# gafniguy/4D-Facial-Avatars

Measured on AMD Instinct MI355X. Metric: rays/sec at 512x512, 64 coarse + 128 fine samples, higher is better.
Workload: dtype f32; 1 GPU; configs[1]: paper-model eval forward, 512x512 frame, 64+128 samples, chunksize 65536, perturb on, expression+latent conditioned, background prior; frames sharded over GPUs

## Files before the change

### 4d-facial-avatars_amd/csrc/nf_mlp_gated_stats.hip

```cpp
#include "nf_mlp_live_kernel.h"

static int nf_gated_stats_launch(bool clocks, const float* packed, const float* bound, const float* cond, const float* ro, const float* rd,
                                 const float* rd_view, const float* z, int64_t n_rays, int n_samples, float* raw, float* scratch,
                                 size_t scratch_floats, int max_workgroups, int64_t* stats, size_t stats_rows, nf_stream_t stream) {
    static_assert(sizeof(long long) == sizeof(int64_t), "a statistics row is int64s");
    if (max_workgroups < 0 || !stats || ((uintptr_t)stats & 7) || stats_rows < (size_t)nf_live_grid_cap(max_workgroups) * NF_MLP_WAVES) return NF_EINVAL;
    const size_t cols = NF_GATE_STAT_COLS + (clocks ? NF_LIVE_PHASES : 0);
    const hipError_t e = hipMemsetAsync(stats, 0, stats_rows * cols * sizeof(int64_t), nf_s(stream));
    if (e != hipSuccess) return (int)e;
    return nf_live_launch<true, true>(packed, cond, ro, rd, rd_view, z, n_rays, n_samples, raw, scratch, scratch_floats, max_workgroups,
                                      reinterpret_cast<long long*>(stats), stream, bound, clocks);
}

extern "C" int nf_paper_mlp_fwd_gated_stats(const float* packed, const float* bound, const float* cond, const float* ro, const float* rd,
                                            const float* rd_view, const float* z, int64_t n_rays, int n_samples, float* raw, float* scratch,
                                            size_t scratch_floats, int max_workgroups, int64_t* stats, size_t stats_rows, nf_stream_t stream) {
    return nf_gated_stats_launch(false, packed, bound, cond, ro, rd, rd_view, z, n_rays, n_samples, raw, scratch, scratch_floats, max_workgroups,
                                 stats, stats_rows, stream);
}

extern "C" int nf_paper_mlp_fwd_gated_phases(const float* packed, const float* bound, const float* cond, const float* ro, const float* rd,
                                             const float* rd_view, const float* z, int64_t n_rays, int n_samples, float* raw, float* scratch,
                                             size_t scratch_floats, int max_workgroups, int64_t* stats, size_t stats_rows, nf_stream_t stream) {
    return nf_gated_stats_launch(true, packed, bound, cond, ro, rd, rd_view, z, n_rays, n_samples, raw, scratch, scratch_floats, max_workgroups,
                                 stats, stats_rows, stream);
}
```

### 4d-facial-avatars_amd/csrc/nf_mlp_live_kernel.h

```cpp
#pragma once
#include <mutex>
#include "nf_mlp_paper_net.h"

#define NF_LIVE_ROWS 64
#ifndef NF_LIVE_PF
#define NF_LIVE_PF 8
#endif
#define NF_LIVE_DIR_B (NF_LIVE_ROWS * 1024)
#define NF_LIVE_META_B (NF_LIVE_DIR_B + NF_LIVE_ROWS * 64)
#define NF_LIVE_WAVE_B (NF_LIVE_META_B + NF_LIVE_ROWS * 16)
#define NF_LIVE_OOB NF_LIVE_WAVE_B
#define NF_LIVE_SC1 16

static_assert(NF_LIVE_ROWS == 64 && NF_MLP_NT == 2, "row numbers wrap with & 63; a pass's liveness is one 32-bit mask");
static_assert(NF_LIVE_PF >= 0 && NF_LIVE_PF <= 16, "prefetched rows live in registers beside fc_alpha's weights");

__device__ __forceinline__ __amdgpu_buffer_rsrc_t nf_live_ring(char* ring_v) {
    const uint64_t a = (uint64_t)ring_v;
    const uint64_t s = (uint64_t)(uint32_t)__builtin_amdgcn_readfirstlane((int)(uint32_t)a) |
                       ((uint64_t)(uint32_t)__builtin_amdgcn_readfirstlane((int)(a >> 32)) << 32);
    return __builtin_amdgcn_make_buffer_rsrc(reinterpret_cast<char*>(s), (short)0, NF_LIVE_WAVE_B, 0x00020000);
}
__device__ __forceinline__ void nf_live_store(__amdgpu_buffer_rsrc_t ring, int off_b, f32x4 v) {
    __builtin_amdgcn_raw_buffer_store_b128(__builtin_bit_cast(nf_u32x4, v), ring, off_b, 0, 0);
}
__device__ __forceinline__ f32x4 nf_live_load(__amdgpu_buffer_rsrc_t ring, int off_b) {
    return __builtin_bit_cast(f32x4, __builtin_amdgcn_raw_buffer_load_b128(ring, off_b, 0, NF_LIVE_SC1));
}
__device__ __forceinline__ int nf_live_pop(unsigned& m) {
    const int r = __builtin_ctz(m);
    m &= m - 1u;
    return r;
}
__device__ __forceinline__ int nf_live_slab(int prow, int lane) { return nf_act_idx4(prow, lane); }

struct NfLivePre {
    NfStream<NF_MLP_NT>& st;
    f32x4 (&wd)[16];
    f32x4 (&pf)[NF_LIVE_PF > 0 ? NF_LIVE_PF : 1];
    char* ring_v;
    int head_v, tail_v;
    __device__ __forceinline__ void wait() const {
        __builtin_amdgcn_fence(__ATOMIC_RELEASE, "workgroup");
        __builtin_amdgcn_s_waitcnt(0x0F70);
        __builtin_amdgcn_fence(__ATOMIC_ACQUIRE, "workgroup");
    }
    __device__ __forceinline__ void loads(const NfW& Wi, const NfW& Ci, int lane) {
        using Net = NfPaperNet;
        const __amdgpu_buffer_rsrc_t ring = nf_live_ring(ring_v);
        const int tail = __builtin_amdgcn_readfirstlane(tail_v), cnt = __builtin_amdgcn_readfirstlane(head_v) - tail;
#pragma unroll
        for (int i = 0; i < NF_LIVE_PF; ++i)
            pf[i] = nf_live_load(ring, i < cnt ? ((tail + i) & (NF_LIVE_ROWS - 1)) * 1024 + lane * 16 : NF_LIVE_OOB);
        nf_load_bias<8>(st.bias, Ci, Net::B_D0, lane);
        nf_load_w16<8>(st.wa, Wi, Net::OFF_D0 / 4, lane);
        nf_load_w16<8>(wd, Wi, Net::OFF_D0 / 4 + 16 * 9 * 64, lane);
        __builtin_amdgcn_sched_barrier(0);
    }
};

struct NfGatePre {
    NfStream<NF_MLP_NT>& st;
    f32x4 (&pf)[NF_LIVE_PF > 0 ? NF_LIVE_PF : 1];
    char* ring_v;
    int head_v, tail_v;
    const float* bound_v;
    __device__ __forceinline__ NfW image() const {
        const uint64_t a = (uint64_t)bound_v;
        const uint64_t s = (uint64_t)(uint32_t)__builtin_amdgcn_readfirstlane((int)(uint32_t)a) |
                           ((uint64_t)(uint32_t)__builtin_amdgcn_readfirstlane((int)(a >> 32)) << 32);
        return nf_w_image(reinterpret_cast<const float*>(s), NF_BOUND_FLOATS);
    }
    __device__ __forceinline__ void wait() const {
        __builtin_amdgcn_fence(__ATOMIC_RELEASE, "workgroup");
        __builtin_amdgcn_s_waitcnt(0x0F70);
        __builtin_amdgcn_fence(__ATOMIC_ACQUIRE, "workgroup");
    }
    __device__ __forceinline__ void loads(const NfW& Wi, const NfW& Ci, int lane) {
        using Net = NfPaperNet;
        const __amdgpu_buffer_rsrc_t ring = nf_live_ring(ring_v);
        const int tail = __builtin_amdgcn_readfirstlane(tail_v), cnt = __builtin_amdgcn_readfirstlane(head_v) - tail;
#pragma unroll
        for (int i = 0; i < NF_LIVE_PF; ++i)
            pf[i] = nf_live_load(ring, i < cnt ? ((tail + i) & (NF_LIVE_ROWS - 1)) * 1024 + lane * 16 : NF_LIVE_OOB);
        nf_load_bias<16>(st.bias, Ci, Net::B_FEAT, lane);
        nf_load_w16<16>(st.wa, Wi, Net::OFF_FEAT / 4, lane);
        __builtin_amdgcn_sched_barrier(0);
    }
};

#define NF_LIVE_STAT_UNITS 0
#define NF_LIVE_STAT_RUNS 1
#define NF_LIVE_STAT_FLUSH 2
#define NF_LIVE_STAT_CLOCK 3
#define NF_GATE_STAT_PROVEN 4
#define NF_LIVE_PH_TRUNK 0
#define NF_LIVE_PH_TILE 1
#define NF_LIVE_PH_APPEND 2
#define NF_LIVE_PH_ENTRY 3
#define NF_LIVE_PH_RUN 4
#define NF_LIVE_PH_DEAD 5
#define NF_LIVE_PHASES 6
#define NF_LIVE_STAT_COLS 4
#define NF_GATE_STAT_COLS 5

template <bool STATS, int COLS = NF_LIVE_STAT_COLS>
__device__ __forceinline__ void nf_live_stat(long long* stats, int col, long long add, bool set = false) {
    if constexpr (STATS) {
        const int cols = COLS + (((uintptr_t)stats & 1) ? NF_LIVE_PHASES : 0);
        stats = reinterpret_cast<long long*>((uintptr_t)stats & ~(uintptr_t)7);
        if ((threadIdx.x & 63) == 0) {
            long long* at = stats + ((size_t)blockIdx.x * NF_MLP_WAVES + (threadIdx.x >> 6)) * cols + col;
            if (set) *at = add;
            else (void)__hip_atomic_fetch_add(at, add, __ATOMIC_RELAXED, __HIP_MEMORY_SCOPE_AGENT);
        }
    }
}

template <bool STATS, int COLS>
__device__ __forceinline__ void nf_live_mark(long long* stats, int end, int start) {
    if constexpr (STATS) {
        if ((uintptr_t)stats & 1) {
            __builtin_amdgcn_sched_barrier(0);
            const long long t = (long long)__builtin_amdgcn_s_memtime();
            if ((threadIdx.x & 63) == 0) {
                long long* row = reinterpret_cast<long long*>((uintptr_t)stats & ~(uintptr_t)7) +
                                 ((size_t)blockIdx.x * NF_MLP_WAVES + (threadIdx.x >> 6)) * (COLS + NF_LIVE_PHASES) + COLS;
                if (end >= 0) (void)__hip_atomic_fetch_add(row + end, t, __ATOMIC_RELAXED, __HIP_MEMORY_SCOPE_AGENT);
                if (start >= 0) (void)__hip_atomic_fetch_add(row + start, -t, __ATOMIC_RELAXED, __HIP_MEMORY_SCOPE_AGENT);
            }
            __builtin_amdgcn_sched_barrier(0);
        }
    }
}
template <class Pre, int COLS>
struct NfMarkedPre : Pre {
    long long* stats;
    __device__ __forceinline__ void wait() const {
        nf_live_mark<true, COLS>(stats, NF_LIVE_PH_TRUNK, NF_LIVE_PH_TILE);
        Pre::wait();
    }
};

template <int NT, bool STATS, bool GATE = false>
__global__ void __launch_bounds__(64 * NF_MLP_WAVES, 1)
k_paper_mlp_fwd_live(const float* __restrict__ packed, const float* __restrict__ cond_, const float* __restrict__ ro,
                     const float* __restrict__ rd, const float* __restrict__ rd_view, const float* __restrict__ z,
                     int64_t n_points, int S, float* __restrict__ raw, float* __restrict__ scratch, unsigned* __restrict__ counter,
                     long long* __restrict__ stats, const float* __restrict__ bound) {
    using Net = NfPaperNet;
    constexpr int COLS = GATE ? NF_GATE_STAT_COLS : NF_LIVE_STAT_COLS;
    __shared__ __attribute__((aligned(16))) f32x4 lds[NF_MLP_WAVES * 16 * NT * 64];
    const int lane = threadIdx.x & 63, wave = threadIdx.x >> 6;
    f32x4* act4 = lds + wave * (16 * NT * 64);
    typedef __attribute__((address_space(1))) f32x4 nf_gf32x4;
    nf_gf32x4* raw_v = (nf_gf32x4*)raw;
    asm volatile("" : "+v"(raw_v));
    char* ring_v = reinterpret_cast<char*>(scratch) + ((size_t)blockIdx.x * NF_MLP_WAVES + wave) * NF_LIVE_WAVE_B;
    asm volatile("" : "+v"(ring_v));
    const float* z_v = z;
    const float* rdv_v = rd_view;
    asm volatile("" : "+v"(z_v), "+v"(rdv_v));
    const float* bound_v = bound;
    if constexpr (GATE) asm volatile("" : "+v"(bound_v));
    int head_v = 0, tail_v = 0;
    asm volatile("" : "+v"(head_v), "+v"(tail_v));
    typedef __attribute__((address_space(1))) unsigned nf_gu32;
    nf_gu32* ctr_v = (nf_gu32*)counter;
    asm volatile("" : "+v"(ctr_v));
    unsigned unit_v = 0;
    if (lane == 0) unit_v = __hip_atomic_fetch_add(ctr_v, 1u, __ATOMIC_RELAXED, __HIP_MEMORY_SCOPE_AGENT);
    asm volatile("" : "+v"(unit_v));
#pragma unroll 1
    for (;;) {
        const int64_t p0 = (int64_t)(uint32_t)__builtin_amdgcn_readfirstlane((int)unit_v) * (16 * NT);
        int64_t p0_v = p0;
        asm volatile("" : "+v"(p0_v));
        int more_v = p0 < n_points;
        asm volatile("" : "+v"(more_v));
        const bool more = __builtin_amdgcn_readfirstlane(more_v) != 0;
        unsigned next_v = 0;
        if (more && lane == 0) next_v = __hip_atomic_fetch_add(ctr_v, 1u, __ATOMIC_RELAXED, __HIP_MEMORY_SCOPE_AGENT);
        if (more) nf_live_stat<STATS, COLS>(stats, NF_LIVE_STAT_UNITS, 1);
        int opaque0 = 0;
        asm volatile("" : "+s"(opaque0));
        const NfW Wi = nf_w_image(packed + opaque0, Net::PACKED), Ci = nf_w_image(cond_ + opaque0, Net::COND_FLOATS);
        NfStream<NT> st;
        f32x4 wd[16], pf[NF_LIVE_PF > 0 ? NF_LIVE_PF : 1];
        f32x4 dirf[NT][1];
        float sigma_own[NT];
        float tag_own[NT] = {};
        bool proven[NT] = {};
        int live_v = 0, run_v = 0;
        if (more) {
            nf_live_mark<STATS, COLS>(stats, -1, NF_LIVE_PH_TRUNK);
            f32x4 pe[NT][4];
            nf_net_inputs<NT>(pe, dirf, p0, n_points, S, lane, ro, rd, rdv_v, z_v);
            f32x4 acc[NT][16];
            if constexpr (GATE) {
                if constexpr (STATS)
                    nf_paper_net_body<Net, NT, 1, true, NfMarkedPre<NfGatePre, COLS>, true>(
                        acc, sigma_own, pe, dirf, Wi, Ci, act4, lane, NfMarkedPre<NfGatePre, COLS>{{st, pf, ring_v, head_v, tail_v, bound_v}, stats});
                else
                    nf_paper_net_body<Net, NT, 1, true, NfGatePre, true>(acc, sigma_own, pe, dirf, Wi, Ci, act4, lane,
                                                                         NfGatePre{st, pf, ring_v, head_v, tail_v, bound_v});
#pragma unroll
                for (int t = 0; t < NT; ++t) {
                    const float s = acc[t][8].x, u = acc[t][8].y;
                    sigma_own[t] = nf_add(s, nf_mul(u, 0x1p-13f));
                    proven[t] = sigma_own[t] < -0x1p-100f && s > -INFINITY && u < INFINITY;
                }
            } else if constexpr (STATS) {
                nf_paper_net_body<Net, NT, 1, true>(acc, sigma_own, pe, dirf, Wi, Ci, act4, lane,
                                                    NfMarkedPre<NfLivePre, COLS>{{st, wd, pf, ring_v, head_v, tail_v}, stats});
            } else {
                nf_paper_net_body<Net, NT, 1, true>(acc, sigma_own, pe, dirf, Wi, Ci, act4, lane, NfLivePre{st, wd, pf, ring_v, head_v, tail_v});
            }
            nf_live_mark<STATS, COLS>(stats, NF_LIVE_PH_TILE, NF_LIVE_PH_APPEND);
            int lane_o = lane;
            asm volatile("" : "+v"(lane_o));
            const int g = lane_o >> 4, c = lane_o & 15;
            unsigned live = 0;
            int S_o = S;
            asm volatile("" : "+v"(S_o));
            const int64_t p0_o = (int64_t)(uint32_t)__builtin_amdgcn_readfirstlane((int)(uint32_t)p0_v) |
                                 ((int64_t)__builtin_amdgcn_readfirstlane((int)(p0_v >> 32)) << 32);
#pragma unroll
            for (int t = 0; t < NT; ++t) {
                const int64_t p = p0_o + 16 * t + c;
                bool is_live;
                if constexpr (GATE) {
                    const bool last = (p + 1) % S_o == 0;
                    is_live = g == 0 && p < n_points && (!proven[t] || last);
                    tag_own[t] = __int_as_float(last ? 1 : 0);
                } else {
                    is_live = g == 0 && p < n_points && (!(sigma_own[t] <= 0.0f) || (p + 1) % S_o == 0);
                }
                live |= ((unsigned)__builtin_amdgcn_ballot_w64(is_live) & 0xffffu) << (16 * t);
            }
            const int head = __builtin_amdgcn_readfirstlane(head_v), cnt = head - __builtin_amdgcn_readfirstlane(tail_v);
            const int n_live = __builtin_popcount(live);
            live_v = (int)live;
            if constexpr (GATE) {
                const int64_t left = n_points - p0_o;
                nf_live_stat<STATS, COLS>(stats, NF_GATE_STAT_PROVEN, (left < 16 * NT ? (int)left : 16 * NT) - n_live);
            }
            if (cnt + n_live >= 16 * NT) {
                run_v = 1;
            } else {
                const __amdgpu_buffer_rsrc_t ring = nf_live_ring(ring_v);
                unsigned mm = live;
#pragma unroll 1
                for (int i = 0; i < n_live; i += 4) {
                    f32x4 v[4];
                    int off[4];
#pragma unroll
                    for (int u = 0; u < 4; ++u) {
                        const bool ok = i + u < n_live;
                        const int r = ok ? nf_live_pop(mm) : 0;
                        off[u] = ok ? ((head + i + u) & (NF_LIVE_ROWS - 1)) * 1024 + lane_o * 16 : NF_LIVE_OOB;
                        v[u] = act4[nf_live_slab(r, lane_o)];
                    }
#pragma unroll
                    for (int u = 0; u < 4; ++u) nf_live_store(ring, off[u], v[u]);
                }
#pragma unroll
                for (int t = 0; t < NT; ++t) {
                    const int bit = 16 * t + c;
                    if ((live >> bit) & 1u) {
                        const int row = (head + __builtin_popcount(live & ((1u << bit) - 1u))) & (NF_LIVE_ROWS - 1);
                        nf_live_store(ring, NF_LIVE_DIR_B + row * 64 + g * 16, dirf[t][0]);
                        if (g == 0) {
                            const int64_t p = p0_o + bit;
                            nf_live_store(ring, NF_LIVE_META_B + row * 16,
                                          (f32x4){__int_as_float((int)(uint32_t)p), __int_as_float((int)(p >> 32)), GATE ? tag_own[t] : sigma_own[t], 0.0f});
                        }
                    }
                }
                head_v = head + n_live;
                asm volatile("" : "+v"(head_v));
            }
            nf_live_mark<STATS, COLS>(stats, NF_LIVE_PH_APPEND, -1);
        } else {
            if constexpr (GATE) {
                NfGatePre pre{st, pf, ring_v, head_v, tail_v, bound_v};
                pre.wait();
                pre.loads(Wi, Ci, lane);
            } else {
                NfLivePre pre{st, wd, pf, ring_v, head_v, tail_v};
                pre.wait();
                pre.loads(Wi, Ci, lane);
            }
#pragma unroll
            for (int t = 0; t < NT; ++t) {
                dirf[t][0] = (f32x4){0.0f, 0.0f, 0.0f, 0.0f};
                sigma_own[t] = 0.0f;
            }
            run_v = __builtin_amdgcn_readfirstlane(head_v) != __builtin_amdgcn_readfirstlane(tail_v) ? 2 : 0;
        }
        asm volatile("" : "+v"(live_v), "+v"(run_v));
        const int run = __builtin_amdgcn_readfirstlane(run_v);
        if (run != 0) {
            nf_live_stat<STATS, COLS>(stats, NF_LIVE_STAT_RUNS, 1);
            if (run == 2) nf_live_stat<STATS, COLS>(stats, NF_LIVE_STAT_FLUSH, __builtin_amdgcn_readfirstlane(head_v) - __builtin_amdgcn_readfirstlane(tail_v));
            nf_live_mark<STATS, COLS>(stats, -1, NF_LIVE_PH_ENTRY);
            int lane_o = lane;
            asm volatile("" : "+v"(lane_o));
            const int g = lane_o >> 4, c = lane_o & 15;
            const __amdgpu_buffer_rsrc_t ring = nf_live_ring(ring_v);
            const int tail = __builtin_amdgcn_readfirstlane(tail_v), cnt = __builtin_amdgcn_readfirstlane(head_v) - tail;
            const unsigned own = run == 1 ? (unsigned)__builtin_amdgcn_readfirstlane(live_v) : 0u;
            const unsigned fill = run == 1 ? ~own : (1u << cnt) - 1u;
            const int n_fill = __builtin_popcount(fill);
            f32x4 meta[NT];
            bool valid[NT];
#pragma unroll
            for (int t = 0; t < NT; ++t) {
                const int bit = 16 * t + c;
                const bool f = (fill >> bit) & 1u;
                const int row = (tail + __builtin_popcount(fill & ((1u << bit) - 1u))) & (NF_LIVE_ROWS - 1);
                const f32x4 fd = nf_live_load(ring, f ? NF_LIVE_DIR_B + row * 64 + g * 16 : NF_LIVE_OOB);
                const f32x4 fm = nf_live_load(ring, f ? NF_LIVE_META_B + row * 16 : NF_LIVE_OOB);
                const int64_t p = (p0_v) + bit;
                dirf[t][0] = f ? fd : dirf[t][0];
                meta[t] = f ? fm : (f32x4){__int_as_float((int)(uint32_t)p), __int_as_float((int)(p >> 32)), GATE ? tag_own[t] : sigma_own[t], 0.0f};
                valid[t] = f || ((own >> bit) & 1u);
            }
            unsigned hh = fill;
#pragma unroll
            for (int i = 0; i < NF_LIVE_PF; ++i) {
                if (i < n_fill) {
                    const int h = nf_live_pop(hh);
                    act4[nf_live_slab(h, lane_o)] = pf[i];
                }
            }
#pragma unroll 1
            for (int i = NF_LIVE_PF; i < n_fill; i += 4) {
                f32x4 v[4];
                int h[4];
#pragma unroll
                for (int u = 0; u < 4; ++u) {
                    const bool ok = i + u < n_fill;
                    h[u] = ok ? nf_live_pop(hh) : -1;
                    v[u] = nf_live_load(ring, ok ? ((tail + i + u) & (NF_LIVE_ROWS - 1)) * 1024 + lane_o * 16 : NF_LIVE_OOB);
                }
#pragma unroll
                for (int u = 0; u < 4; ++u)
                    if (h[u] >= 0) act4[nf_live_slab(h[u], lane_o)] = v[u];
            }
            constexpr int NDIR = 1;
            constexpr unsigned D0 = Net::OFF_D0 / 4;
            nf_read_b<NT>(st.b0, act4, lane, 0);
            nf_live_mark<STATS, COLS>(stats, NF_LIVE_PH_ENTRY, NF_LIVE_PH_RUN);
            f32x4 acc[NT][16], bj[NT];
            float sigma_raw[NT];
            if constexpr (GATE) {
                nf_seg_lds<NT, 16, true, true>(acc, st, Wi, Net::OFF_FEAT / 4, 16, act4, lane);
                nf_pending_b<NT, true>(bj, st);
                nf_tail<NT, 16, 16, 9, 1>(acc, st.wb, bj, st, Wi, D0, Ci, Net::B_D0, act4, lane);
                NF_NET_COLOUR();
            } else {
                NF_NET_COLOUR_D0(8, 9, wd);
                NF_NET_COLOUR_REST();
            }
            int lane_s = lane;
            asm volatile("" : "+v"(lane_s));
            if ((lane_s >> 4) == 0) {
#pragma unroll
                for (int t = 0; t < NT; ++t) {
                    if (valid[t]) {
                        const int64_t p = (int64_t)(uint32_t)__float_as_int(meta[t].x) | ((int64_t)__float_as_int(meta[t].y) << 32);
                        if constexpr (GATE) {
                            const bool keep = !(sigma_raw[t] <= 0.0f) || __float_as_int(meta[t].z) != 0;
                            if (p >= 0 && p < n_points)
                                raw_v[p] = (f32x4){keep ? acc[t][0].x : 0.0f, keep ? acc[t][0].y : 0.0f, keep ? acc[t][0].z : 0.0f, sigma_raw[t]};
                        } else {
                            if (p >= 0 && p < n_points) raw_v[p] = (f32x4){acc[t][0].x, acc[t][0].y, acc[t][0].z, meta[t].z};
                        }
                    }
                }
            }
            tail_v = tail + n_fill;
            asm volatile("" : "+v"(tail_v));
            nf_live_mark<STATS, COLS>(stats, NF_LIVE_PH_RUN, -1);
        }
        asm volatile("" : "+v"(more_v));
        if (__builtin_amdgcn_readfirstlane(more_v) == 0) break;
        {
            nf_live_mark<STATS, COLS>(stats, -1, NF_LIVE_PH_DEAD);
            int lane_s = lane;
            asm volatile("" : "+v"(lane_s));
            const int g = lane_s >> 4, c = lane_s & 15;
            asm volatile("" : "+v"(live_v));
#pragma unroll
            for (int t = 0; t < NT; ++t) {
                const int64_t p = p0_v + 16 * t + c;
                if (g == 0 && p < n_points && !(((unsigned)live_v >> (16 * t + c)) & 1u)) raw_v[p] = (f32x4){0.0f, 0.0f, 0.0f, sigma_own[t]};
            }
            nf_live_mark<STATS, COLS>(stats, NF_LIVE_PH_DEAD, -1);
        }
        asm volatile("" : "+v"(next_v));
        unit_v = next_v;
    }
    nf_live_stat<STATS, COLS>(stats, NF_LIVE_STAT_CLOCK, (long long)wall_clock64(), true);
}

static inline int64_t nf_live_grid_cap(int max_workgroups) {
    const int64_t cu = nf_cu_count();
    return max_workgroups > 0 && max_workgroups < cu ? max_workgroups : cu;
}

#define NF_LIVE_SLOTS 256
#define NF_LIVE_SLOT_B 128

inline unsigned* nf_live_counter(hipStream_t stream) {
    struct Pool {
        char* base;
        const void* owner[NF_LIVE_SLOTS];
        int used;
    };
    static std::mutex mu;
    static Pool pools[64];
    static thread_local char this_thread;
    int dev = 0;
    if (hipGetDevice(&dev) != hipSuccess || dev < 0 || dev >= 64) return nullptr;
    const void* key = stream == hipStreamPerThread ? (const void*)&this_thread : (const void*)stream;
    std::lock_guard<std::mutex> lock(mu);
    Pool& p = pools[dev];
    if (!p.base) {
        void* mem = nullptr;
        if (hipMalloc(&mem, (size_t)NF_LIVE_SLOTS * NF_LIVE_SLOT_B) != hipSuccess) {
            (void)hipGetLastError();
            return nullptr;
        }
        p.base = (char*)mem;
        p.used = 0;
    }
    int i = 0;
    while (i < p.used && p.owner[i] != key) ++i;
    if (i == p.used) {
        if (p.used == NF_LIVE_SLOTS) {
            if (hipDeviceSynchronize() != hipSuccess) return nullptr;
            p.used = i = 0;
        }
        p.owner[p.used++] = key;
    }
    return reinterpret_cast<unsigned*>(p.base + (size_t)i * NF_LIVE_SLOT_B);
}

template <bool STATS, bool GATE = false>
static inline int nf_live_launch(const float* packed, const float* cond, const float* ro, const float* rd, const float* rd_view, const float* z,
                                 int64_t n_rays, int n_samples, float* raw, float* scratch, size_t scratch_floats, int max_workgroups,
                                 long long* stats, nf_stream_t stream, const float* bound = nullptr, bool clocks = false) {
    static_assert(NF_MLP_WAVES * 16 * NF_MLP_NT == 128, "nf_mlp_fwd_launch sizes the grid for 128 points per workgroup");
    if (max_workgroups < 0 || !scratch || ((uintptr_t)scratch & 15) ||
        scratch_floats < (size_t)nf_live_grid_cap(max_workgroups) * NF_MLP_WAVES * (NF_LIVE_WAVE_B / 4) ||
        (GATE && (!bound || ((uintptr_t)bound & 15))))
        return NF_EINVAL;
    const float* rdv = rd_view ? rd_view : rd;
    if (STATS && clocks) stats = reinterpret_cast<long long*>((uintptr_t)stats | 1);
    int rc = 0;
    const int launched = nf_mlp_fwd_launch(NF_FWD_INFER, packed, cond, ro, rd, z, raw, nullptr, n_rays, n_samples, [&](int64_t n_points, unsigned grid) {
        if ((n_points + 31) / 32 > ((int64_t)1 << 31)) {
            rc = NF_EINVAL;
            return;
        }
        unsigned* counter = nf_live_counter(nf_s(stream));
        if (!counter) {
            rc = (int)hipErrorOutOfMemory;
            return;
        }
        const hipError_t e = hipMemsetAsync(counter, 0, sizeof(unsigned), nf_s(stream));
        if (e != hipSuccess) {
            rc = (int)e;
            return;
        }
        const int64_t cap = nf_live_grid_cap(max_workgroups);
        hipLaunchKernelGGL((k_paper_mlp_fwd_live<NF_MLP_NT, STATS, GATE>), dim3((unsigned)(grid < cap ? grid : cap)), dim3(64 * NF_MLP_WAVES), 0,
                           nf_s(stream), packed, cond, ro, rd, rdv, z, n_points, n_samples, raw, scratch, counter, stats, bound);
    });
    return rc ? rc : launched;
}
```

### 4d-facial-avatars_amd/csrc/nf_mlp_live_stats.hip

```cpp
#include "nf_mlp_live_kernel.h"

static int nf_live_stats_launch(bool clocks, const float* packed, const float* cond, const float* ro, const float* rd, const float* rd_view,
                                const float* z, int64_t n_rays, int n_samples, float* raw, float* scratch, size_t scratch_floats,
                                int max_workgroups, int64_t* stats, size_t stats_rows, nf_stream_t stream) {
    static_assert(sizeof(long long) == sizeof(int64_t), "a statistics row is int64s");
    if (max_workgroups < 0 || !stats || ((uintptr_t)stats & 7) || stats_rows < (size_t)nf_live_grid_cap(max_workgroups) * NF_MLP_WAVES) return NF_EINVAL;
    const size_t cols = NF_LIVE_STAT_COLS + (clocks ? NF_LIVE_PHASES : 0);
    const hipError_t e = hipMemsetAsync(stats, 0, stats_rows * cols * sizeof(int64_t), nf_s(stream));
    if (e != hipSuccess) return (int)e;
    return nf_live_launch<true>(packed, cond, ro, rd, rd_view, z, n_rays, n_samples, raw, scratch, scratch_floats, max_workgroups,
                                reinterpret_cast<long long*>(stats), stream, nullptr, clocks);
}

extern "C" int nf_paper_mlp_fwd_live_stats(const float* packed, const float* cond, const float* ro, const float* rd, const float* rd_view,
                                           const float* z, int64_t n_rays, int n_samples, float* raw, float* scratch, size_t scratch_floats,
                                           int max_workgroups, int64_t* stats, size_t stats_rows, nf_stream_t stream) {
    return nf_live_stats_launch(false, packed, cond, ro, rd, rd_view, z, n_rays, n_samples, raw, scratch, scratch_floats, max_workgroups, stats,
                                stats_rows, stream);
}

extern "C" int nf_paper_mlp_fwd_live_phases(const float* packed, const float* cond, const float* ro, const float* rd, const float* rd_view,
                                            const float* z, int64_t n_rays, int n_samples, float* raw, float* scratch, size_t scratch_floats,
                                            int max_workgroups, int64_t* stats, size_t stats_rows, nf_stream_t stream) {
    return nf_live_stats_launch(true, packed, cond, ro, rd, rd_view, z, n_rays, n_samples, raw, scratch, scratch_floats, max_workgroups, stats,
                                stats_rows, stream);
}
```

### 4d-facial-avatars_amd/csrc/nf_mlp_net_common.h

```cpp
#pragma once
#include "nf_mlp_dev.h"
#include "nf_mlp_stream.h"

template <int NT>
__device__ __forceinline__ void nf_net_inputs(f32x4 (&pe)[NT][4], f32x4 (&dirf)[NT][1], int64_t p0, int64_t n_points, int S, int lane,
                                              const float* __restrict__ ro, const float* __restrict__ rd,
                                              const float* __restrict__ rd_view, const float* __restrict__ z) {
    const int g = lane >> 4, c = lane & 15;
#pragma unroll
    for (int t = 0; t < NT; ++t) {
        int64_t p = p0 + 16 * t + c;
        if (p >= n_points) p = n_points - 1;
        const int64_t ray = p / S;
        const float zz = z[p];
        const float dx = rd[ray * 3 + 0], dy = rd[ray * 3 + 1], dz = rd[ray * 3 + 2];
        const float px = nf_add(ro[ray * 3 + 0], nf_mul(dx, zz));
        const float py = nf_add(ro[ray * 3 + 1], nf_mul(dy, zz));
        const float pz = nf_add(ro[ray * 3 + 2], nf_mul(dz, zz));
        nf_encode_point(px, py, pz, g, pe[t]);
        float s, cs;
        nf_sincos(nf_mul(rd_view[ray * 3 + 2], (float)(1 << g)), &s, &cs);
        dirf[t][0] = (f32x4){s, cs, 0.0f, 0.0f};
    }
}

template <int NT>
__device__ __forceinline__ void nf_net_inputs_encoded(f32x4 (&pe)[NT][4], f32x4 (&dirf)[NT][2], int64_t p0, int64_t n_points, int lane,
                                                      const float* __restrict__ x87) {
    const int g = lane >> 4, c = lane & 15;
#pragma unroll
    for (int t = 0; t < NT; ++t) {
        int64_t p = p0 + 16 * t + c;
        if (p >= n_points) p = n_points - 1;
        const float* row = x87 + p * 87;
#pragma unroll
        for (int j = 0; j < 4; ++j) {
            float v[4];
#pragma unroll
            for (int r = 0; r < 4; ++r) {
                const int col = nfl::pe_slot_to_col(16 * j + 4 * g + r);
                v[r] = col >= 0 ? row[col] : 0.0f;
            }
            pe[t][j] = (f32x4){v[0], v[1], v[2], v[3]};
        }
#pragma unroll
        for (int j = 0; j < 2; ++j) {
            float v[4];
#pragma unroll
            for (int r = 0; r < 4; ++r) {
                const int s = 16 * j + 4 * g + r;
                v[r] = s < 24 ? row[63 + s] : 0.0f;
            }
            dirf[t][j] = (f32x4){v[0], v[1], v[2], v[3]};
        }
    }
}

template <int NT>
__device__ __forceinline__ void nf_net_store_raw(const f32x4 (&acc)[NT][16], const float (&sigma_raw)[NT], int64_t p0, int64_t n_points,
                                                 int lane, float* __restrict__ out) {
    const int g = lane >> 4, c = lane & 15;
    if (g == 0) {
#pragma unroll
        for (int t = 0; t < NT; ++t) {
            const int64_t p = p0 + 16 * t + c;
            if (p < n_points) reinterpret_cast<f32x4*>(out)[p] = (f32x4){acc[t][0].x, acc[t][0].y, acc[t][0].z, sigma_raw[t]};
        }
    }
}

#define NF_NET_PE_B(J_) do { _Pragma("unroll") for (int t = 0; t < NT; ++t) bj[t] = pe[t][J_]; } while (0)
#define NF_NET_PE_LAYER(B_, OFF_, OFF_NEXT_, B_NEXT_)                                                         \
    do {                                                                                                      \
        nf_load_bias<16>(st.bias, Ci, B_, lane);                                                              \
        f32x4 w[16];                                                                                          \
        nf_load_w16<16>(w, Wi, (OFF_) / 4, lane);                                                             \
        NF_NET_PE_B(0); nf_chunk<NT, 16, true>(acc, w, bj, st.bias);                                          \
        nf_load_w16<16>(w, Wi, (OFF_) / 4 + 1 * 16 * 64, lane);                                               \
        NF_NET_PE_B(1); nf_chunk<NT, 16, false>(acc, w, bj, st.bias);                                         \
        nf_load_w16<16>(w, Wi, (OFF_) / 4 + 2 * 16 * 64, lane);                                               \
        NF_NET_PE_B(2); nf_chunk<NT, 16, false>(acc, w, bj, st.bias);                                         \
        nf_load_w16<16>(w, Wi, (OFF_) / 4 + 3 * 16 * 64, lane);                                               \
        NF_NET_PE_B(3); nf_tail<NT, 16, 16, 16, 1>(acc, w, bj, st, Wi, (OFF_NEXT_) / 4, Ci, B_NEXT_, act4, lane); \
    } while (0)

#define NF_NET_SAVE_PENDING(RELU_, MASKL_, NCH_)                                                    \
    do {                                                                                            \
        nf_pending_b<NT, RELU_>(bj, st);                                                            \
        if ((MASKL_) >= 0) {                                                                        \
            nf_mask_bits<NT>(m64, st.bp, (NCH_) - 2);                                               \
            nf_mask_bits<NT>(m64, bj, (NCH_) - 1);                                                  \
            _Pragma("unroll") for (int t = 0; t < NT; ++t)                                          \
                if (p0 + 16 * t < n)                                                                \
                    *nf_mask_ptr<Net::S_MASK>(saved, n, (MASKL_) >= 0 ? (MASKL_) : 0, (p0 >> 4) + t, lane) = make_uint2((uint32_t)m64[t], (uint32_t)(m64[t] >> 32)); \
        }                                                                                           \
    } while (0)
#define NF_NET_SAVE_LAYER256(OFF_, FIRST_, SEC_, MASKL_, OFF_NEXT_, B_NEXT_, NO_NEXT_, NEXT_B_)                           \
    do {                                                                                                                   \
        NfCopyH<64, 4, ((MASKL_) >= 0)> cs{act4, sec(SEC_, 256), lane, 8, {}};                                             \
        cs.prime();                                                                                                        \
        _Pragma("unroll") for (int t = 0; t < NT; ++t) m64[t] = 0;                                                         \
        nf_seg_lds<NT, 16, FIRST_, ((MASKL_) >= 0), ((MASKL_) >= 0)>(acc, st, Wi, OFF_, 16, act4, lane, cs, m64);          \
        NF_NET_SAVE_PENDING(((MASKL_) >= 0), MASKL_, 16);                                                                  \
        nf_tail<NT, 16, 16, NO_NEXT_, NEXT_B_>(acc, st.wb, bj, st, Wi, OFF_NEXT_, Ci, B_NEXT_, act4, lane);               \
    } while (0)

#define NF_NET_CHAIN_BEGIN(MASKL_, OFF_NEXT_, NO_NEXT_)                                                               \
    static_assert(NT == 2, "the copy schedule below is written for 32-point slabs");                                 \
    const int lane = threadIdx.x & 63, wave = threadIdx.x >> 6;                                                      \
    const int g = lane >> 4, c = lane & 15;                                                                          \
    const int64_t p0 = ((int64_t)blockIdx.x * NF_MLP_WAVES + wave) * (16 * NT);                                      \
    if (p0 >= n_points) return;                                                                                      \
    f32x4* act4 = lds + wave * (16 * NT * 64);                                                                       \
    const int64_t n = n_points;                                                                                      \
    const NfW Wi = nf_w_image(packed_t, Net::PACKED_T);                                                              \
    auto sec = [&](int zs, int width) { return nf_slab_copy(dz, zs, width, p0, n); };                                \
    auto masks = [&](int l, uint2 (&m)[NT]) {                                                                        \
        _Pragma("unroll") for (int t = 0; t < NT; ++t)                                                               \
            m[t] = p0 + 16 * t < n ? *nf_mask_ptr<Net::S_MASK>(const_cast<float*>(saved), n, l, (p0 >> 4) + t, lane) : make_uint2(0u, 0u); \
    };                                                                                                               \
    f32x4 frag_rgb[NT][1], frag_sig[NT];                                                                             \
    _Pragma("unroll") for (int t = 0; t < NT; ++t) {                                                                 \
        const int64_t p = p0 + 16 * t + c;                                                                           \
        f32x4 d = (f32x4){0.f, 0.f, 0.f, 0.f};                                                                       \
        if (p < n && g == 0) d = reinterpret_cast<const f32x4*>(d_raw)[p];                                           \
        frag_rgb[t][0] = (f32x4){d.x, d.y, d.z, 0.f};                                                                \
        frag_sig[t] = (f32x4){d.w, 0.f, 0.f, 0.f};                                                                   \
    }                                                                                                                \
    f32x4 acc[NT][16];                                                                                               \
    NfStream<NT> st;                                                                                                 \
    f32x4 bj[NT];                                                                                                    \
    uint64_t unused64[NT];                                                                                           \
    uint2 m[NT];                                                                                                     \
    _Pragma("unroll") for (int no = 0; no < 16; ++no) st.bias[no] = (f32x4){0.f, 0.f, 0.f, 0.f};                     \
    masks(MASKL_, m);                                                                                                \
    nf_zero_acc<NT, 8>(acc);                                                                                         \
    nf_mma_from_regs<NT, 8, 1>(acc, reinterpret_cast<const f32x4*>(packed_t) + Net::OFFT_RGB / 4, frag_rgb, lane);   \
    nf_apply_mask<NT, 8>(acc, m);                                                                                    \
    nf_store_act<NT, 8, false>(acc, act4, lane);                                                                     \
    nf_load_w16<NO_NEXT_>(st.wa, Wi, OFF_NEXT_, lane);                                                               \
    nf_read_b<NT>(st.b0, act4, lane, 0)
#define NF_NET_CHAIN_LAYER(OFF_, NO_, NCH_, W4_, ZSEC_, MASKL_, OFF_NEXT_, NO_NEXT_)                                   \
    do {                                                                                                             \
        NfCopyH<W4_, 4, false> cs{act4, sec(ZSEC_, 4 * (W4_)), lane, (NCH_) / 2, {}};                                  \
        cs.prime();                                                                                                  \
        if ((MASKL_) >= 0) masks((MASKL_) >= 0 ? (MASKL_) : 0, m);                                                   \
        nf_seg_lds<NT, NO_, true, false, false>(acc, st, Wi, OFF_, NCH_, act4, lane, cs, unused64);                  \
        nf_pending_b<NT, false>(bj, st);                                                                             \
        nf_tail_dz<NT, NO_, NO_NEXT_, ((MASKL_) >= 0)>(acc, st.wb, bj, st, Wi, OFF_NEXT_, act4, lane, m);            \
    } while (0)
#define NF_NET_CHAIN_END(ZSEC_)                                                                                      \
    do {                                                                                                             \
        const NfSlabCopy cp = sec(ZSEC_, 256);                                                                       \
        _Pragma("unroll 4") for (int k = 0; k < 16 * NT; ++k) nf_copy_rows<64>(act4, cp, k, lane);                   \
    } while (0)
```

### 4d-facial-avatars_amd/csrc/nf_mlp_paper_net.h

```cpp
#pragma once
#include "nf_mlp_net_common.h"
#include "nf_mlp_smaller_layout.h"
#include "nf_pack.h"

#define NF_NET_COMMON(F)                                                                                                              \
    F(FRAG) F(NCOND) F(OFF_L0) F(OFF_L1) F(OFF_L2) F(OFF_L3) F(OFF_L4) F(OFF_FEAT) F(OFF_D0) F(OFF_D0E) F(OFF_D1) F(OFF_D2) F(OFF_RGB) \
    F(OFF_WC0) F(OFF_WC3) F(OFF_WCD) F(OFF_BIAS) F(B_L0) F(B_L1) F(B_L2) F(B_L3) F(B_L4) F(B_FEAT) F(B_D0) F(B_D1) F(B_D2) F(B_RGB)     \
    F(B_CVEC) F(B_DVEC) F(COND_FLOATS) F(S_PE) F(S_H0) F(S_H1) F(S_H2) F(S_H3) F(S_H4) F(S_FEAT) F(S_D0) F(S_D1) F(S_D2) F(S_DIRF)     \
    F(S_MASK) F(SAVED_PER_POINT) F(Z_L0) F(Z_L1) F(Z_L2) F(Z_L3) F(Z_L4) F(Z_FEAT) F(Z_D0) F(Z_D1) F(Z_D2) F(DZ_PER_POINT)             \
    F(OFFT_RGB) F(OFFT_D2) F(OFFT_D1) F(OFFT_D0) F(OFFT_FEAT) F(OFFT_L4) F(OFFT_L3) F(OFFT_L2) F(OFFT_L1)                              \
    F(G_L0) F(G_L1) F(G_L2) F(G_L3A) F(G_L3B) F(G_L4) F(G_FEAT) F(G_D0A) F(G_D0B) F(G_D1) F(G_D2) F(G_RGB) F(G_ALPHA)                  \
    F(CS_L0) F(CS_D0) F(CS_RGB) F(SLAB_FLOATS) F(GRAD_PARAM_FLOATS) F(GRAD_FLOATS)

struct NfPaperNet {
#define NF_NET_COPY(X) static constexpr int X = nfl::X;
    NF_NET_COMMON(NF_NET_COPY)
    NF_NET_COPY(OFF_L5) NF_NET_COPY(B_L5) NF_NET_COPY(S_H5) NF_NET_COPY(Z_L5) NF_NET_COPY(OFFT_L5) NF_NET_COPY(G_L5)
#undef NF_NET_COPY
    static constexpr bool HAS_L5 = true, D0_EXPR = false;
    static constexpr int PACKED = nfl::PACKED_FLOATS, PACKED_T = nfl::PACKED_T_FLOATS, NPARAMS = NF_PAPER_NUM_PARAMS;
    static constexpr int N_RELU = (nfl::SAVED_PER_POINT - nfl::S_MASK) / 8;
    static constexpr int D0_COLS = 280;
    static constexpr int MODEL = 0;
};

struct NfSmallerNet {
#define NF_NET_COPY(X) static constexpr int X = nsm::X;
    NF_NET_COMMON(NF_NET_COPY)
    NF_NET_COPY(OFF_WCE) NF_NET_COPY(NEXPR) NF_NET_COPY(PACKED) NF_NET_COPY(PACKED_T) NF_NET_COPY(NPARAMS) NF_NET_COPY(N_RELU)
#undef NF_NET_COPY
    static constexpr bool HAS_L5 = false, D0_EXPR = true;
    static constexpr int D0_COLS = 280 + nsm::NEXPR;
    static constexpr int MODEL = 2;
};
#undef NF_NET_COMMON

template <class Net> constexpr int nf_net_n_xyz = Net::HAS_L5 ? 6 : 5;

enum { NF_R_XYZ0_W = 0, NF_R_XYZ3_W = 6, NF_R_L5_W = 10, NF_R_FEAT_W = 12, NF_R_FEAT_B = 13, NF_R_ALPHA_W = 14, NF_R_ALPHA_B = 15,
       NF_R_DIR0_W = 16, NF_R_DIR0_B = 17, NF_R_DIR1_W = 18, NF_R_DIR2_W = 20, NF_R_RGB_W = 24, NF_R_RGB_B = 25 };
template <class Net>
__host__ __device__ constexpr int nf_net_id(int role) {
    return role >= NF_R_RGB_W ? Net::NPARAMS - 2 + (role - NF_R_RGB_W) : (role >= NF_R_FEAT_W && !Net::HAS_L5 ? role - 2 : role);
}
template <class Net>
__host__ __device__ constexpr int nf_net_role(int id) {
    return id >= Net::NPARAMS - 2 ? NF_R_RGB_W + (id - (Net::NPARAMS - 2)) : (id >= NF_R_L5_W && !Net::HAS_L5 ? id + 2 : id);
}

template <class Net>
static void nf_paper_net_table(std::vector<uint32_t>& t) {
    constexpr int NX = nf_net_n_xyz<Net>;
    auto id = [](int role) { return nf_net_id<Net>(role); };
    t.assign(Net::PACKED, NF_ZERO_CODE);
    auto fill = [&](int off, int nk, int no_tiles, int tensor, int n_out, int n_cols, auto col_of, int alpha_row = -1) {
        nf_fill_frag(t, off, nk, no_tiles, [&](int slot, int n) {
            if (n < n_out) {
                const int col = col_of(slot);
                return col >= 0 ? nf_code(tensor, n, col, n_cols) : NF_ZERO_CODE;
            }
            return n == alpha_row && slot < 256 ? nf_code(id(NF_R_ALPHA_W), 0, slot, 256) : NF_ZERO_CODE;
        });
    };
    auto ident = [](int s) { return s; };
    fill(Net::OFF_L0, 4, 16, NF_R_XYZ0_W, 256, 171, [](int s) { return nfl::pe_slot_to_col(s); });
    fill(Net::OFF_L1, 16, 16, 2, 256, 256, ident);
    fill(Net::OFF_L2, 16, 16, 4, 256, 256, ident);
    fill(Net::OFF_L3, 20, 16, NF_R_XYZ3_W, 256, 427, [](int s) { return s < 64 ? nfl::pe_slot_to_col(s) : 171 + (s - 64); });
    fill(Net::OFF_L4, 16, 16, 8, 256, 256, ident);
    if constexpr (Net::HAS_L5) fill(Net::OFF_L5, 16, 16, NF_R_L5_W, 256, 256, ident);
    fill(Net::OFF_FEAT, 16, 16, id(NF_R_FEAT_W), 256, 256, ident);
    fill(Net::OFF_D0, 17, 9, id(NF_R_DIR0_W), 128, Net::D0_COLS,
         [](int s) {
             if (s < 256) return s;
             const int g = ((s - 256) >> 2) & 3, r = (s - 256) & 3;
             return r < 2 ? 256 + 6 * g + 3 * r : -1;
         },
         128);
    fill(Net::OFF_D0E, 18, 9, id(NF_R_DIR0_W), 128, Net::D0_COLS, [](int s) { return s < 280 ? s : -1; }, 128);
    fill(Net::OFF_D1, 8, 8, id(NF_R_DIR1_W), 128, 128, ident);
    fill(Net::OFF_D2, 8, 8, id(NF_R_DIR2_W), 128, 128, ident);
    fill(Net::OFF_RGB, 8, 1, id(NF_R_RGB_W), 3, 128, ident);
    for (int n = 0; n < 256; ++n)
        for (int k = 0; k < Net::NCOND; ++k) {
            t[Net::OFF_WC0 + n * Net::NCOND + k] = nf_code(NF_R_XYZ0_W, n, 63 + k, 171);
            t[Net::OFF_WC3 + n * Net::NCOND + k] = nf_code(NF_R_XYZ3_W, n, 63 + k, 427);
        }
    for (int n = 0; n < 128; ++n) {
        for (int f = 0; f < 4; ++f)
            for (int sc = 0; sc < 2; ++sc)
                for (int comp = 1; comp < 3; ++comp)
                    t[Net::OFF_WCD + n * 16 + 4 * f + 2 * sc + (comp - 1)] = nf_code(id(NF_R_DIR0_W), n, 256 + 6 * f + 3 * sc + comp, Net::D0_COLS);
        if constexpr (Net::D0_EXPR)
            for (int k = 0; k < Net::NEXPR; ++k) t[Net::OFF_WCE + n * Net::NEXPR + k] = nf_code(id(NF_R_DIR0_W), n, 280 + k, Net::D0_COLS);
    }
    for (int n = 0; n < 256; ++n) {
        for (int l = 0; l < NX; ++l) t[Net::OFF_BIAS + 256 * l + n] = nf_code(2 * l + 1, 0, n, 256);
        t[Net::OFF_BIAS + Net::B_FEAT + n] = nf_code(id(NF_R_FEAT_B), 0, n, 256);
    }
    for (int n = 0; n < 128; ++n) {
        t[Net::OFF_BIAS + Net::B_D0 + n] = nf_code(id(NF_R_DIR0_B), 0, n, 128);
        t[Net::OFF_BIAS + Net::B_D1 + n] = nf_code(id(NF_R_DIR1_W) + 1, 0, n, 128);
        t[Net::OFF_BIAS + Net::B_D2 + n] = nf_code(id(NF_R_DIR2_W) + 1, 0, n, 128);
    }
    t[Net::OFF_BIAS + Net::B_D0 + 128] = nf_code(id(NF_R_ALPHA_B), 0, 0, 1);
    for (int n = 0; n < 3; ++n) t[Net::OFF_BIAS + Net::B_RGB + n] = nf_code(id(NF_R_RGB_B), 0, n, 3);
}

template <class Net>
static inline size_t nf_paper_net_saved_floats(int64_t n_points) {
    return (size_t)Net::SAVED_PER_POINT * (size_t)((n_points + 31) & ~(int64_t)31) + Net::N_RELU * 128;
}

template <class Net, bool DIRS>
__device__ __forceinline__ void nf_paper_net_condition(const float* __restrict__ packed, const float* __restrict__ expr,
                                                       const float* __restrict__ latent, float near_z, float far_z, float* __restrict__ cond) {
    __shared__ float cvec[Net::NCOND];
    __shared__ float dvec[16];
    const int tid = threadIdx.x;
    if (tid < 76) cvec[tid] = nf_div(nf_mul(expr[tid], 1.0f), 3.0f);
    else if (tid < Net::NCOND) cvec[tid] = latent[tid - 76];
    if (tid >= 128 && tid < 144) {
        const int k = tid - 128, f = k >> 2, sc = (k >> 1) & 1, comp = k & 1;
        const float a = nf_mul(comp ? far_z : near_z, exp2f((float)f));
        dvec[k] = DIRS ? (sc ? cosf(a) : sinf(a)) : 0.0f;
    }
    __syncthreads();
    const float* bias = packed + Net::OFF_BIAS;
    for (int i = blockIdx.x * blockDim.x + tid; i < Net::COND_FLOATS; i += gridDim.x * blockDim.x) {
        if (i >= Net::B_CVEC) { cond[i] = i < Net::B_DVEC ? cvec[i - Net::B_CVEC] : dvec[i - Net::B_DVEC]; continue; }
        float v = bias[i];
        if (i < Net::B_L1 || (i >= Net::B_L3 && i < Net::B_L4)) {
            const int n = i < Net::B_L1 ? i : i - Net::B_L3;
            const float* w = packed + (i < Net::B_L1 ? Net::OFF_WC0 : Net::OFF_WC3) + n * Net::NCOND;
            float s = 0.0f;
            for (int k = 0; k < Net::NCOND; ++k) s = fmaf(w[k], cvec[k], s);
            v += s;
        } else if ((DIRS || Net::D0_EXPR) && i >= Net::B_D0 && i < Net::B_D0 + 128) {
            float s = 0.0f;
            if (DIRS) {
                const float* w = packed + Net::OFF_WCD + (i - Net::B_D0) * 16;
                for (int k = 0; k < 16; ++k) s = fmaf(w[k], dvec[k], s);
            }
            if constexpr (Net::D0_EXPR) {
                const float* we = packed + Net::OFF_WCE + (i - Net::B_D0) * Net::NEXPR;
                for (int k = 0; k < Net::NEXPR; ++k) s = fmaf(we[k], cvec[k], s);
            }
            v += s;
        }
        cond[i] = v;
    }
}

template <class Net>
static inline dim3 nf_paper_net_condition_grid() { return dim3((Net::COND_FLOATS + 255) / 256); }

#define NF_NET_L3_PE()                                                                                        \
    do {                                                                                                      \
        NF_NET_PE_B(0); nf_chunk<NT, 16, true>(acc, st.wa, bj, st.bias);                                          \
        nf_load_w16<16>(st.wa, Wi, Net::OFF_L3 / 4 + 4 * 16 * 64, lane);    \
        nf_read_b<NT>(st.b0, act4, lane, 0);                                                                  \
        f32x4 w[16];                                                                                          \
        nf_load_w16<16>(w, Wi, Net::OFF_L3 / 4 + 1 * 16 * 64, lane);                                          \
        NF_NET_PE_B(1); nf_chunk<NT, 16, false>(acc, w, bj, st.bias);                                             \
        nf_load_w16<16>(w, Wi, Net::OFF_L3 / 4 + 2 * 16 * 64, lane);                                          \
        NF_NET_PE_B(2); nf_chunk<NT, 16, false>(acc, w, bj, st.bias);                                             \
        nf_load_w16<16>(w, Wi, Net::OFF_L3 / 4 + 3 * 16 * 64, lane);                                          \
        NF_NET_PE_B(3); nf_chunk<NT, 16, false>(acc, w, bj, st.bias);                                             \
    } while (0)

#define NF_NET_COLOUR_D0(NO0_, WS0_, WD_)                                                                                  \
                                \
    {                                                                                                                      \
        nf_seg_lds<NT, NO0_, true, false, WS0_>(acc, st, Wi, D0, 16, act4, lane);                                          \
        nf_pending_b<NT, false>(bj, st);                                                                                   \
        nf_chunk<NT, NO0_, false>(acc, st.wb, bj, st.bias);                                                                \
        if (NDIR == 2) {                                                                                                   \
            nf_load_w16<NO0_>(st.wb, Wi, D0 + 17 * (WS0_) * 64, lane);                                                     \
            _Pragma("unroll") for (int t = 0; t < NT; ++t) bj[t] = dirf[t][0];                                             \
            nf_chunk<NT, NO0_, false>(acc, WD_, bj, st.bias);                                                              \
        }                                                                                                                  \
        _Pragma("unroll") for (int t = 0; t < NT; ++t) bj[t] = dirf[t][NDIR - 1];                                          \
        if constexpr (NDIR == 2) nf_tail<NT, NO0_, 8, 8, 1>(acc, st.wb, bj, st, Wi, Net::OFF_D1 / 4, Ci, Net::B_D1, act4, lane); \
        else nf_tail<NT, NO0_, 8, 8, 1>(acc, WD_, bj, st, Wi, Net::OFF_D1 / 4, Ci, Net::B_D1, act4, lane);                  \
        if constexpr ((NO0_) > 8) { _Pragma("unroll") for (int t = 0; t < NT; ++t) sigma_raw[t] = acc[t][8].x; }           \
    }
#define NF_NET_COLOUR()                                                                                                    \
    {                                                                                                                      \
        f32x4 wd[16];                                                                                                      \
        nf_load_w16<9>(wd, Wi, D0 + 16 * 9 * 64, lane);                      \
        NF_NET_COLOUR_D0(9, 9, wd);                                                                                        \
    }                                                                                                                      \
    NF_NET_COLOUR_REST()
#define NF_NET_COLOUR_REST()                                                                                               \
                                                                                           \
    nf_seg_lds<NT, 8, true, true>(acc, st, Wi, Net::OFF_D1 / 4, 8, act4, lane);                                            \
    nf_pending_b<NT, true>(bj, st);                                                                                        \
    nf_tail<NT, 8, 8, 8, 1>(acc, st.wb, bj, st, Wi, Net::OFF_D2 / 4, Ci, Net::B_D2, act4, lane);                           \
    nf_seg_lds<NT, 8, true, true>(acc, st, Wi, Net::OFF_D2 / 4, 8, act4, lane);                                            \
    nf_pending_b<NT, true>(bj, st);                                                                                        \
    nf_tail<NT, 8, 8, 1, 1>(acc, st.wb, bj, st, Wi, Net::OFF_RGB / 4, Ci, Net::B_RGB, act4, lane);                         \
                                                                                                     \
    nf_seg_lds<NT, 1, true, true>(acc, st, Wi, Net::OFF_RGB / 4, 8, act4, lane);                                           \
    nf_pending_b<NT, true>(bj, st);                                                                                        \
    nf_chunk<NT, 1, false>(acc, st.wb, bj, st.bias)

struct NfNoPre {
    __device__ __forceinline__ void wait() const {}
    __device__ __forceinline__ void loads(const NfW&, const NfW&, int) const {}
};
#define NF_BOUND_BIAS 4096
#define NF_BOUND_FLOATS (NF_BOUND_BIAS + 16)
template <int NT, bool RELU_IN, class Pre>
__device__ __forceinline__ void nf_net_lone_tile(f32x4 (&acc)[NT][16], const NfStream<NT>& st, f32x4 (&bj)[NT], const NfW& W, unsigned first4,
                                                 unsigned stride4, const NfW& Wi, const NfW& Ci, const f32x4* act4, int lane, Pre& pre) {
    f32x4 w8[16];
    w8[0] = st.wa[0];
    pre.wait();
#pragma unroll
    for (int ch = 1; ch < 16; ++ch) w8[ch] = nf_load_w1(W, first4 + stride4 * ch, lane);
    if constexpr (RELU_IN) __builtin_amdgcn_sched_barrier(0);
    pre.loads(Wi, Ci, lane);
    if constexpr (RELU_IN) {
        f32x4 cur[NT], nxt[NT];
#pragma unroll
        for (int t = 0; t < NT; ++t) cur[t] = nf_relu_i(st.b0[t]);
#pragma unroll
        for (int ch = 0; ch < 16; ++ch) {
            if (ch + 1 < 16) nf_read_b<NT>(nxt, act4, lane, ch + 1);
            __builtin_amdgcn_sched_barrier(0);
#pragma unroll
            for (int r = 0; r < 2; ++r)
#pragma unroll
                for (int t = 0; t < NT; ++t)
                    acc[t][8] = __builtin_amdgcn_mfma_f32_16x16x4f32(w8[ch][r], cur[t][r], (ch == 0 && r == 0) ? st.bias[0] : acc[t][8], 0, 0, 0);
#pragma unroll
            for (int r = 2; r < 4; ++r)
#pragma unroll
                for (int t = 0; t < NT; ++t) {
                    __builtin_amdgcn_sched_barrier(0);
                    if (ch + 1 < 16) {
                        const int e = 2 * (r - 2);
#pragma unroll
                        for (int q = e; q < e + 2; ++q) {
                            const int xi = __float_as_int(nxt[t][q]);
                            nxt[t][q] = __int_as_float(xi > 0 ? xi : 0);
                        }
                    }
                    __builtin_amdgcn_sched_barrier(0);
                    acc[t][8] = __builtin_amdgcn_mfma_f32_16x16x4f32(w8[ch][r], cur[t][r], acc[t][8], 0, 0, 0);
                }
            __builtin_amdgcn_sched_barrier(0);
#pragma unroll
            for (int t = 0; t < NT; ++t) cur[t] = nxt[t];
        }
        return;
    }
#pragma unroll
    for (int ch = 0; ch < 16; ++ch) {
        if (ch == 0) {
#pragma unroll
            for (int t = 0; t < NT; ++t) bj[t] = RELU_IN ? nf_relu_i(st.b0[t]) : st.b0[t];
        } else {
            nf_read_b<NT>(bj, act4, lane, ch);
            if (RELU_IN) {
#pragma unroll
                for (int t = 0; t < NT; ++t) bj[t] = nf_relu_i(bj[t]);
            }
        }
#pragma unroll
        for (int r = 0; r < 4; ++r)
#pragma unroll
            for (int t = 0; t < NT; ++t)
                acc[t][8] = __builtin_amdgcn_mfma_f32_16x16x4f32(w8[ch][r], bj[t][r], (ch == 0 && r == 0) ? st.bias[0] : acc[t][8], 0, 0, 0);
    }
}
template <class Net, int NT, int NDIR, bool SIGMA = false, class Pre = NfNoPre, bool GATE = false>
__device__ __forceinline__ void nf_paper_net_body(f32x4 (&acc)[NT][16], float (&sigma_raw)[NT], const f32x4 (&pe)[NT][4],
                                                  const f32x4 (&dirf)[NT][NDIR], const NfW& Wi, const NfW& Ci, f32x4* act4, int lane,
                                                  Pre pre = Pre()) {
    static_assert(!GATE || (SIGMA && Net::HAS_L5), "the bound tile stands in for fc_alpha's lone tile, behind layers_xyz.5");
    constexpr unsigned D0 = (NDIR == 1 ? Net::OFF_D0 : Net::OFF_D0E) / 4;
    NfStream<NT> st;
    f32x4 bj[NT];
#define NF_NET_LAYER256(OFF_, FIRST_, OFF_NEXT_, B_NEXT_, NO_NEXT_, NEXT_B_)                                                \
    nf_seg_lds<NT, 16, FIRST_, true>(acc, st, Wi, OFF_, 16, act4, lane);                                                    \
    nf_pending_b<NT, true>(bj, st);                                                                                         \
    nf_tail<NT, 16, 16, NO_NEXT_, NEXT_B_>(acc, st.wb, bj, st, Wi, OFF_NEXT_, Ci, B_NEXT_, act4, lane)
    NF_NET_PE_LAYER(Net::B_L0, Net::OFF_L0, Net::OFF_L1, Net::B_L1);
    NF_NET_LAYER256(Net::OFF_L1 / 4, true, Net::OFF_L2 / 4, Net::B_L2, 16, 1);
    NF_NET_LAYER256(Net::OFF_L2 / 4, true, Net::OFF_L3 / 4, Net::B_L3, 16, 0);
    NF_NET_L3_PE();
    NF_NET_LAYER256(Net::OFF_L3 / 4 + 4 * 16 * 64, false, Net::OFF_L4 / 4, Net::B_L4, 16, 1);
    if constexpr (GATE) {
        NF_NET_LAYER256(Net::OFF_L4 / 4, true, Net::OFF_L5 / 4, Net::B_L5, 16, 1);
        const NfW Bi = pre.image();
        nf_seg_lds<NT, 16, true, true>(acc, st, Wi, Net::OFF_L5 / 4, 16, act4, lane);
        nf_pending_b<NT, true>(bj, st);
        nf_tail<NT, 16, 16, 1, 1>(acc, st.wb, bj, st, Bi, 0, Bi, NF_BOUND_BIAS, act4, lane);
        nf_net_lone_tile<NT, true>(acc, st, bj, Bi, 0, 64, Wi, Ci, act4, lane, pre);
        return;
    } else if constexpr (Net::HAS_L5) {
        NF_NET_LAYER256(Net::OFF_L4 / 4, true, Net::OFF_L5 / 4, Net::B_L5, 16, 1);
        NF_NET_LAYER256(Net::OFF_L5 / 4, true, Net::OFF_FEAT / 4, Net::B_FEAT, 16, 1);
    } else {
        NF_NET_LAYER256(Net::OFF_L4 / 4, true, Net::OFF_FEAT / 4, Net::B_FEAT, 16, 1);
    }
    if constexpr (SIGMA) {
        NF_NET_LAYER256(Net::OFF_FEAT / 4, true, D0 + 8 * 64, Net::B_D0 + 128, 1, 1);
        nf_net_lone_tile<NT, false>(acc, st, bj, Wi, D0 + 8 * 64, 9 * 64, Wi, Ci, act4, lane, pre);
#pragma unroll
        for (int t = 0; t < NT; ++t) sigma_raw[t] = acc[t][8].x;
        return;
    }
    NF_NET_LAYER256(Net::OFF_FEAT / 4, true, D0, Net::B_D0, 9, 1);
#undef NF_NET_LAYER256
    NF_NET_COLOUR();
}

template <class Net, int NT>
__device__ __forceinline__ void nf_paper_net_fwd_encoded(f32x4* lds, const float* __restrict__ packed, const float* __restrict__ cond,
                                                         const float* __restrict__ x87, int64_t n_points, float* __restrict__ out) {
    const int lane = threadIdx.x & 63, wave = threadIdx.x >> 6;
    const int64_t p0 = ((int64_t)blockIdx.x * NF_MLP_WAVES + wave) * (16 * NT);
    if (p0 >= n_points) return;
    f32x4* act4 = lds + wave * (16 * NT * 64);
    f32x4 pe[NT][4];
    f32x4 dirf[NT][2];
    nf_net_inputs_encoded<NT>(pe, dirf, p0, n_points, lane, x87);
    f32x4 acc[NT][16];
    float sigma_raw[NT];
    const NfW Wi = nf_w_image(packed, Net::PACKED), Ci = nf_w_image(cond, Net::COND_FLOATS);
    nf_paper_net_body<Net, NT, 2>(acc, sigma_raw, pe, dirf, Wi, Ci, act4, lane);
    nf_net_store_raw<NT>(acc, sigma_raw, p0, n_points, lane, out);
}

template <class Condition, class Forward>
static inline int nf_paper_net_forward_encoded(const float* packed, const float* x87, const float* expr76, const float* latent32,
                                               int64_t n_points, float* cond, float* out, Condition condition, Forward forward) {
    if (n_points == 0) return 0;
    if (!packed || !x87 || !expr76 || !latent32 || !cond || !out || n_points < 0) return NF_EINVAL;
    condition();
    const int64_t per_block = (int64_t)NF_MLP_WAVES * 16 * NF_MLP_NT;
    const int64_t grid = (n_points + per_block - 1) / per_block;
    if (grid > 0x7fffffff) return NF_EINVAL;
    forward((unsigned)grid);
    NF_RETURN_LAUNCH();
}

template <class Net, int NT>
__device__ __forceinline__ void nf_paper_net_body_save(f32x4 (&acc)[NT][16], float (&sigma_raw)[NT], const f32x4 (&pe)[NT][4],
                                                       const f32x4 (&dirf)[NT][1], const NfW& Wi, const NfW& Ci, f32x4* act4, int lane,
                                                       float* __restrict__ saved, int64_t p0, int64_t n) {
    static_assert(NT == 2, "the copy schedule below is written for 32-point slabs");
    constexpr int NX = nf_net_n_xyz<Net>;
    const int g = lane >> 4, c = lane & 15;
    auto sec = [&](int s, int width) { return nf_slab_copy(saved, s, width, p0, n); };
#pragma unroll
    for (int t = 0; t < NT; ++t) {
        const int64_t p = p0 + 16 * t + c;
        if (p < n) *reinterpret_cast<f32x4*>(saved + Net::S_DIRF * n + p * 16 + 4 * g) = dirf[t][0];
#pragma unroll
        for (int j = 0; j < 4; ++j) act4[nf_act_idx4(16 * t + c, 4 * j + g)] = pe[t][j];
    }
    {
        const NfSlabCopy cp = sec(Net::S_PE, 64);
#pragma unroll
        for (int k = 0; k < 16 * NT / 4; ++k) nf_copy_rows<16>(act4, cp, k, lane);
    }
    uint64_t m64[NT];
    NfStream<NT> st;
    f32x4 bj[NT];
#define NF_NET_LAYER128(OFF_, NO_, SEC_, MASKL_)                                                                          \
    NfCopyH<32, 4, true> cs{act4, sec(SEC_, 128), lane, 4, {}};                                                            \
    cs.prime();                                                                                                            \
    _Pragma("unroll") for (int t = 0; t < NT; ++t) m64[t] = 0;                                                             \
    nf_seg_lds<NT, NO_, true, true, true>(acc, st, Wi, OFF_, 8, act4, lane, cs, m64);                                      \
    NF_NET_SAVE_PENDING(true, MASKL_, 8)
    NF_NET_PE_LAYER(Net::B_L0, Net::OFF_L0, Net::OFF_L1, Net::B_L1);
    NF_NET_SAVE_LAYER256(Net::OFF_L1 / 4, true, Net::S_H0, 0, Net::OFF_L2 / 4, Net::B_L2, 16, 1);
    NF_NET_SAVE_LAYER256(Net::OFF_L2 / 4, true, Net::S_H1, 1, Net::OFF_L3 / 4, Net::B_L3, 16, 0);
    NF_NET_L3_PE();
    NF_NET_SAVE_LAYER256(Net::OFF_L3 / 4 + 4 * 16 * 64, false, Net::S_H2, 2, Net::OFF_L4 / 4, Net::B_L4, 16, 1);
    if constexpr (Net::HAS_L5) {
        NF_NET_SAVE_LAYER256(Net::OFF_L4 / 4, true, Net::S_H3, 3, Net::OFF_L5 / 4, Net::B_L5, 16, 1);
        NF_NET_SAVE_LAYER256(Net::OFF_L5 / 4, true, Net::S_H4, 4, Net::OFF_FEAT / 4, Net::B_FEAT, 16, 1);
        NF_NET_SAVE_LAYER256(Net::OFF_FEAT / 4, true, Net::S_H5, 5, Net::OFF_D0 / 4, Net::B_D0, 9, 1);
    } else {
        NF_NET_SAVE_LAYER256(Net::OFF_L4 / 4, true, Net::S_H3, 3, Net::OFF_FEAT / 4, Net::B_FEAT, 16, 1);
        NF_NET_SAVE_LAYER256(Net::OFF_FEAT / 4, true, Net::S_H4, 4, Net::OFF_D0 / 4, Net::B_D0, 9, 1);
    }
    {
        f32x4 wd[16];
        nf_load_w16<9>(wd, Wi, Net::OFF_D0 / 4 + 16 * 9 * 64, lane);
        NfCopyH<64, 4, false> cs{act4, sec(Net::S_FEAT, 256), lane, 8, {}};
        cs.prime();
        nf_seg_lds<NT, 9, true, false, false>(acc, st, Wi, Net::OFF_D0 / 4, 16, act4, lane, cs, m64);
        NF_NET_SAVE_PENDING(false, -1, 16);
        nf_chunk<NT, 9, false>(acc, st.wb, bj, st.bias);
#pragma unroll
        for (int t = 0; t < NT; ++t) bj[t] = dirf[t][0];
        nf_tail<NT, 9, 8, 8, 1>(acc, wd, bj, st, Wi, Net::OFF_D1 / 4, Ci, Net::B_D1, act4, lane);
#pragma unroll
        for (int t = 0; t < NT; ++t) sigma_raw[t] = acc[t][8].x;
    }
    {
        NF_NET_LAYER128(Net::OFF_D1 / 4, 8, Net::S_D0, NX);
        nf_tail<NT, 8, 8, 8, 1>(acc, st.wb, bj, st, Wi, Net::OFF_D2 / 4, Ci, Net::B_D2, act4, lane);
    }
    {
        NF_NET_LAYER128(Net::OFF_D2 / 4, 8, Net::S_D1, NX + 1);
        nf_tail<NT, 8, 8, 1, 1>(acc, st.wb, bj, st, Wi, Net::OFF_RGB / 4, Ci, Net::B_RGB, act4, lane);
    }
    {
        NF_NET_LAYER128(Net::OFF_RGB / 4, 1, Net::S_D2, NX + 2);
        nf_chunk<NT, 1, false>(acc, st.wb, bj, st.bias);
    }
#undef NF_NET_LAYER128
}
#undef NF_NET_L3_PE

template <class Net, int NT>
__device__ __forceinline__ void nf_paper_net_fwd_save(f32x4* lds, const float* __restrict__ packed, const float* __restrict__ cond,
                                                      const float* __restrict__ ro, const float* __restrict__ rd,
                                                      const float* __restrict__ rd_view, const float* __restrict__ z, int64_t n_points, int S,
                                                      float* __restrict__ raw, float* __restrict__ saved) {
    const int lane = threadIdx.x & 63, wave = threadIdx.x >> 6;
    const int64_t p0 = ((int64_t)blockIdx.x * NF_MLP_WAVES + wave) * (16 * NT);
    if (p0 >= n_points) return;
    f32x4* act4 = lds + wave * (16 * NT * 64);
    f32x4 pe[NT][4];
    f32x4 dirf[NT][1];
    nf_net_inputs<NT>(pe, dirf, p0, n_points, S, lane, ro, rd, rd_view, z);
    f32x4 acc[NT][16];
    float sigma_raw[NT];
    const NfW Wi = nf_w_image(packed, Net::PACKED), Ci = nf_w_image(cond, Net::COND_FLOATS);
    nf_paper_net_body_save<Net, NT>(acc, sigma_raw, pe, dirf, Wi, Ci, act4, lane, saved, p0, n_points);
    nf_net_store_raw<NT>(acc, sigma_raw, p0, n_points, lane, raw);
}

template <class Fwd, class FwdSave>
static inline int nf_paper_net_launch_fwd(Fwd fwd, FwdSave fwd_save, const float* packed, const float* cond, const float* ro, const float* rd,
                                          const float* rd_view, const float* z, int64_t n_rays, int n_samples, float* raw, float* saved,
                                          nf_stream_t stream) {
    static_assert(NF_MLP_WAVES * 16 * NF_MLP_NT == 128, "nf_mlp_fwd_launch sizes the grid for 128 points per workgroup");
    const float* rdv = rd_view ? rd_view : rd;
    return nf_mlp_fwd_launch(saved ? NF_FWD_TRAIN_F32 : NF_FWD_INFER, packed, cond, ro, rd, z, raw, saved, n_rays, n_samples,
                             [&](int64_t n_points, unsigned grid) {
        if (saved)
            hipLaunchKernelGGL(fwd_save, dim3(grid), dim3(64 * NF_MLP_WAVES), 0, nf_s(stream), packed, cond, ro, rd, rdv, z, n_points,
                               n_samples, raw, saved);
        else
            hipLaunchKernelGGL(fwd, dim3((unsigned)(grid < nf_cu_count() ? grid : nf_cu_count())), dim3(64 * NF_MLP_WAVES), 0, nf_s(stream),
                               packed, cond, ro, rd, rdv, z, n_points, n_samples, raw);
    });
}

template <class Net, int NT>
__device__ __forceinline__ void nf_paper_net_fwd_sigma(f32x4* lds, const float* __restrict__ packed, const float* __restrict__ cond_,
                                                       const float* __restrict__ ro, const float* __restrict__ rd, const float* __restrict__ z,
                                                       int64_t n_points, int S, float* __restrict__ sigma) {
    const int lane = threadIdx.x & 63, wave = threadIdx.x >> 6;
    const int c = lane & 15;
    f32x4* act4 = lds + wave * (16 * NT * 64);
    typedef __attribute__((address_space(1))) float nf_gf32;
    nf_gf32* sigma_v = (nf_gf32*)sigma;
    asm volatile("" : "+v"(sigma_v));
    int stride_v = (int)gridDim.x;
    asm volatile("" : "+v"(stride_v));
    const float* z_v = z;
    asm volatile("" : "+v"(z_v));
#pragma unroll 1
    for (int64_t blk = blockIdx.x;; blk += __builtin_amdgcn_readfirstlane(stride_v)) {
        const int64_t p0 = (blk * NF_MLP_WAVES + wave) * (16 * NT);
        if (p0 >= n_points) break;
        int opaque0 = 0;
        asm volatile("" : "+s"(opaque0));
        const float* W = packed + opaque0;
        const float* cond = cond_ + opaque0;
        f32x4 pe[NT][4];
        f32x4 dirf[NT][1];
        nf_net_inputs<NT>(pe, dirf, p0, n_points, S, lane, ro, rd, rd, z_v);
        f32x4 acc[NT][16];
        float sigma_raw[NT];
        const NfW Wi = nf_w_image(W, Net::PACKED), Ci = nf_w_image(cond, Net::COND_FLOATS);
        nf_paper_net_body<Net, NT, 1, true>(acc, sigma_raw, pe, dirf, Wi, Ci, act4, lane);
        int lane_o = lane;
        asm volatile("" : "+v"(lane_o));
        if ((lane_o >> 4) == 0) {
#pragma unroll
            for (int t = 0; t < NT; ++t) {
                const int64_t p = p0 + 16 * t + c;
                if (p < n_points) sigma_v[p] = sigma_raw[t];
            }
        }
    }
}

template <class Sigma>
static inline int nf_paper_net_launch_sigma(Sigma kernel, const float* packed, const float* cond, const float* ro, const float* rd,
                                            const float* z, int64_t n_rays, int n_samples, float* sigma, nf_stream_t stream) {
    static_assert(NF_MLP_WAVES * 16 * NF_MLP_NT == 128, "nf_mlp_fwd_launch sizes the grid for 128 points per workgroup");
    return nf_mlp_fwd_launch(NF_FWD_INFER, packed, cond, ro, rd, z, sigma, nullptr, n_rays, n_samples, [&](int64_t n_points, unsigned grid) {
        hipLaunchKernelGGL(kernel, dim3((unsigned)(grid < nf_cu_count() ? grid : nf_cu_count())), dim3(64 * NF_MLP_WAVES), 0, nf_s(stream),
                           packed, cond, ro, rd, z, n_points, n_samples, sigma);
    });
}
```

### 4d-facial-avatars_amd/nerf/_hip.py

```python
from __future__ import annotations

import ctypes as C
import os
import threading

import torch

_LIB_PATH = os.environ.get("NERFACE_HIP_LIB") or os.path.join(os.path.dirname(os.path.dirname(os.path.abspath(__file__))), "lib",
                                                             "libnerface_hip.so")
_lib = None
_lock = threading.Lock()

NF_PAPER_NUM_PARAMS = 26

_P, _I, _L, _F, _Z = C.c_void_p, C.c_int, C.c_int64, C.c_float, C.c_size_t
_PROTOTYPES = {
    "nf_abi_version": (C.c_int, []),
    "nf_error_string": (C.c_char_p, [_I]),
    "nf_build_info": (C.c_char_p, []),
    "nf_ray_bundle": (C.c_int, [_I, _I, _F, _F, _F, _F, _P, _I, _P, _P, _P]),
    "nf_weighted_choice_workspace_bytes": (_Z, []),
    "nf_weighted_choice": (C.c_int, [_P, _P, _L, _I, _P, _P, _Z, _P]),
    "nf_ray_batch": (C.c_int, [_I, _I, _F, _F, _F, _F, _P, _I, _P, _I, _L, _P, _I, _P, _P, _P, _P, _P, _P, _P]),
    "nf_sample_coarse": (C.c_int, [_L, _I, _F, _F, _P, _P, _P, _P]),
    "nf_sample_coarse_ex": (C.c_int, [_L, _I, _F, _F, _P, _P, _I, _P, _P]),
    "nf_posenc": (C.c_int, [_P, _L, _I, _I, _I, _P, _P]),
    "nf_paper_packed_floats": (_Z, []),
    "nf_paper_cond_floats": (_Z, []),
    "nf_paper_gather_table": (C.c_int, [_P, _Z]),
    "nf_paper_pack": (C.c_int, [_P, _P, _P]),
    "nf_paper_condition": (C.c_int, [_P, _P, _P, _F, _F, _P, _P]),
    "nf_paper_mlp_fwd": (C.c_int, [_P, _P, _P, _P, _P, _P, _L, _I, _P, _P]),
    "nf_paper_forward_encoded": (C.c_int, [_P, _P, _P, _P, _L, _P, _P, _P]),
    "nf_paper_packed_bf16_bytes": (_Z, []),
    "nf_paper_pack_bf16": (C.c_int, [_P, _P, _P]),
    "nf_paper_mlp_fwd_bf16": (C.c_int, [_P, _P, _P, _P, _P, _P, _L, _I, _P, _P]),
    "nf_paper_packed_f16_bytes": (_Z, []),
    "nf_paper_f16_flag_offset": (_Z, []),
    "nf_paper_pack_f16": (C.c_int, [_P, _P, _P]),
    "nf_paper_mlp_fwd_f16": (C.c_int, [_P, _P, _P, _P, _P, _P, _L, _I, _P, _P]),
    "nf_paper_mlp_fwd_f16x2": (C.c_int, [_P, _P, _P, _P, _P, _P, _L, _I, _P, _P]),
    "nf_paper_mlp_fwd_train_f16": (C.c_int, [_P, _P, _P, _P, _P, _P, _L, _I, _P, _P, _P]),
    "nf_paper_packed_bwd_f16_bytes": (_Z, []),
    "nf_paper_pack_bwd_f16": (C.c_int, [_P, _P, _P]),
    "nf_paper_mlp_bwd_f16": (C.c_int, [_P, _P, _P, _P, _P, _L, _I, _P, _Z, _P, _P]),
    "nf_paper_mlp_fwd_train_bf16": (C.c_int, [_P, _P, _P, _P, _P, _P, _L, _I, _P, _P, _P]),
    "nf_paper_saved_floats": (_Z, [_L]),
    "nf_paper_mlp_fwd_train": (C.c_int, [_P, _P, _P, _P, _P, _P, _L, _I, _P, _P, _P]),
    "nf_paper_packed_bwd_floats": (_Z, []),
    "nf_paper_pack_bwd": (C.c_int, [_P, _P, _P]),
    "nf_paper_packed_bwd_bf16_bytes": (_Z, []),
    "nf_paper_pack_bwd_bf16": (C.c_int, [_P, _P, _P]),
    "nf_paper_mlp_bwd_bf16": (C.c_int, [_P, _P, _P, _P, _P, _L, _I, _P, _Z, _P, _I, _P, _P]),
    "nf_split_saved_to_f32": (C.c_int, [_I, _P, _L, _I, _P, _P]),
    "nf_paper_grad_floats": (_Z, []),
    "nf_paper_bwd_workspace_floats": (_Z, [_L]),
    "nf_paper_mlp_bwd": (C.c_int, [_P, _P, _P, _P, _P, _L, _I, _P, _Z, _P, _P]),
    "nf_paper_mlp_bwd_stage_ms": (C.c_int, [_P, _P, _I, _P, _P, _P, _L, _I, _P, _Z, _P, _P, _P]),
    "nf_lcode_packed_floats": (_Z, []),
    "nf_lcode_cond_floats": (_Z, []),
    "nf_lcode_pack": (C.c_int, [_P, _P, _P]),
    "nf_lcode_condition": (C.c_int, [_P, _P, _P, _F, _F, _P, _P]),
    "nf_lcode_mlp_fwd": (C.c_int, [_P, _P, _P, _P, _P, _P, _L, _I, _P, _P]),
    "nf_lcode_packed_bf16_bytes": (_Z, []),
    "nf_lcode_pack_bf16": (C.c_int, [_P, _P, _P]),
    "nf_lcode_mlp_fwd_bf16": (C.c_int, [_P, _P, _P, _P, _P, _P, _L, _I, _P, _P]),
    "nf_lcode_packed_f16_bytes": (_Z, []),
    "nf_lcode_f16_flag_offset": (_Z, []),
    "nf_lcode_pack_f16": (C.c_int, [_P, _P, _P]),
    "nf_lcode_mlp_fwd_f16": (C.c_int, [_P, _P, _P, _P, _P, _P, _L, _I, _P, _P]),
    "nf_lcode_mlp_fwd_f16x2": (C.c_int, [_P, _P, _P, _P, _P, _P, _L, _I, _P, _P]),
    "nf_lcode_mlp_fwd_train_f16": (C.c_int, [_P, _P, _P, _P, _P, _P, _L, _I, _P, _P, _P]),
    "nf_lcode_packed_bwd_f16_bytes": (_Z, []),
    "nf_lcode_pack_bwd_f16": (C.c_int, [_P, _P, _P]),
    "nf_lcode_mlp_bwd_f16": (C.c_int, [_P, _P, _P, _P, _P, _L, _I, _P, _Z, _P, _P]),
    "nf_lcode_mlp_fwd_train_bf16": (C.c_int, [_P, _P, _P, _P, _P, _P, _L, _I, _P, _P, _P]),
    "nf_lcode_packed_bwd_bf16_bytes": (_Z, []),
    "nf_lcode_pack_bwd_bf16": (C.c_int, [_P, _P, _P]),
    "nf_lcode_mlp_bwd_bf16": (C.c_int, [_P, _P, _P, _P, _P, _L, _I, _P, _Z, _P, _P]),
    "nf_selftest_dw_tables_f32": (C.c_int, []),
    "nf_selftest_dw_tables_lcode_f32": (C.c_int, []),
    "nf_selftest_dw_tables_bf16": (C.c_int, []),
    "nf_paper_stream_table_bf16": (C.c_long, [_P, _Z]),
    "nf_paper_stream_table_bwd_bf16": (C.c_long, [_P, _Z]),
    "nf_lcode_stream_table_bf16": (C.c_long, [_P, _Z]),
    "nf_lcode_stream_table_bwd_bf16": (C.c_long, [_P, _Z]),
    "nf_lcode_forward_encoded": (C.c_int, [_P, _P, _P, _P, _L, _P, _P, _P]),
    "nf_lcode_saved_floats": (_Z, [_L]),
    "nf_lcode_mlp_fwd_train": (C.c_int, [_P, _P, _P, _P, _P, _P, _L, _I, _P, _P, _P]),
    "nf_lcode_packed_bwd_floats": (_Z, []),
    "nf_lcode_pack_bwd": (C.c_int, [_P, _P, _P]),
    "nf_lcode_grad_floats": (_Z, []),
    "nf_lcode_bwd_workspace_floats": (_Z, [_L]),
    "nf_lcode_mlp_bwd": (C.c_int, [_P, _P, _P, _P, _P, _L, _I, _P, _Z, _P, _P]),
    "nf_smaller_packed_floats": (_Z, []),
    "nf_smaller_cond_floats": (_Z, []),
    "nf_smaller_gather_table": (C.c_int, [_P, _Z]),
    "nf_smaller_pack": (C.c_int, [_P, _P, _P]),
    "nf_smaller_condition": (C.c_int, [_P, _P, _P, _F, _F, _P, _P]),
    "nf_smaller_mlp_fwd": (C.c_int, [_P, _P, _P, _P, _P, _P, _L, _I, _P, _P]),
    "nf_smaller_forward_encoded": (C.c_int, [_P, _P, _P, _P, _L, _P, _P, _P]),
    "nf_smaller_saved_floats": (_Z, [_L]),
    "nf_smaller_mlp_fwd_train": (C.c_int, [_P, _P, _P, _P, _P, _P, _L, _I, _P, _P, _P]),
    "nf_smaller_packed_bwd_floats": (_Z, []),
    "nf_smaller_pack_bwd": (C.c_int, [_P, _P, _P]),
    "nf_smaller_grad_floats": (_Z, []),
    "nf_smaller_bwd_workspace_floats": (_Z, [_L]),
    "nf_smaller_mlp_bwd": (C.c_int, [_P, _P, _P, _P, _P, _L, _I, _P, _Z, _P, _P]),
    "nf_smaller_mlp_bwd_stage_ms": (C.c_int, [_P, _P, _P, _P, _P, _L, _I, _P, _Z, _P, _P, _P]),
    "nf_selftest_dw_tables_smaller_f32": (C.c_int, []),
    "nf_eval_postprocess": (C.c_int, [_P, _P, _P, _I, _I, _F, _F, _F, _F, _P, _P, _P]),
    "nf_tiny_packed_floats": (_Z, []),
    "nf_tiny_pack": (C.c_int, [_P, _P, _P]),
    "nf_tiny_mlp_fwd": (C.c_int, [_P, _P, _P, _P, _I, _L, _I, _P, _P]),
    "nf_render_volume_density": (C.c_int, [_P, _P, _L, _I, _P, _P, _P, _P]),
    "nf_tiny_saved_floats": (_Z, [_L]),
    "nf_tiny_mlp_fwd_train": (C.c_int, [_P, _P, _P, _P, _I, _L, _I, _P, _P, _P]),
    "nf_render_volume_density_bwd": (C.c_int, [_P, _P, _P, _L, _I, _P, _P]),
    "nf_render_volume_density_bwd_full": (C.c_int, [_P, _P, _P, _P, _P, _L, _I, _P, _P]),
    "nf_tiny_packed_bwd_floats": (_Z, []),
    "nf_tiny_pack_bwd": (C.c_int, [_P, _P, _P]),
    "nf_tiny_grad_floats": (_Z, []),
    "nf_tiny_bwd_workspace_floats": (_Z, [_L]),
    "nf_tiny_mlp_bwd": (C.c_int, [_P, _P, _P, _L, _I, _P, _Z, _P, _P]),
    "nf_selftest_dw_tables_tiny": (C.c_int, []),
    "nf_flex_packed_floats": (_Z, [_I]),
    "nf_flex_pack": (C.c_int, [_I, _P, _P, _P]),
    "nf_flex_mlp_fwd": (C.c_int, [_I, _P, _P, _P, _P, _I, _L, _I, _P, _P]),
    "nf_flex_saved_floats": (_Z, [_I, _L]),
    "nf_flex_mlp_fwd_train": (C.c_int, [_I, _P, _P, _P, _P, _I, _L, _I, _P, _P, _P]),
    "nf_flex_packed_bwd_floats": (_Z, [_I]),
    "nf_flex_pack_bwd": (C.c_int, [_I, _P, _P, _P]),
    "nf_flex_grad_floats": (_Z, [_I]),
    "nf_flex_bwd_workspace_floats": (_Z, [_I, _L]),
    "nf_flex_mlp_bwd": (C.c_int, [_I, _P, _P, _P, _L, _I, _P, _Z, _P, _P]),
    "nf_selftest_dw_tables_flex": (C.c_int, [_I]),
    "nf_volume_render_fwd": (C.c_int, [_P, _P, _P, _P, _P, _L, _I, _I, _P, _P, _P, _P, _P]),
    "nf_volume_render_bwd": (C.c_int, [_P, _P, _P, _P, _P, _P, _L, _I, _I, _P, _P]),
    "nf_volume_render_bwd_full": (C.c_int, [_P, _P, _P, _P, _P, _P, _P, _P, _P, _P, _L, _I, _I, _P, _P, _P]),
    "nf_sample_pdf": (C.c_int, [_P, _P, _P, _L, _L, _I, _I, _P, _P]),
    "nf_sample_pdf_ex": (C.c_int, [_P, _P, _P, _L, _L, _I, _I, _P, _P, _P, _P]),
    "nf_resample_merge": (C.c_int, [_P, _P, _P, _L, _L, _I, _I, _P, _P, _P]),
    "nf_render_rays_workspace_floats": (_Z, [_L, _I, _I]),
    "nf_render_rays_fwd": (C.c_int, [_P] * 13 + [_L, _P, _P, _L, _I, _I, _F, _F, _I, _P, _Z] + [_P] * 7 + [_P]),
    "nf_render_rays_fwd_f16": (C.c_int, [_P] * 13 + [_L, _P, _P, _L, _I, _I, _F, _F, _I, _P, _Z] + [_P] * 7 + [_P]),
    "nf_render_rays_fwd_f16x2": (C.c_int, [_P] * 13 + [_L, _P, _P, _L, _I, _I, _F, _F, _I, _P, _Z] + [_P] * 7 + [_P]),
    "nf_adam_step": (C.c_int, [_P, _P, _P, _P, _P, _I, _F, _F, _F, _F, _L, _P]),
    "nf_train_loss_fwd": (C.c_int, [_P, _P, _P, _L, _P, _I, _F, _F, _P, _P]),
    "nf_train_loss_bwd": (C.c_int, [_P, _P, _P, _L, _P, _I, _F, _F, _P, _P, _P, _P, _P, _P]),
    "nf_adam_step_dev": (C.c_int, [_P, _P, _P, _P, _P, _I, _F, _F, _F, _P, _P]),
    "nf_train_loss_bg_fwd": (C.c_int, [_P, _P, _P, _L, _P, _I, _F, _F, _P, _P, _F, _P, _P]),
    "nf_train_loss_bg_bwd": (C.c_int, [_P, _P, _P, _L, _P, _I, _F, _F, _P, _P, _F, _P, _P, _P, _P, _P, _P, _P, _P]),
    "nf_sort_rows": (C.c_int, [_P, _L, _I, _P, _P]),
    "nf_image_metrics_workspace_bytes": (_Z, [_L, _I, _I]),
    "nf_image_metrics": (C.c_int, [_P, _P, _L, _I, _I, C.c_double, _P, _Z, _P, _P, _P]),
}
_FAMILY_ENTRY_POINTS = {
    "packed_floats": (_Z, []), "cond_floats": (_Z, []), "pack": (C.c_int, [_P, _P, _P]),
    "condition": (C.c_int, [_P, _P, _P, _F, _F, _P, _P]),
    "mlp_fwd": (C.c_int, [_P, _P, _P, _P, _P, _P, _L, _I, _P, _P]), "mlp_fwd_bf16": (C.c_int, [_P, _P, _P, _P, _P, _P, _L, _I, _P, _P]),
    "mlp_fwd_f16": (C.c_int, [_P, _P, _P, _P, _P, _P, _L, _I, _P, _P]), "mlp_fwd_f16x2": (C.c_int, [_P, _P, _P, _P, _P, _P, _L, _I, _P, _P]),
    "saved_floats": (_Z, [_L]),
    "mlp_fwd_train": (C.c_int, [_P, _P, _P, _P, _P, _P, _L, _I, _P, _P, _P]),
    "mlp_fwd_train_bf16": (C.c_int, [_P, _P, _P, _P, _P, _P, _L, _I, _P, _P, _P]),
    "mlp_fwd_train_f16": (C.c_int, [_P, _P, _P, _P, _P, _P, _L, _I, _P, _P, _P]),
    "packed_bwd_floats": (_Z, []), "pack_bwd": (C.c_int, [_P, _P, _P]),
    "packed_bf16_bytes": (_Z, []), "pack_bf16": (C.c_int, [_P, _P, _P]),
    "packed_bwd_bf16_bytes": (_Z, []), "pack_bwd_bf16": (C.c_int, [_P, _P, _P]),
    "packed_f16_bytes": (_Z, []), "pack_f16": (C.c_int, [_P, _P, _P]),
    "packed_bwd_f16_bytes": (_Z, []), "pack_bwd_f16": (C.c_int, [_P, _P, _P]),
    "f16_flag_offset": (_Z, []),
    "bwd_workspace_floats": (_Z, [_L]), "grad_floats": (_Z, []),
    "mlp_bwd": (C.c_int, [_P, _P, _P, _P, _P, _L, _I, _P, _Z, _P, _P]),
    "mlp_bwd_bf16": (C.c_int, [_P, _P, _P, _P, _P, _L, _I, _P, _Z, _P, _P]),
    "mlp_bwd_f16": (C.c_int, [_P, _P, _P, _P, _P, _L, _I, _P, _Z, _P, _P]),
    "forward_encoded": (C.c_int, [_P, _P, _P, _P, _L, _P, _P, _P]),
}
for _prefix in ("nf_bshape", "nf_cbshape"):
    _PROTOTYPES.update({f"{_prefix}_{_name}": _sig for _name, _sig in _FAMILY_ENTRY_POINTS.items()})
_SIGMA_SIG = (C.c_int, [_P, _P, _P, _P, _P, _P, _L, _I, _P, _P])
SIGMA_ENTRY_POINTS = tuple(f"{_prefix}_mlp_sigma{_suffix}" for _prefix in ("nf_paper", "nf_lcode", "nf_bshape", "nf_cbshape")
                           for _suffix in ("", "_bf16", "_f16", "_f16x2")) + ("nf_smaller_mlp_sigma",)
_PROTOTYPES.update({_name: _SIGMA_SIG for _name in SIGMA_ENTRY_POINTS})
_PROTOTYPES["nf_volume_weights_fwd"] = (C.c_int, [_P, _P, _P, _P, _L, _I, _P, _P, _P, _P])
_PROTOTYPES["nf_paper_mlp_fwd_live_scratch_floats"] = (_Z, [_I])
_PROTOTYPES["nf_paper_mlp_fwd_live"] = (C.c_int, [_P, _P, _P, _P, _P, _P, _L, _I, _P, _P, _Z, _I, _P])
_PROTOTYPES["nf_paper_mlp_fwd_live_stats"] = (C.c_int, [_P, _P, _P, _P, _P, _P, _L, _I, _P, _P, _Z, _I, _P, _Z, _P])
_PROTOTYPES["nf_paper_sigma_bound_floats"] = (_Z, [])
_PROTOTYPES["nf_paper_sigma_bound"] = (C.c_int, [_P, _P, _P])
_PROTOTYPES["nf_paper_mlp_fwd_gated"] = (C.c_int, [_P, _P, _P, _P, _P, _P, _P, _L, _I, _P, _P, _Z, _I, _P])
_PROTOTYPES["nf_paper_mlp_fwd_live_phases"] = _PROTOTYPES["nf_paper_mlp_fwd_live_stats"]
_PROTOTYPES["nf_paper_mlp_fwd_gated_stats"] = (C.c_int, [_P, _P, _P, _P, _P, _P, _P, _L, _I, _P, _P, _Z, _I, _P, _Z, _P])
_PROTOTYPES["nf_paper_mlp_fwd_gated_phases"] = _PROTOTYPES["nf_paper_mlp_fwd_gated_stats"]
_PROTOTYPES["nf_isosurface_workspace_bytes"] = (_Z, [_I, _I, _I])
_PROTOTYPES["nf_isosurface_count"] = (C.c_int, [_P, _I, _I, _I, _F, _P, _Z, _P, _P])
_PROTOTYPES["nf_isosurface_emit"] = (C.c_int, [_P, _I, _I, _I, _F, _P, _P, _P, _Z, _P, _L, _P, _L, _P, _P])
_PROTOTYPES["nf_isosurface_table"] = (C.c_int, [_P])
_PROTOTYPES["nf_sparse_grid_workspace_bytes"] = (_Z, [_I, _I, _I, _I])
_PROTOTYPES["nf_sparse_grid_lattice"] = (C.c_int, [_I, _I, _I, _I, _P, _P, _P, _P, _L, _P])
_PROTOTYPES["nf_sparse_grid_classify"] = (C.c_int, [_P, _I, _I, _I, _I, _F, _F, _I, _P, _Z, _P])
_PROTOTYPES["nf_sparse_grid_mark"] = (C.c_int, [_I, _I, _I, _I, _P, _Z, _P, _P])
_PROTOTYPES["nf_sparse_grid_emit"] = (C.c_int, [_P, _I, _I, _I, _I, _P, _P, _P, _Z, _P, _P, _L, _P])
_PROTOTYPES["nf_sparse_grid_scatter"] = (C.c_int, [_P, _P, _L, _P, _I, _I, _I, _P])
_PROTOTYPES["nf_mesh_components_workspace_bytes"] = (_Z, [_L, _L])
_PROTOTYPES["nf_mesh_components_label"] = (C.c_int, [_P, _L, _L, _P, _Z, _P, _P, _P, _P, _P, _P])
_PROTOTYPES["nf_mesh_components_select"] = (C.c_int, [_P, _P, _P, _L, _L, _I, _L, _P, _Z, _P, _P])
_PROTOTYPES["nf_mesh_components_emit"] = (C.c_int, [_P, _P, _P, _P, _P, _P, _L, _L, _P, _Z, _P, _L, _P, _L, _P, _P])
_PROTOTYPES["nf_mesh_smooth_workspace_bytes"] = (_Z, [_L, _L])
_PROTOTYPES["nf_mesh_smooth_adjacency"] = (C.c_int, [_P, _L, _L, _P, _Z, _P, _P, _P, _P, _P, _P])
_PROTOTYPES["nf_mesh_smooth_run"] = (C.c_int, [_P, _L, _P, _P, _P, _I, _F, _F, _P, _P, _P])
_PROTOTYPES["nf_mesh_smooth_normals"] = (C.c_int, [_P, _P, _L, _L, _P, _Z, _P, _P])
for _prefix in ("nf_lcode", "nf_bshape", "nf_cbshape"):
    _PROTOTYPES[f"{_prefix}_mlp_bwd_stage_ms"] = (C.c_int, [_P, _P, _I, _P, _P, _P, _L, _I, _P, _Z, _P, _P, _P])
_OPTIONAL = set()
ABI_VERSION = 5


def lib_path() -> str:
    return _LIB_PATH


def lib():
    global _lib
    if _lib is not None:
        return _lib
    with _lock:
        if _lib is not None:
            return _lib
        if not os.path.exists(_LIB_PATH):
            raise RuntimeError(
                f"libnerface_hip.so not found at {_LIB_PATH}: build it with `python 4d-facial-avatars_amd/build.py` "
                "(or __graft_entry__.build()).  This package has no CPU / PyTorch fallback.")
        handle = C.CDLL(_LIB_PATH, mode=C.RTLD_GLOBAL)
        for name, (res, args) in _PROTOTYPES.items():
            try:
                fn = getattr(handle, name)
            except AttributeError:
                if name in _OPTIONAL:
                    continue
                raise RuntimeError(f"libnerface_hip.so does not export {name}; rebuild it")
            fn.restype, fn.argtypes = res, args
        if handle.nf_abi_version() != ABI_VERSION:
            raise RuntimeError(f"libnerface_hip.so at {_LIB_PATH} has ABI revision {handle.nf_abi_version()}, this binding needs {ABI_VERSION}: "
                               "rebuild it (python 4d-facial-avatars_amd/build.py --force)")
        _lib = handle
    return _lib


def check(rc: int, what: str) -> None:
    if rc != 0:
        msg = lib().nf_error_string(rc)
        raise RuntimeError(f"{what} failed: {msg.decode() if msg else rc} (code {rc})")


def stream_ptr(device) -> int:
    return int(torch.cuda.current_stream(device).cuda_stream)


def require_device(*tensors) -> torch.device:
    dev = None
    for t in tensors:
        if t is None:
            continue
        if not t.is_cuda:
            raise RuntimeError("nerf (MI355X build): tensors must live on a ROCm device (`device='cuda'`); "
                               "there is no CPU path in this package")
        if t.dtype != torch.float32:
            raise RuntimeError(f"nerf (MI355X build): expected float32 tensors, got {t.dtype}")
        if not t.is_contiguous():
            raise RuntimeError("nerf (MI355X build): internal error, tensor is not contiguous")
        if dev is None:
            dev = t.device
        elif t.device != dev:
            raise RuntimeError("nerf (MI355X build): tensors are on different devices")
    return dev


def ptr(t) -> int:
    return 0 if t is None else int(t.data_ptr())
```

### 4d-facial-avatars_amd/nerf/ops.py

```python
from __future__ import annotations

import ctypes as C
import os
import weakref
from typing import NamedTuple, Optional, Sequence

import numpy as np
import torch

from . import _hip as H

PAPER_KEYS = (
    [f"layers_xyz.{i}.{p}" for i in range(6) for p in ("weight", "bias")]
    + [f"{n}.{p}" for n in ("fc_feat", "fc_alpha") for p in ("weight", "bias")]
    + [f"layers_dir.{i}.{p}" for i in range(4) for p in ("weight", "bias")]
    + [f"fc_rgb.{p}" for p in ("weight", "bias")]
)
LCODE_KEYS = [f"{n}.{p}" for n in ("layer1", "layers_xyz.0", "layers_xyz.1", "layers_xyz.2", "layers_dir.0", "fc_alpha", "fc_rgb", "fc_feat")
              for p in ("weight", "bias")]
SMALLER_KEYS = [f"{n}.{p}" for n in ([f"layers_xyz.{i}" for i in range(5)] + ["fc_feat", "fc_alpha"] + [f"layers_dir.{i}" for i in range(3)]
                                     + ["fc_rgb"]) for p in ("weight", "bias")]
BSHAPE_KEYS = list(LCODE_KEYS)
CBSHAPE_KEYS = [f"layers_expr.{i}.{p}" for i in range(3) for p in ("weight", "bias")] + LCODE_KEYS

# ... 64 lines not shown
    u = _c(u.reshape(-1))
    H.require_device(u)
    if u.numel() != n_items:
        raise ValueError("u must hold one uniform number per weight")
    lib = H.lib()
    ws_bytes = int(lib.nf_weighted_choice_workspace_bytes())
    ws = torch.empty(ws_bytes // 4, dtype=torch.int32, device=dev)
    idx = torch.empty(n, dtype=torch.int64, device=dev)
    with torch.cuda.device(dev):
        H.check(lib.nf_weighted_choice(H.ptr(w), H.ptr(u), n_items, int(n), H.ptr(idx), H.ptr(ws), ws_bytes, H.stream_ptr(dev)),
                "nf_weighted_choice")
    if check and n > 0 and int(ws[5].item()):
        raise ValueError("Fewer non-zero entries in p than size")
    return idx


class _SelectedBackground(torch.autograd.Function):

    @staticmethod
    def forward(ctx, background, sel, bg):
        ctx.save_for_backward(sel)
        ctx.hw = tuple(background.shape[:2])
        return bg.view_as(bg)

    @staticmethod
    def backward(ctx, g):
        (sel,) = ctx.saved_tensors
        h, w = ctx.hw
        row, col = (torch.div(sel, w, rounding_mode="floor"), sel % w) if sel.dim() == 1 else (sel[:, 0], sel[:, 1])
        ok = (row >= 0) & (row < h) & (col >= 0) & (col < w) if sel.dim() == 2 else (sel >= 0) & (sel < h * w)
        d = torch.zeros((h, w, 3), dtype=g.dtype, device=g.device)
        d.index_put_((row.clamp(0, h - 1), col.clamp(0, w - 1)), g * ok[:, None].to(g.dtype), accumulate=True)
        return d, None, None


def ray_batch(height: int, width: int, fx: float, fy: float, cx: float, cy: float, c2w: torch.Tensor, sel: torch.Tensor,
              image: Optional[torch.Tensor] = None, background: Optional[torch.Tensor] = None, check: bool = False):
    c2w = c2w if (c2w.dtype == torch.float32 and c2w.stride(-1) == 1) else c2w.to(torch.float32).contiguous()
    if sel.dtype != torch.int64 or not (sel.dim() == 1 or (sel.dim() == 2 and sel.shape[1] == 2)):
        raise ValueError("sel must be an (n, 2) int64 tensor of {row, col} or an (n,) int64 tensor of flat pixel indices")
    sel, image, background = sel.contiguous(), _c(image), _c(background)
    dev = H.require_device(c2w, image, background)
    if sel.device != dev:
        raise RuntimeError("ray_batch: select_inds must live on the device of the pose")
    n = int(sel.shape[0])
    if image is not None and (image.dim() != 3 or tuple(image.shape[:2]) != (height, width) or image.dtype != torch.float32):
        raise ValueError("image must be a float32 (H, W, C) tensor")
    if background is not None and (tuple(background.shape) != (height, width, 3) or background.dtype != torch.float32):
        raise ValueError("background must be a float32 (H, W, 3) tensor")
    ch = int(image.shape[2]) if image is not None else 0
    ro = torch.empty((n, 3), dtype=torch.float32, device=dev)
    rd = torch.empty((n, 3), dtype=torch.float32, device=dev)
    target = torch.empty((n, ch), dtype=torch.float32, device=dev) if image is not None else None
    bg = torch.empty((n, 3), dtype=torch.float32, device=dev) if background is not None else None
    flag = torch.zeros(1, dtype=torch.int32, device=dev)
    cx_w = float(np.float32(np.float64(width) * np.float64(cx)))
    cy_h = float(np.float32(np.float64(height) * np.float64(cy)))
    with torch.cuda.device(dev):
        H.check(H.lib().nf_ray_batch(height, width, float(np.float32(fx)), float(np.float32(fy)), cx_w, cy_h, H.ptr(c2w),
                                     int(c2w.stride(0)), H.ptr(sel), 1 if sel.dim() == 1 else 0, n, H.ptr(image), ch, H.ptr(background),
                                     H.ptr(ro), H.ptr(rd),
                                     H.ptr(target), H.ptr(bg), H.ptr(flag), H.stream_ptr(dev)), "nf_ray_batch")
    if check and int(flag.item()):
        raise IndexError("ray_batch: a selected pixel lies outside the image")
    if background is not None and background.requires_grad and torch.is_grad_enabled():
        bg = _SelectedBackground.apply(background, sel, bg)
    return ro, rd, target, bg


def sample_coarse(n_rays: int, n_coarse: int, near: float, far: float, device, t_rand: Optional[torch.Tensor] = None,
                  lindisp: bool = False):
    t_rand = _c(t_rand)
    tv = linspace01(n_coarse, device)
    z = torch.empty((n_rays, n_coarse), dtype=torch.float32, device=device)
    if t_rand is not None:
        H.require_device(t_rand)
        assert tuple(t_rand.shape) == (n_rays, n_coarse)
    with torch.cuda.device(device):
        H.check(H.lib().nf_sample_coarse_ex(n_rays, n_coarse, float(np.float32(near)), float(np.float32(far)), H.ptr(tv),
                                            H.ptr(t_rand), 1 if lindisp else 0, H.ptr(z), H.stream_ptr(device)), "nf_sample_coarse_ex")
    return z


def posenc(x: torch.Tensor, n_freq: int, include_input: bool) -> torch.Tensor:
    x = _c(x)
    dev = H.require_device(x)
    dim = x.shape[-1]
    rows = x.numel() // dim if dim else 0
    width = dim * ((1 if include_input else 0) + 2 * n_freq)
    out = torch.empty(tuple(x.shape[:-1]) + (width,), dtype=torch.float32, device=dev)
    with torch.cuda.device(dev):
        H.check(H.lib().nf_posenc(H.ptr(x), rows, dim, n_freq, 1 if include_input else 0, H.ptr(out), H.stream_ptr(dev)),
                "nf_posenc")
    return out


class MLPFamily(NamedTuple):
    prefix: str
    keys: tuple
    hidden: tuple
    none_grads: tuple
    exact_dw: bool
    precisions: tuple = _VALID_PRECISIONS

    def require_precision(self, precision: str) -> None:
        if precision not in self.precisions:
            raise NotImplementedError(f'the {self.prefix} model family has no "{precision}" kernels (it serves '
                                      f'{", ".join(repr(p) for p in self.precisions)}): use nerf.set_mlp_precision("f32")')

    def fn(self, name: str):
        return getattr(H.lib(), f"{self.prefix}_{name}")

    def call(self, name: str, *args) -> None:
        H.check(self.fn(name)(*args), f"{self.prefix}_{name}")


PAPER = MLPFamily("nf_paper", tuple(PAPER_KEYS),
                  (64, 2240),
                  (22, 23),
                  True)
LCODE = MLPFamily("nf_lcode", tuple(LCODE_KEYS),
                  (64, 1472),
                  (), False)
SMALLER = MLPFamily("nf_smaller", tuple(SMALLER_KEYS),
                    (64, 1984),
                    (), False,
                    ("f32",))

BSHAPE = MLPFamily("nf_bshape", tuple(BSHAPE_KEYS), LCODE.hidden, (), False)
CBSHAPE = MLPFamily("nf_cbshape", tuple(CBSHAPE_KEYS), LCODE.hidden, (), False)

_PACK_EPOCH = [0]


def bump_pack_epoch() -> None:
    _PACK_EPOCH[0] += 1


def pack_epoch() -> int:
    return _PACK_EPOCH[0]


class MLPWeights:

    _KINDS = {
        "f32": ("packed_floats", "pack", torch.float32),
        "f32_t": ("packed_bwd_floats", "pack_bwd", torch.float32),
        "bf16": ("packed_bf16_bytes", "pack_bf16", torch.uint8),
        "bf16_t": ("packed_bwd_bf16_bytes", "pack_bwd_bf16", torch.uint8),
        "f16": ("packed_f16_bytes", "pack_f16", torch.uint8),
        "f16_t": ("packed_bwd_f16_bytes", "pack_bwd_f16", torch.uint8),
    }

    def __init__(self, family: MLPFamily, params: Sequence[torch.Tensor]):
        assert len(params) == len(family.keys)
        self.family = family
        self._params = list(params)
        self._cache = {}
        self._f16_sticky = None

    def invalidate(self) -> None:
        for kind, (_, buf) in list(self._cache.items()):
            self._cache[kind] = (None, buf)

    def _signature(self):
        return (_PACK_EPOCH[0],) + tuple((int(p.data_ptr()), int(p._version)) for p in self._params)

    def _get(self, kind: str) -> torch.Tensor:
        sig = self._signature()
        hit = self._cache.get(kind)
        if hit is None or hit[0] != sig:
            size_fn, pack_fn, dtype = self._KINDS[kind]
            dev = H.require_device(*[p.detach() for p in self._params])
            buf = hit[1] if hit is not None and hit[1].device == dev else torch.empty(self.family.fn(size_fn)(), dtype=dtype, device=dev)
            if kind == "f16" and hit is not None and hit[1] is buf:
                if self._f16_sticky is None or self._f16_sticky.device != dev:
                    self._f16_sticky = torch.zeros((), dtype=torch.int32, device=dev)
                off = self.family.fn("f16_flag_offset")()
                self._f16_sticky.bitwise_or_(buf[off:off + 4].view(torch.int32)[0])
            arr = (C.c_void_p * len(self._params))(*[int(p.data_ptr()) for p in self._params])
            with torch.cuda.device(dev):
                self.family.call(pack_fn, arr, H.ptr(buf), H.stream_ptr(dev))
            self._cache[kind] = (sig, buf)
        return self._cache[kind][1]

    def get(self) -> torch.Tensor:
        return self._get("f32")

    def get_bound(self) -> torch.Tensor:
        packed = self._get("f32")
        sig = self._cache["f32"][0]
        hit = self._cache.get("bound")
        if hit is None or hit[0] != sig or hit[1].device != packed.device:
            self._cache["bound"] = hit = (sig, sigma_bound(self.family, packed))
        return hit[1]

    def get_t(self) -> torch.Tensor:
        return self._get("f32_t")

    def get_bf16(self) -> torch.Tensor:
        return self._get("bf16")

    def get_bf16_t(self) -> torch.Tensor:
        return self._get("bf16_t")

    def get_f16(self) -> torch.Tensor:
        return self._get("f16")

    def get_f16_t(self) -> torch.Tensor:
        return self._get("f16_t")

    def f16_range_flag(self) -> Optional[torch.Tensor]:
        hit = self._cache.get("f16")
        if hit is None:
            return None
        off = self.family.fn("f16_flag_offset")()
        flag = hit[1][off:off + 4].view(torch.int32)[0]
        return flag if self._f16_sticky is None else torch.bitwise_or(flag, self._f16_sticky)


def check_conditioning(expr: torch.Tensor, latent: torch.Tensor) -> None:
    if expr.numel() != 76 or latent.numel() != 32:
        raise ValueError("expected a 76-d expression and a 32-d latent code")


def mlp_condition(fam: MLPFamily, packed, expr, latent, near: float, far: float) -> torch.Tensor:
    expr, latent = _c(expr.detach()), _c(latent.detach())
    dev = H.require_device(packed, expr, latent)
    check_conditioning(expr, latent)
    cond = torch.empty(fam.fn("cond_floats")(), dtype=torch.float32, device=dev)
    with torch.cuda.device(dev):
        fam.call("condition", H.ptr(packed), H.ptr(expr), H.ptr(latent), float(np.float32(near)), float(np.float32(far)), H.ptr(cond),
                 H.stream_ptr(dev))
    return cond


_FWD_ENTRY = {"f32": "mlp_fwd", "bf16x3": "mlp_fwd_bf16", "f16x3": "mlp_fwd_f16", "f16x2": "mlp_fwd_f16x2"}


def mlp_fwd(fam: MLPFamily, precision: str, packed, cond, ro, rd, z, rd_view=None) -> torch.Tensor:
    dev = H.require_device(packed if precision == "f32" else None, cond, ro, rd, z, rd_view)
    n_rays, n_samples = z.shape
    raw = torch.empty((n_rays, n_samples, 4), dtype=torch.float32, device=dev)
    with torch.cuda.device(dev):
        fam.call(_FWD_ENTRY[precision], H.ptr(packed), H.ptr(cond), H.ptr(ro), H.ptr(rd), H.ptr(rd_view), H.ptr(z), n_rays, n_samples,
                 H.ptr(raw), H.stream_ptr(dev))
    return raw


LIVE_FAMILIES = ("nf_paper",)
LIVE_PASSES_DEFAULT = ("coarse", "fine")
_live_passes = set(LIVE_PASSES_DEFAULT)
_live_launches = [0]
_LIVE_SCRATCH = {}
LIVE_RING_ROWS = 64
LIVE_ROW_BYTES = 1024 + 64 + 16
LIVE_PREFETCH_ROWS = 8


def live_rotation_step(workgroups: int) -> int:
    step = (workgroups * 5 // 13) | 1
    return step if step < workgroups else 0


def set_live_colour(on, passes=("coarse", "fine")) -> None:
    global _live_passes, _gated_passes
    _live_passes = set(LIVE_PASSES_DEFAULT) if on is None else (set(passes) if on else set())
    _gated_passes = set(GATED_PASSES_DEFAULT) if on is None else set()


def live_colour_kernel(fam: MLPFamily) -> bool:
    return _mlp_precision == "f32" and fam.prefix in LIVE_FAMILIES


def live_colour_applies(fam: MLPFamily, which: str) -> bool:
    return which in _live_passes and live_colour_kernel(fam)


def live_colour_launches() -> int:
    return _live_launches[0]


def mlp_fwd_live(fam: MLPFamily, packed, cond, ro, rd, z, rd_view=None, max_workgroups: int = 0) -> torch.Tensor:
    if fam.prefix not in LIVE_FAMILIES:
        raise NotImplementedError(f"the {fam.prefix} model family has no live-colour kernel")
    dev = H.require_device(packed, cond, ro, rd, z, rd_view)
    n_rays, n_samples = z.shape
    raw = torch.empty((n_rays, n_samples, 4), dtype=torch.float32, device=dev)
    with torch.cuda.device(dev):
        key = (dev, H.stream_ptr(dev), int(max_workgroups))
        scratch = _LIVE_SCRATCH.get(key)
        if scratch is None:
            scratch = _LIVE_SCRATCH[key] = torch.empty(fam.fn("mlp_fwd_live_scratch_floats")(int(max_workgroups)), dtype=torch.float32, device=dev)
        fam.call("mlp_fwd_live", H.ptr(packed), H.ptr(cond), H.ptr(ro), H.ptr(rd), H.ptr(rd_view), H.ptr(z), n_rays, n_samples, H.ptr(raw),
                 H.ptr(scratch), scratch.numel(), int(max_workgroups), H.stream_ptr(dev))
    _live_launches[0] += 1
    return raw


LIVE_PHASE_COLUMNS = ("clk_trunk", "clk_lone_tile", "clk_append", "clk_run_entry", "clk_run", "clk_dead_stores")
LIVE_STAT_COLUMNS = ("units", "colour_runs", "flush_rows", "exit_clock") + LIVE_PHASE_COLUMNS


def mlp_fwd_live_stats(fam: MLPFamily, packed, cond, ro, rd, z, rd_view=None, max_workgroups: int = 0):
    if fam.prefix not in LIVE_FAMILIES:
        raise NotImplementedError(f"the {fam.prefix} model family has no live-colour kernel")
    dev = H.require_device(packed, cond, ro, rd, z, rd_view)
    n_rays, n_samples = z.shape
    raw = torch.empty((n_rays, n_samples, 4), dtype=torch.float32, device=dev)
    with torch.cuda.device(dev):
        scratch = torch.empty(fam.fn("mlp_fwd_live_scratch_floats")(int(max_workgroups)), dtype=torch.float32, device=dev)
        waves = scratch.numel() * 4 // (LIVE_RING_ROWS * LIVE_ROW_BYTES)
        stats = torch.empty((waves, len(LIVE_STAT_COLUMNS)), dtype=torch.int64, device=dev)
        fam.call("mlp_fwd_live_phases", H.ptr(packed), H.ptr(cond), H.ptr(ro), H.ptr(rd), H.ptr(rd_view), H.ptr(z), n_rays, n_samples,
                 H.ptr(raw), H.ptr(scratch), scratch.numel(), int(max_workgroups), stats.data_ptr(), waves, H.stream_ptr(dev))
    return raw, stats


GATED_PASSES_DEFAULT = ("coarse", "fine")
_gated_passes = (set(GATED_PASSES_DEFAULT) if os.environ.get("NERFACE_SIGMA_GATE") is None
                 else {p for p in os.environ["NERFACE_SIGMA_GATE"].split(",") if p in ("coarse", "fine")})
_gated_launches = [0]
GATED_STAT_COLUMNS = LIVE_STAT_COLUMNS[:4] + ("proven_rows",) + LIVE_PHASE_COLUMNS


def set_sigma_gate(on, passes=("coarse", "fine")) -> None:
    global _gated_passes
    _gated_passes = set(GATED_PASSES_DEFAULT) if on is None else (set(passes) if on else set())


def sigma_gate_applies(fam: MLPFamily, which: str) -> bool:
    return which in _gated_passes and live_colour_kernel(fam)


def live_mode(fam: MLPFamily, which: str):
    if sigma_gate_applies(fam, which):
        return "gated"
    return live_colour_applies(fam, which)


def sigma_gate_launches() -> int:
    return _gated_launches[0]


def sigma_bound(fam: MLPFamily, packed) -> torch.Tensor:
    if fam.prefix not in LIVE_FAMILIES:
        raise NotImplementedError(f"the {fam.prefix} model family has no gated kernel")
    dev = H.require_device(packed)
    bound = torch.empty(fam.fn("sigma_bound_floats")(), dtype=torch.float32, device=dev)
    with torch.cuda.device(dev):
        fam.call("sigma_bound", H.ptr(packed), H.ptr(bound), H.stream_ptr(dev))
    return bound


def _gated_call(entry, fam, packed, bound, cond, ro, rd, z, rd_view, max_workgroups, scratch, raw, *tail):
    n_rays, n_samples = z.shape
    fam.call(entry, H.ptr(packed), H.ptr(bound), H.ptr(cond), H.ptr(ro), H.ptr(rd), H.ptr(rd_view), H.ptr(z), n_rays, n_samples, H.ptr(raw),
             H.ptr(scratch), scratch.numel(), int(max_workgroups), *tail)


def mlp_fwd_gated(fam: MLPFamily, packed, bound, cond, ro, rd, z, rd_view=None, max_workgroups: int = 0) -> torch.Tensor:
    if fam.prefix not in LIVE_FAMILIES:
        raise NotImplementedError(f"the {fam.prefix} model family has no gated kernel")
    dev = H.require_device(packed, bound, cond, ro, rd, z, rd_view)
    n_rays, n_samples = z.shape
    raw = torch.empty((n_rays, n_samples, 4), dtype=torch.float32, device=dev)
    with torch.cuda.device(dev):
        key = (dev, H.stream_ptr(dev), int(max_workgroups))
        scratch = _LIVE_SCRATCH.get(key)
        if scratch is None:
            scratch = _LIVE_SCRATCH[key] = torch.empty(fam.fn("mlp_fwd_live_scratch_floats")(int(max_workgroups)), dtype=torch.float32, device=dev)
        _gated_call("mlp_fwd_gated", fam, packed, bound, cond, ro, rd, z, rd_view, max_workgroups, scratch, raw, H.stream_ptr(dev))
    _gated_launches[0] += 1
    return raw


def mlp_fwd_gated_stats(fam: MLPFamily, packed, bound, cond, ro, rd, z, rd_view=None, max_workgroups: int = 0):
    if fam.prefix not in LIVE_FAMILIES:
        raise NotImplementedError(f"the {fam.prefix} model family has no gated kernel")
    dev = H.require_device(packed, bound, cond, ro, rd, z, rd_view)
    n_rays, n_samples = z.shape
    raw = torch.empty((n_rays, n_samples, 4), dtype=torch.float32, device=dev)
    with torch.cuda.device(dev):
        scratch = torch.empty(fam.fn("mlp_fwd_live_scratch_floats")(int(max_workgroups)), dtype=torch.float32, device=dev)
        waves = scratch.numel() * 4 // (LIVE_RING_ROWS * LIVE_ROW_BYTES)
        stats = torch.empty((waves, len(GATED_STAT_COLUMNS)), dtype=torch.int64, device=dev)
        _gated_call("mlp_fwd_gated_phases", fam, packed, bound, cond, ro, rd, z, rd_view, max_workgroups, scratch, raw, stats.data_ptr(), waves,
                    H.stream_ptr(dev))
    return raw, stats


_SIGMA_ENTRY = {"f32": "mlp_sigma", "bf16x3": "mlp_sigma_bf16", "f16x3": "mlp_sigma_f16", "f16x2": "mlp_sigma_f16x2"}


def mlp_sigma(fam: MLPFamily, precision: str, image, cond, ro, rd, z) -> torch.Tensor:
    dev = H.require_device(image if precision == "f32" else None, cond, ro, rd, z)
    n_rays, n_samples = z.shape
    sigma = torch.empty((n_rays, n_samples), dtype=torch.float32, device=dev)
    with torch.cuda.device(dev):
        fam.call(_SIGMA_ENTRY[precision], H.ptr(image), H.ptr(cond), H.ptr(ro), H.ptr(rd), 0, H.ptr(z), n_rays, n_samples, H.ptr(sigma),
                 H.stream_ptr(dev))
    return sigma


def mlp_fwd_train(fam: MLPFamily, packed, cond, ro, rd, z, rd_view=None, packed_b=None, packed_h=None):
    dev = H.require_device(packed, cond, ro, rd, z, rd_view)
    n_rays, n_samples = z.shape
    raw = torch.empty((n_rays, n_samples, 4), dtype=torch.float32, device=dev)
    saved = torch.empty(fam.fn("saved_floats")(n_rays * n_samples), dtype=torch.float32, device=dev)
    entry, image = (("mlp_fwd_train_f16", packed_h) if packed_h is not None else
                    ("mlp_fwd_train_bf16", packed_b) if packed_b is not None else ("mlp_fwd_train", packed))
    with torch.cuda.device(dev):
        fam.call(entry, H.ptr(image), H.ptr(cond), H.ptr(ro), H.ptr(rd), H.ptr(rd_view), H.ptr(z), n_rays, n_samples, H.ptr(raw),
                 H.ptr(saved), H.stream_ptr(dev))
    return raw, (saved,)


def mlp_bwd(fam: MLPFamily, weights: MLPWeights, packed, cond, z, d_raw, saved_t, split=False, exact_dw=False):
    if exact_dw and not fam.exact_dw:
        raise ValueError(f"exact_dw: the split-bf16 backward of {fam.prefix} has no exact-f32 weight-gradient form")
    d_raw = _c(d_raw)
    dev = H.require_device(packed, cond, saved_t, d_raw)
    n_rays, n_samples = z.shape
    with torch.cuda.device(dev):
        ws_floats = fam.fn("bwd_workspace_floats")(n_rays * n_samples)
    ws = torch.empty(ws_floats, dtype=torch.float32, device=dev)
    flat = torch.empty(fam.fn("grad_floats")(), dtype=torch.float32, device=dev)
    args = (H.ptr(cond), H.ptr(saved_t), H.ptr(d_raw), n_rays, n_samples, H.ptr(ws), ws_floats, H.ptr(flat))
    with torch.cuda.device(dev):
        if split == "f16":
            fam.call("mlp_bwd_f16", H.ptr(packed), H.ptr(weights.get_f16_t()), *args, H.stream_ptr(dev))
        elif split:
            packed_bt, exact = weights.get_bf16_t(), ()
            if fam.exact_dw:
                saved_f32 = split_saved_to_f32(saved_t, n_rays * n_samples, False) if exact_dw else None
                exact = (int(bool(exact_dw)), H.ptr(saved_f32))
            fam.call("mlp_bwd_bf16", H.ptr(packed), H.ptr(packed_bt), *args, *exact, H.stream_ptr(dev))
        else:
            fam.call("mlp_bwd", H.ptr(packed), H.ptr(weights.get_t()), *args, H.stream_ptr(dev))
    grads, off = [], 0
    for i, p in enumerate(weights._params):
        n = p.numel()
        grads.append(None if i in fam.none_grads else flat[off:off + n].view(p.shape))
        off += n
    return grads, flat[off:off + 32]


def mlp_forward_encoded(weights: MLPWeights, x, expr, latent) -> torch.Tensor:
    x = _c(x.detach())
    if x.dim() != 2 or x.shape[1] != 87:
        raise ValueError("expected pre-encoded inputs of shape (N, 87)")
    expr, latent = _c(expr.detach()).reshape(-1), _c(latent.detach()).reshape(-1)
    check_conditioning(expr, latent)
    packed = weights.get()
    dev = H.require_device(packed, x, expr, latent)
    fam = weights.family
    cond = torch.empty(fam.fn("cond_floats")(), dtype=torch.float32, device=dev)
    out = torch.empty((x.shape[0], 4), dtype=torch.float32, device=dev)
    with torch.cuda.device(dev):
        fam.call("forward_encoded", H.ptr(packed), H.ptr(x), H.ptr(expr), H.ptr(latent), x.shape[0], H.ptr(cond), H.ptr(out),
                 H.stream_ptr(dev))
    return out


def paper_condition(packed: torch.Tensor, expr: torch.Tensor, latent: torch.Tensor, near: float, far: float) -> torch.Tensor:
    return mlp_condition(PAPER, packed, expr, latent, near, far)


def paper_mlp_fwd(packed, cond, ro, rd, z, rd_view=None) -> torch.Tensor:
    return mlp_fwd(PAPER, "f32", packed, cond, ro, rd, z, rd_view)


def paper_mlp_fwd_bf16(packed_b, cond, ro, rd, z, rd_view=None) -> torch.Tensor:
    return mlp_fwd(PAPER, "bf16x3", packed_b, cond, ro, rd, z, rd_view)


def paper_mlp_fwd_f16(packed_h, cond, ro, rd, z, rd_view=None) -> torch.Tensor:
    return mlp_fwd(PAPER, "f16x3", packed_h, cond, ro, rd, z, rd_view)


def paper_mlp_fwd_f16x2(packed_h, cond, ro, rd, z, rd_view=None) -> torch.Tensor:
    return mlp_fwd(PAPER, "f16x2", packed_h, cond, ro, rd, z, rd_view)


def paper_mlp_fwd_train(packed, cond, ro, rd, z, rd_view=None, packed_b=None, packed_h=None):
    return mlp_fwd_train(PAPER, packed, cond, ro, rd, z, rd_view, packed_b=packed_b, packed_h=packed_h)


def paper_mlp_bwd(model, packed, cond, z, d_raw, saved, split=False, exact_dw=False):
    (saved_t,) = saved
    return mlp_bwd(PAPER, model.hip_weights(), packed, cond, z, d_raw, saved_t, split=split, exact_dw=exact_dw)


def split_saved_to_f32(saved_t: torch.Tensor, n_points: int, f16: bool, family: str = "paper") -> torch.Tensor:
    fam = LCODE if family == "lcode" else PAPER
    dev = H.require_device(saved_t)
    out = torch.empty(fam.fn("saved_floats")(n_points), dtype=torch.float32, device=dev)
    with torch.cuda.device(dev):
        H.check(H.lib().nf_split_saved_to_f32(int(fam is LCODE), H.ptr(saved_t), n_points, int(bool(f16)), H.ptr(out), H.stream_ptr(dev)),
                "nf_split_saved_to_f32")
    return out


def require_trainable_precision() -> None:
    if _mlp_precision in INFERENCE_ONLY_PRECISIONS:
        raise RuntimeError(f'nerf.set_mlp_precision("{_mlp_precision}") is an inference arithmetic: train with "f32", "f16x3" or "bf16x3"')


_f16_train_probe_every = [128]


def set_f16_train_probe_every(n: int) -> None:
    _f16_train_probe_every[0] = max(1, int(n))


def f16_train_probe_every() -> int:
    return _f16_train_probe_every[0]


F16_ACT_LIMIT = 65504.0 / 16.0
F16_PREFLIGHT_MARGIN = 4.0


def f16_preflight(model, ro, rd, z, rd_view, expr, latent, near, far, max_rays: int = 256, max_samples: int = 8) -> float:
    n_rays, n_s = z.shape
    rs = max(1, n_rays // max_rays)
    ss = max(1, n_s // max_samples)
    ro_s, rd_s = ro[::rs].contiguous(), rd[::rs].contiguous()
    z_s = z[::rs, ::ss].contiguous()
    rv_s = None if rd_view is None else rd_view[::rs].contiguous()
    hw = model.hip_weights()
    packed = hw.get()
    cond = mlp_condition(hw.family, packed, expr, latent, near, far)
    _, (saved,) = mlp_fwd_train(hw.family, packed, cond, ro_s, rd_s, z_s, rv_s)
    lo, hi = hw.family.hidden
    n = z_s.numel()
    return float(saved[lo * n:hi * n].abs().max().item())


def f16_guard(model, ro, rd, z, rd_view, expr, latent, near, far, training: bool) -> None:
    state = model.__dict__
    if training and torch.cuda.is_current_stream_capturing():
        return
    if training:
        n_calls = state["_f16_train_calls"] = state.get("_f16_train_calls", 0) + 1
        if not (_f16_train_probe_every[0] == 1 or n_calls % _f16_train_probe_every[0] == 1):
            return
    else:
        key = (model.hip_weights()._signature()[1:], expr.data_ptr(), latent.data_ptr(), expr._version, latent._version)
        if state.get("_f16_probe_key") == key:
            return
    amax = f16_preflight(model, ro, rd, z, rd_view, expr, latent, near, far)
    if not amax * F16_PREFLIGHT_MARGIN < F16_ACT_LIMIT:
        where, use = (", ", "train") if training else (" on a sample of this frame, ", "render")
        raise RuntimeError(f'nerf.set_mlp_precision("{_mlp_precision}"): hidden activations of {type(model).__name__} reach {amax:.3g}{where}'
                           f'within {F16_PREFLIGHT_MARGIN:g}x of the fp16 range limit ({F16_ACT_LIMIT:g}) -- {use} this model with "f32" or "bf16x3"')
    if not training:
        state["_f16_probe_key"] = key


def check_f16_range(*models, sync_ranks: bool = False) -> None:
    flags = [m.hip_weights().f16_range_flag() for m in models if m is not None and hasattr(m, "hip_weights")]
    flags = [f for f in flags if f is not None]
    if not flags:
        return
    total = torch.stack(flags).sum().to(torch.int32).reshape(1)
    if sync_ranks:
        import torch.distributed as dist
        if dist.is_available() and dist.is_initialized() and dist.get_world_size() > 1:
            dist.all_reduce(total, op=dist.ReduceOp.MAX)
    if int(total.item()) != 0:
        raise RuntimeError(f'nerf.set_mlp_precision("{_mlp_precision}"): an activation left the fp16 range (|x| >= 4094) and a density output is '
                           'not finite -- render this model with "f32" or "bf16x3"')


MAX_BINS = 512
MAX_SORT = 1024
MAX_BWD_SAMPLES = 1024


def _refuse(what: str, got: str, limit: str) -> None:
    raise ValueError(f"{what}: {got} exceeds {limit} (csrc/nf_render.hip); there is no kernel for this size")


def check_resample_sizes(n_coarse: int, n_fine: int, what: str = "resample_merge") -> None:
    if n_coarse - 1 > MAX_BINS:
        _refuse(what, f"{n_coarse} coarse samples ({n_coarse - 1} bins)", f"the sampler's table limit NF_MAX_BINS = {MAX_BINS}")
    if n_coarse + n_fine > MAX_SORT:
        _refuse(what, f"{n_coarse} + {n_fine} = {n_coarse + n_fine} samples per ray", f"the row-sort limit NF_MAX_SORT = {MAX_SORT}")


def check_bwd_samples(n_samples: int, what: str = "volume_render_bwd") -> None:
    if n_samples > MAX_BWD_SAMPLES:
        _refuse(what, f"{n_samples} samples per ray",
                f"the integrator backward's limit of NF_MAX_CHUNKS = {MAX_BWD_SAMPLES // 64} chunks of 64 = {MAX_BWD_SAMPLES}")


def check_sample_counts(n_coarse: int, n_fine: int, need_grad: bool) -> None:
    if n_fine > 0:
        check_resample_sizes(n_coarse, n_fine, "run_one_iter_of_nerf (num_coarse + num_fine)")
    if need_grad:
        check_bwd_samples(n_coarse + max(n_fine, 0), "run_one_iter_of_nerf (training step)")


def volume_render_fwd(raw, z, rd, noise=None, bg=None, white_background=False):
    dev = H.require_device(raw, z, rd, noise, bg)
    n_rays, n_samples = z.shape
    rgb = torch.empty((n_rays, 3), dtype=torch.float32, device=dev)
    disp = torch.empty((n_rays,), dtype=torch.float32, device=dev)
    acc = torch.empty((n_rays,), dtype=torch.float32, device=dev)
    w = torch.empty((n_rays, n_samples), dtype=torch.float32, device=dev)
    with torch.cuda.device(dev):
        H.check(H.lib().nf_volume_render_fwd(H.ptr(raw), H.ptr(z), H.ptr(rd), H.ptr(noise), H.ptr(bg), n_rays, n_samples,
                                             1 if white_background else 0, H.ptr(rgb), H.ptr(disp), H.ptr(acc), H.ptr(w),
                                             H.stream_ptr(dev)), "nf_volume_render_fwd")
    return rgb, disp, acc, w


def volume_weights_fwd(sigma, z, rd, noise=None):
    dev = H.require_device(sigma, z, rd, noise)
    n_rays, n_samples = z.shape
    disp = torch.empty((n_rays,), dtype=torch.float32, device=dev)
    acc = torch.empty((n_rays,), dtype=torch.float32, device=dev)
    w = torch.empty((n_rays, n_samples), dtype=torch.float32, device=dev)
    with torch.cuda.device(dev):
        H.check(H.lib().nf_volume_weights_fwd(H.ptr(sigma), H.ptr(z), H.ptr(rd), H.ptr(noise), n_rays, n_samples, H.ptr(disp), H.ptr(acc),
                                              H.ptr(w), H.stream_ptr(dev)), "nf_volume_weights_fwd")
    return disp, acc, w


def volume_render_bwd(raw, z, rd, noise, bg, d_rgb, white_background=False):
    d_rgb = _c(d_rgb)
    dev = H.require_device(raw, z, rd, noise, bg, d_rgb)
    n_rays, n_samples = z.shape
    check_bwd_samples(n_samples)
    d_raw = torch.empty((n_rays, n_samples, 4), dtype=torch.float32, device=dev)
    with torch.cuda.device(dev):
        H.check(H.lib().nf_volume_render_bwd(H.ptr(raw), H.ptr(z), H.ptr(rd), H.ptr(noise), H.ptr(bg), H.ptr(d_rgb), n_rays,
                                             n_samples, 1 if white_background else 0, H.ptr(d_raw), H.stream_ptr(dev)),
                "nf_volume_render_bwd")
    return d_raw


def _cotangent(name: str, t, shape, what: str):
    if t is None:
        return None
    if not torch.is_tensor(t) or tuple(t.shape) != tuple(shape):
        got = tuple(t.shape) if torch.is_tensor(t) else type(t).__name__
        raise ValueError(f"{what}: {name} must have shape {tuple(shape)}, got {got}")
    if t.dtype != torch.float32:
        raise ValueError(f"{what}: {name} must be float32, got {t.dtype}")
    return t if t.is_contiguous() else t.contiguous()


def volume_render_bwd_full(raw, z, rd, noise, bg, d_rgb=None, d_disp=None, d_acc=None, d_weights=None, d_w_last=None,
                           white_background=False, need_d_bg=False):
    what = "volume_render_bwd_full"
    n_rays, n_samples = z.shape
    d_rgb = _cotangent("d_rgb", d_rgb, (n_rays, 3), what)
    d_disp = _cotangent("d_disp", d_disp, (n_rays,), what)
    d_acc = _cotangent("d_acc", d_acc, (n_rays,), what)
    d_weights = _cotangent("d_weights", d_weights, (n_rays, n_samples), what)
    d_w_last = _cotangent("d_w_last", d_w_last, (n_rays,), what)
    if d_rgb is None and d_disp is None and d_acc is None and d_weights is None and d_w_last is None:
        raise ValueError(f"{what}: no cotangent given (d_rgb, d_disp, d_acc, d_weights and d_w_last are all None)")
    if need_d_bg and bg is None:
        raise ValueError(f"{what}: need_d_bg without a background prior (bg is None)")
    check_bwd_samples(n_samples, what)
    dev = H.require_device(raw, z, rd, noise, bg, d_rgb, d_disp, d_acc, d_weights, d_w_last)
    d_raw = torch.empty((n_rays, n_samples, 4), dtype=torch.float32, device=dev)
    d_bg = torch.empty((n_rays, 3), dtype=torch.float32, device=dev) if need_d_bg else None
    with torch.cuda.device(dev):
        H.check(H.lib().nf_volume_render_bwd_full(H.ptr(raw), H.ptr(z), H.ptr(rd), H.ptr(noise), H.ptr(bg), H.ptr(d_rgb), H.ptr(d_disp),
                                                  H.ptr(d_acc), H.ptr(d_weights), H.ptr(d_w_last), n_rays, n_samples,
                                                  1 if white_background else 0, H.ptr(d_raw), H.ptr(d_bg), H.stream_ptr(dev)),
                "nf_volume_render_bwd_full")
    return d_raw, d_bg


def render_volume_density(raw, depth):
    dev = H.require_device(raw, depth)
    n_rays, n_samples = depth.shape
    rgb = torch.empty((n_rays, 3), dtype=torch.float32, device=dev)
    dmap = torch.empty((n_rays,), dtype=torch.float32, device=dev)
    acc = torch.empty((n_rays,), dtype=torch.float32, device=dev)
    with torch.cuda.device(dev):
        H.check(H.lib().nf_render_volume_density(H.ptr(raw), H.ptr(depth), n_rays, n_samples, H.ptr(rgb), H.ptr(dmap), H.ptr(acc),
                                                 H.stream_ptr(dev)), "nf_render_volume_density")
    return rgb, dmap, acc

# ... 595 lines not shown
```

### include/nerface_hip.h

```cpp
#ifndef NERFACE_HIP_H
#define NERFACE_HIP_H

#include <stddef.h>
#include <stdint.h>

#ifdef __cplusplus
extern "C" {
#endif

typedef void* nf_stream_t;

#define NF_EINVAL (-22)

int         nf_abi_version(void);
const char* nf_error_string(int code);
const char* nf_build_info(void);

int nf_ray_bundle(int height, int width, float fx, float fy, float cx_w, float cy_h,
                  const float* c2w, int c2w_row_stride, float* ro, float* rd, nf_stream_t stream);

int nf_ray_batch(int height, int width, float fx, float fy, float cx_w, float cy_h, const float* c2w, int c2w_row_stride,
                 const int64_t* sel, int sel_is_flat, int64_t n, const float* image, int channels, const float* bg, float* ro,
                 float* rd, float* target, float* bg_out, int* bad_flag, nf_stream_t stream);

// ... 86 lines not shown
int nf_lcode_condition(const float* packed, const float* expr76, const float* latent32, float near_z, float far_z,
                       float* cond, nf_stream_t stream);
int nf_lcode_mlp_fwd(const float* packed, const float* cond, const float* ro, const float* rd, const float* rd_view,
                     const float* z, int64_t n_rays, int n_samples, float* raw, nf_stream_t stream);
int nf_lcode_forward_encoded(const float* packed, const float* x87, const float* expr76, const float* latent32,
                             int64_t n_points, float* cond, float* out, nf_stream_t stream);
size_t nf_lcode_packed_bf16_bytes(void);
int nf_lcode_pack_bf16(const float* const* params, void* packed_bf16, nf_stream_t stream);
int nf_lcode_mlp_fwd_bf16(const void* packed_bf16, const float* cond, const float* ro, const float* rd,
                          const float* rd_view, const float* z, int64_t n_rays, int n_samples, float* raw,
                          nf_stream_t stream);
size_t nf_lcode_packed_f16_bytes(void);
size_t nf_lcode_f16_flag_offset(void);
int nf_lcode_pack_f16(const float* const* params, void* stream_out, nf_stream_t stream);
int nf_lcode_mlp_fwd_f16(const void* packed_f16, const float* cond, const float* ro, const float* rd, const float* rd_view,
                         const float* z, int64_t n_rays, int n_samples, float* raw, nf_stream_t stream);
int nf_lcode_mlp_fwd_f16x2(const void* packed_f16, const float* cond, const float* ro, const float* rd, const float* rd_view,
                           const float* z, int64_t n_rays, int n_samples, float* raw, nf_stream_t stream);
int nf_lcode_mlp_fwd_train_f16(const void* packed_f16, const float* cond, const float* ro, const float* rd, const float* rd_view,
                               const float* z, int64_t n_rays, int n_samples, float* raw, float* saved, nf_stream_t stream);
size_t nf_lcode_packed_bwd_f16_bytes(void);
int nf_lcode_pack_bwd_f16(const float* const* params, void* stream_out, nf_stream_t stream);
int nf_lcode_mlp_bwd_f16(const float* packed, const void* packed_t_f16, const float* cond, const float* saved, const float* d_raw,
                         int64_t n_rays, int n_samples, float* workspace, size_t workspace_floats, float* grads, nf_stream_t stream);

size_t nf_lcode_saved_floats(int64_t n_points);
int nf_lcode_mlp_fwd_train(const float* packed, const float* cond, const float* ro, const float* rd, const float* rd_view,
                           const float* z, int64_t n_rays, int n_samples, float* raw, float* saved, nf_stream_t stream);
size_t nf_lcode_packed_bwd_floats(void);
int nf_lcode_pack_bwd(const float* const* params, float* packed_t, nf_stream_t stream);
size_t nf_lcode_grad_floats(void);
size_t nf_lcode_bwd_workspace_floats(int64_t n_points);
int nf_lcode_mlp_bwd(const float* packed, const float* packed_t, const float* cond, const float* saved, const float* d_raw,
                     int64_t n_rays, int n_samples, float* workspace, size_t workspace_floats, float* grads,
                     nf_stream_t stream);

int nf_lcode_mlp_fwd_train_bf16(const void* packed_bf16, const float* cond, const float* ro, const float* rd,
                                const float* rd_view, const float* z, int64_t n_rays, int n_samples, float* raw,
                                float* saved, nf_stream_t stream);
size_t nf_lcode_packed_bwd_bf16_bytes(void);
int nf_lcode_pack_bwd_bf16(const float* const* params, void* packed_t_bf16, nf_stream_t stream);
int nf_lcode_mlp_bwd_bf16(const float* packed, const void* packed_t_bf16, const float* cond, const float* saved,
                          const float* d_raw, int64_t n_rays, int n_samples, float* workspace, size_t workspace_floats,
                          float* grads, nf_stream_t stream);

size_t nf_bshape_packed_floats(void);
size_t nf_bshape_cond_floats(void);
int nf_bshape_pack(const float* const* params, float* packed, nf_stream_t stream);
int nf_bshape_condition(const float* packed, const float* expr76, const float* latent32, float near_z, float far_z, float* cond,
                    nf_stream_t stream);
int nf_bshape_mlp_fwd(const float* packed, const float* cond, const float* ro, const float* rd, const float* rd_view, const float* z,
                  int64_t n_rays, int n_samples, float* raw, nf_stream_t stream);
int nf_bshape_forward_encoded(const float* packed, const float* x87, const float* expr76, const float* latent32, int64_t n_points,
                          float* cond, float* out, nf_stream_t stream);
size_t nf_bshape_packed_bf16_bytes(void);
int nf_bshape_pack_bf16(const float* const* params, void* packed_bf16, nf_stream_t stream);
int nf_bshape_mlp_fwd_bf16(const void* packed_bf16, const float* cond, const float* ro, const float* rd, const float* rd_view,
                       const float* z, int64_t n_rays, int n_samples, float* raw, nf_stream_t stream);
size_t nf_bshape_packed_f16_bytes(void);
size_t nf_bshape_f16_flag_offset(void);
int nf_bshape_pack_f16(const float* const* params, void* stream_out, nf_stream_t stream);
int nf_bshape_mlp_fwd_f16(const void* packed_f16, const float* cond, const float* ro, const float* rd, const float* rd_view,
                      const float* z, int64_t n_rays, int n_samples, float* raw, nf_stream_t stream);
int nf_bshape_mlp_fwd_f16x2(const void* packed_f16, const float* cond, const float* ro, const float* rd, const float* rd_view,
                        const float* z, int64_t n_rays, int n_samples, float* raw, nf_stream_t stream);
size_t nf_bshape_saved_floats(int64_t n_points);
int nf_bshape_mlp_fwd_train(const float* packed, const float* cond, const float* ro, const float* rd, const float* rd_view,
                        const float* z, int64_t n_rays, int n_samples, float* raw, float* saved, nf_stream_t stream);
int nf_bshape_mlp_fwd_train_bf16(const void* packed_bf16, const float* cond, const float* ro, const float* rd, const float* rd_view,
                             const float* z, int64_t n_rays, int n_samples, float* raw, float* saved, nf_stream_t stream);
int nf_bshape_mlp_fwd_train_f16(const void* packed_f16, const float* cond, const float* ro, const float* rd, const float* rd_view,
                            const float* z, int64_t n_rays, int n_samples, float* raw, float* saved, nf_stream_t stream);
size_t nf_bshape_packed_bwd_floats(void);
int nf_bshape_pack_bwd(const float* const* params, float* packed_t, nf_stream_t stream);
size_t nf_bshape_packed_bwd_bf16_bytes(void);
int nf_bshape_pack_bwd_bf16(const float* const* params, void* packed_t_bf16, nf_stream_t stream);
size_t nf_bshape_packed_bwd_f16_bytes(void);
int nf_bshape_pack_bwd_f16(const float* const* params, void* stream_out, nf_stream_t stream);
size_t nf_bshape_grad_floats(void);
size_t nf_bshape_bwd_workspace_floats(int64_t n_points);
int nf_bshape_mlp_bwd(const float* packed, const float* packed_t, const float* cond, const float* saved, const float* d_raw,
                  int64_t n_rays, int n_samples, float* workspace, size_t workspace_floats, float* grads, nf_stream_t stream);
int nf_bshape_mlp_bwd_bf16(const float* packed, const void* packed_t_bf16, const float* cond, const float* saved, const float* d_raw,
                       int64_t n_rays, int n_samples, float* workspace, size_t workspace_floats, float* grads, nf_stream_t stream);
int nf_bshape_mlp_bwd_f16(const float* packed, const void* packed_t_f16, const float* cond, const float* saved, const float* d_raw,
                      int64_t n_rays, int n_samples, float* workspace, size_t workspace_floats, float* grads, nf_stream_t stream);

size_t nf_cbshape_packed_floats(void);
size_t nf_cbshape_cond_floats(void);
int nf_cbshape_pack(const float* const* params, float* packed, nf_stream_t stream);
int nf_cbshape_condition(const float* packed, const float* expr76, const float* latent32, float near_z, float far_z, float* cond,
                    nf_stream_t stream);
int nf_cbshape_mlp_fwd(const float* packed, const float* cond, const float* ro, const float* rd, const float* rd_view, const float* z,
                  int64_t n_rays, int n_samples, float* raw, nf_stream_t stream);
int nf_cbshape_forward_encoded(const float* packed, const float* x87, const float* expr76, const float* latent32, int64_t n_points,
                          float* cond, float* out, nf_stream_t stream);
size_t nf_cbshape_packed_bf16_bytes(void);
int nf_cbshape_pack_bf16(const float* const* params, void* packed_bf16, nf_stream_t stream);
int nf_cbshape_mlp_fwd_bf16(const void* packed_bf16, const float* cond, const float* ro, const float* rd, const float* rd_view,
                       const float* z, int64_t n_rays, int n_samples, float* raw, nf_stream_t stream);
size_t nf_cbshape_packed_f16_bytes(void);
size_t nf_cbshape_f16_flag_offset(void);
int nf_cbshape_pack_f16(const float* const* params, void* stream_out, nf_stream_t stream);
int nf_cbshape_mlp_fwd_f16(const void* packed_f16, const float* cond, const float* ro, const float* rd, const float* rd_view,
                      const float* z, int64_t n_rays, int n_samples, float* raw, nf_stream_t stream);
int nf_cbshape_mlp_fwd_f16x2(const void* packed_f16, const float* cond, const float* ro, const float* rd, const float* rd_view,
                        const float* z, int64_t n_rays, int n_samples, float* raw, nf_stream_t stream);
size_t nf_cbshape_saved_floats(int64_t n_points);
int nf_cbshape_mlp_fwd_train(const float* packed, const float* cond, const float* ro, const float* rd, const float* rd_view,
                        const float* z, int64_t n_rays, int n_samples, float* raw, float* saved, nf_stream_t stream);
int nf_cbshape_mlp_fwd_train_bf16(const void* packed_bf16, const float* cond, const float* ro, const float* rd, const float* rd_view,
                             const float* z, int64_t n_rays, int n_samples, float* raw, float* saved, nf_stream_t stream);
int nf_cbshape_mlp_fwd_train_f16(const void* packed_f16, const float* cond, const float* ro, const float* rd, const float* rd_view,
                            const float* z, int64_t n_rays, int n_samples, float* raw, float* saved, nf_stream_t stream);
size_t nf_cbshape_packed_bwd_floats(void);
int nf_cbshape_pack_bwd(const float* const* params, float* packed_t, nf_stream_t stream);
size_t nf_cbshape_packed_bwd_bf16_bytes(void);
int nf_cbshape_pack_bwd_bf16(const float* const* params, void* packed_t_bf16, nf_stream_t stream);
size_t nf_cbshape_packed_bwd_f16_bytes(void);
int nf_cbshape_pack_bwd_f16(const float* const* params, void* stream_out, nf_stream_t stream);
size_t nf_cbshape_grad_floats(void);
size_t nf_cbshape_bwd_workspace_floats(int64_t n_points);
int nf_cbshape_mlp_bwd(const float* packed, const float* packed_t, const float* cond, const float* saved, const float* d_raw,
                  int64_t n_rays, int n_samples, float* workspace, size_t workspace_floats, float* grads, nf_stream_t stream);
int nf_cbshape_mlp_bwd_bf16(const float* packed, const void* packed_t_bf16, const float* cond, const float* saved, const float* d_raw,
                       int64_t n_rays, int n_samples, float* workspace, size_t workspace_floats, float* grads, nf_stream_t stream);
int nf_cbshape_mlp_bwd_f16(const float* packed, const void* packed_t_f16, const float* cond, const float* saved, const float* d_raw,
                      int64_t n_rays, int n_samples, float* workspace, size_t workspace_floats, float* grads, nf_stream_t stream);

int nf_lcode_mlp_bwd_stage_ms(const float* packed, const void* packed_t_any, int precision, const float* cond, const float* saved,
                              const float* d_raw, int64_t n_rays, int n_samples, float* workspace, size_t workspace_floats,
                              float* grads, float* stage_ms, nf_stream_t stream);
int nf_bshape_mlp_bwd_stage_ms(const float* packed, const void* packed_t_any, int precision, const float* cond, const float* saved,
                               const float* d_raw, int64_t n_rays, int n_samples, float* workspace, size_t workspace_floats,
                               float* grads, float* stage_ms, nf_stream_t stream);
int nf_cbshape_mlp_bwd_stage_ms(const float* packed, const void* packed_t_any, int precision, const float* cond, const float* saved,
                                const float* d_raw, int64_t n_rays, int n_samples, float* workspace, size_t workspace_floats,
                                float* grads, float* stage_ms, nf_stream_t stream);

size_t nf_smaller_packed_floats(void);
size_t nf_smaller_cond_floats(void);
int nf_smaller_gather_table(uint32_t* out, size_t n );
int nf_smaller_pack(const float* const* params, float* packed, nf_stream_t stream);
int nf_smaller_condition(const float* packed, const float* expr76, const float* latent32, float near_z, float far_z,
                         float* cond, nf_stream_t stream);
int nf_smaller_mlp_fwd(const float* packed, const float* cond, const float* ro, const float* rd, const float* rd_view,
                       const float* z, int64_t n_rays, int n_samples, float* raw, nf_stream_t stream);
int nf_smaller_forward_encoded(const float* packed, const float* x87, const float* expr76, const float* latent32,
                               int64_t n_points, float* cond, float* out, nf_stream_t stream);
size_t nf_smaller_saved_floats(int64_t n_points);
int nf_smaller_mlp_fwd_train(const float* packed, const float* cond, const float* ro, const float* rd, const float* rd_view,
                             const float* z, int64_t n_rays, int n_samples, float* raw, float* saved, nf_stream_t stream);
size_t nf_smaller_packed_bwd_floats(void);
int nf_smaller_pack_bwd(const float* const* params, float* packed_t, nf_stream_t stream);
size_t nf_smaller_grad_floats(void);
size_t nf_smaller_bwd_workspace_floats(int64_t n_points);
int nf_smaller_mlp_bwd(const float* packed, const float* packed_t, const float* cond, const float* saved, const float* d_raw,
                       int64_t n_rays, int n_samples, float* workspace, size_t workspace_floats, float* grads,
                       nf_stream_t stream);
int nf_smaller_mlp_bwd_stage_ms(const float* packed, const float* packed_t, const float* cond, const float* saved,
                                const float* d_raw, int64_t n_rays, int n_samples, float* workspace, size_t workspace_floats,
                                float* grads, float* stage_ms, nf_stream_t stream);

size_t nf_tiny_packed_floats(void);
int nf_tiny_pack(const float* const* params, float* packed, nf_stream_t stream);
int nf_tiny_mlp_fwd(const float* packed, const float* ro, const float* rd, const float* depth, int depth_per_ray,
                    int64_t n_rays, int n_samples, float* raw, nf_stream_t stream);
int nf_render_volume_density(const float* raw, const float* depth, int64_t n_rays, int n_samples, float* rgb,
                             float* depth_map, float* acc, nf_stream_t stream);

size_t nf_tiny_saved_floats(int64_t n_points);
int nf_tiny_mlp_fwd_train(const float* packed, const float* ro, const float* rd, const float* depth, int depth_per_ray,
                          int64_t n_rays, int n_samples, float* raw, float* saved, nf_stream_t stream);
int nf_render_volume_density_bwd(const float* raw, const float* depth, const float* d_rgb, int64_t n_rays, int n_samples,
                                 float* d_raw, nf_stream_t stream);
int nf_render_volume_density_bwd_full(const float* raw, const float* depth, const float* d_rgb, const float* d_depth,
                                      const float* d_acc, int64_t n_rays, int n_samples, float* d_raw, nf_stream_t stream);
size_t nf_tiny_packed_bwd_floats(void);
int nf_tiny_pack_bwd(const float* const* params, float* packed_t, nf_stream_t stream);
size_t nf_tiny_grad_floats(void);
size_t nf_tiny_bwd_workspace_floats(int64_t n_points);
int nf_tiny_mlp_bwd(const float* packed_t, const float* saved, const float* d_raw, int64_t n_rays, int n_samples,
                    float* workspace, size_t workspace_floats, float* grads, nf_stream_t stream);

size_t nf_flex_packed_floats(int num_layers);
int nf_flex_pack(int num_layers, const float* const* params, float* packed, nf_stream_t stream);
int nf_flex_mlp_fwd(int num_layers, const float* packed, const float* ro, const float* rd, const float* depth, int depth_per_ray,
                    int64_t n_rays, int n_samples, float* raw, nf_stream_t stream);
size_t nf_flex_saved_floats(int num_layers, int64_t n_points);
int nf_flex_mlp_fwd_train(int num_layers, const float* packed, const float* ro, const float* rd, const float* depth,
                          int depth_per_ray, int64_t n_rays, int n_samples, float* raw, float* saved, nf_stream_t stream);
size_t nf_flex_packed_bwd_floats(int num_layers);
int nf_flex_pack_bwd(int num_layers, const float* const* params, float* packed_t, nf_stream_t stream);
size_t nf_flex_grad_floats(int num_layers);
size_t nf_flex_bwd_workspace_floats(int num_layers, int64_t n_points);
int nf_flex_mlp_bwd(int num_layers, const float* packed_t, const float* saved, const float* d_raw, int64_t n_rays, int n_samples,
                    float* workspace, size_t workspace_floats, float* grads, nf_stream_t stream);

int nf_eval_postprocess(const float* rgb, const float* depthmap, const float* weights, int height, int width, float fx,
                        float fy, float cx_w, float cy_h, uint8_t* rgb_u8, uint8_t* normals_u8, nf_stream_t stream);

size_t nf_image_metrics_workspace_bytes(int64_t n, int height, int width);
int nf_image_metrics(const uint8_t* a, const uint8_t* b, int64_t n, int height, int width, double ssim_range, void* workspace,
                     size_t workspace_bytes, double* out_f64, int64_t* out_i64, nf_stream_t stream);

int nf_sample_pdf(const float* bins, const float* weights, const float* u, int64_t u_row_stride,
                  int64_t n_rays, int n_bins, int n_out, float* samples, nf_stream_t stream);
int nf_sample_pdf_ex(const float* bins, const float* weights, const float* u, int64_t u_row_stride, int64_t n_rays,
                     int n_bins, int n_out, float* samples, int* inds, float* cdf, nf_stream_t stream);

int nf_resample_merge(const float* z_coarse, const float* w_coarse, const float* u, int64_t u_row_stride,
                      int64_t n_rays, int n_coarse, int n_fine, float* z_samples ,
                      float* z_fine , nf_stream_t stream);

size_t nf_render_rays_workspace_floats(int64_t n_rays, int n_coarse, int n_fine);
int nf_render_rays_fwd(const float* packed_coarse, const void* packed_bf16_coarse, const float* packed_fine,
                       const void* packed_bf16_fine, const float* expr76, const float* latent32, const float* ro,
                       const float* rd, const float* rd_view, const float* bg, const float* t_vals, const float* t_rand,
                       const float* u, int64_t u_row_stride, const float* noise_coarse, const float* noise_fine,
                       int64_t n_rays, int n_coarse, int n_fine, float near_z, float far_z, int white_background,
                       float* workspace, size_t workspace_floats, float* rgb_coarse, float* disp_coarse, float* acc_coarse,
                       float* rgb_fine, float* disp_fine, float* acc_fine, float* w_last, nf_stream_t stream);

int nf_render_rays_fwd_f16(const float* packed_coarse, const void* packed_f16_coarse, const float* packed_fine,
                           const void* packed_f16_fine, const float* expr76, const float* latent32, const float* ro,
                           const float* rd, const float* rd_view, const float* bg, const float* t_vals, const float* t_rand,
                           const float* u, int64_t u_row_stride, const float* noise_coarse, const float* noise_fine,
                           int64_t n_rays, int n_coarse, int n_fine, float near_z, float far_z, int white_background,
                           float* workspace, size_t workspace_floats, float* rgb_coarse, float* disp_coarse, float* acc_coarse,
                           float* rgb_fine, float* disp_fine, float* acc_fine, float* w_last, nf_stream_t stream);

int nf_render_rays_fwd_f16x2(const float* packed_coarse, const void* packed_f16_coarse, const float* packed_fine,
                             const void* packed_f16_fine, const float* expr76, const float* latent32, const float* ro,
                             const float* rd, const float* rd_view, const float* bg, const float* t_vals, const float* t_rand,
                             const float* u, int64_t u_row_stride, const float* noise_coarse, const float* noise_fine,
                             int64_t n_rays, int n_coarse, int n_fine, float near_z, float far_z, int white_background,
                             float* workspace, size_t workspace_floats, float* rgb_coarse, float* disp_coarse, float* acc_coarse,
                             float* rgb_fine, float* disp_fine, float* acc_fine, float* w_last, nf_stream_t stream);

int nf_adam_step(float* const* params, const float* const* grads, float* const* exp_avg, float* const* exp_avg_sq,
                 const int64_t* numel, int n_tensors, float lr, float beta1, float beta2, float eps, int64_t step,
                 nf_stream_t stream);

int nf_train_loss_fwd(const float* rgb_coarse, const float* rgb_fine, const float* target, int64_t n_elems, const float* latent,
                      int n_latent, float code_weight, float code_scale, float* out7, nf_stream_t stream);
int nf_train_loss_bwd(const float* rgb_coarse, const float* rgb_fine, const float* target, int64_t n_elems, const float* latent,
                      int n_latent, float code_weight, float code_scale, const float* out7, const float* grad_out,
                      float* d_rgb_coarse, float* d_rgb_fine, float* d_latent, nf_stream_t stream);

int nf_adam_step_dev(float* const* params, const float* const* grads, float* const* exp_avg, float* const* exp_avg_sq,
                     const int64_t* numel, int n_tensors, float beta1, float beta2, float eps, void* state, nf_stream_t stream);
int nf_train_loss_bg_fwd(const float* rgb_coarse, const float* rgb_fine, const float* target, int64_t n_elems, const float* latent,
                         int n_latent, float code_weight, float code_scale, const float* bg, const float* w_last, float bg_weight,
                         float* out8, nf_stream_t stream);
int nf_train_loss_bg_bwd(const float* rgb_coarse, const float* rgb_fine, const float* target, int64_t n_elems, const float* latent,
                         int n_latent, float code_weight, float code_scale, const float* bg, const float* w_last, float bg_weight,
                         const float* out8, const float* grad_out, float* d_rgb_coarse, float* d_rgb_fine, float* d_latent,
                         float* d_bg, float* d_w_last, nf_stream_t stream);

int nf_sort_rows(const float* in, int64_t n_rows, int n_cols, float* out, nf_stream_t stream);

#define NF_DECLARE_MLP_SIGMA(PFX)                                                                                                   \
    int PFX##_mlp_sigma(const float* packed, const float* cond, const float* ro, const float* rd, const float* rd_view,            \
                        const float* z, int64_t n_rays, int n_samples, float* sigma, nf_stream_t stream);
#define NF_DECLARE_MLP_SIGMA_SPLIT(PFX)                                                                                             \
    int PFX##_mlp_sigma_bf16(const void* packed_bf16, const float* cond, const float* ro, const float* rd, const float* rd_view,   \
                             const float* z, int64_t n_rays, int n_samples, float* sigma, nf_stream_t stream);                     \
    int PFX##_mlp_sigma_f16(const void* packed_f16, const float* cond, const float* ro, const float* rd, const float* rd_view,     \
                            const float* z, int64_t n_rays, int n_samples, float* sigma, nf_stream_t stream);                      \
    int PFX##_mlp_sigma_f16x2(const void* packed_f16, const float* cond, const float* ro, const float* rd, const float* rd_view,   \
                              const float* z, int64_t n_rays, int n_samples, float* sigma, nf_stream_t stream);
NF_DECLARE_MLP_SIGMA(nf_paper) NF_DECLARE_MLP_SIGMA_SPLIT(nf_paper)
NF_DECLARE_MLP_SIGMA(nf_lcode) NF_DECLARE_MLP_SIGMA_SPLIT(nf_lcode)
NF_DECLARE_MLP_SIGMA(nf_bshape) NF_DECLARE_MLP_SIGMA_SPLIT(nf_bshape)
NF_DECLARE_MLP_SIGMA(nf_cbshape) NF_DECLARE_MLP_SIGMA_SPLIT(nf_cbshape)
NF_DECLARE_MLP_SIGMA(nf_smaller)
#undef NF_DECLARE_MLP_SIGMA
#undef NF_DECLARE_MLP_SIGMA_SPLIT
int nf_volume_weights_fwd(const float* sigma, const float* z, const float* rd, const float* noise, int64_t n_rays, int n_samples,
                          float* disp, float* acc, float* weights, nf_stream_t stream);

size_t nf_paper_mlp_fwd_live_scratch_floats(int max_workgroups);
int nf_paper_mlp_fwd_live(const float* packed, const float* cond, const float* ro, const float* rd, const float* rd_view,
                          const float* z, int64_t n_rays, int n_samples, float* raw, float* scratch, size_t scratch_floats,
                          int max_workgroups, nf_stream_t stream);
int nf_paper_mlp_fwd_live_phases(const float* packed, const float* cond, const float* ro, const float* rd, const float* rd_view,
                                 const float* z, int64_t n_rays, int n_samples, float* raw, float* scratch, size_t scratch_floats,
                                 int max_workgroups, int64_t* stats, size_t stats_rows, nf_stream_t stream);
int nf_paper_mlp_fwd_live_stats(const float* packed, const float* cond, const float* ro, const float* rd, const float* rd_view,
                                const float* z, int64_t n_rays, int n_samples, float* raw, float* scratch, size_t scratch_floats,
                                int max_workgroups, int64_t* stats, size_t stats_rows, nf_stream_t stream);

int nf_paper_mlp_fwd_gated_phases(const float* packed, const float* bound, const float* cond, const float* ro, const float* rd,
                                  const float* rd_view, const float* z, int64_t n_rays, int n_samples, float* raw, float* scratch,
                                  size_t scratch_floats, int max_workgroups, int64_t* stats, size_t stats_rows, nf_stream_t stream);
size_t nf_paper_sigma_bound_floats(void);
int nf_paper_sigma_bound(const float* packed, float* bound, nf_stream_t stream);
int nf_paper_mlp_fwd_gated(const float* packed, const float* bound, const float* cond, const float* ro, const float* rd,
                           const float* rd_view, const float* z, int64_t n_rays, int n_samples, float* raw, float* scratch,
                           size_t scratch_floats, int max_workgroups, nf_stream_t stream);
int nf_paper_mlp_fwd_gated_stats(const float* packed, const float* bound, const float* cond, const float* ro, const float* rd,
                                 const float* rd_view, const float* z, int64_t n_rays, int n_samples, float* raw, float* scratch,
                                 size_t scratch_floats, int max_workgroups, int64_t* stats, size_t stats_rows, nf_stream_t stream);

size_t nf_isosurface_workspace_bytes(int nx, int ny, int nz);
int nf_isosurface_count(const float* grid, int nx, int ny, int nz, float level, void* workspace, size_t workspace_bytes,
                        int64_t* counts_dev, nf_stream_t stream);
int nf_isosurface_emit(const float* grid, int nx, int ny, int nz, float level, const float* lo, const float* hi, void* workspace,
                       size_t workspace_bytes, float* verts, int64_t n_verts, int* faces, int64_t n_faces, float* normals,
                       nf_stream_t stream);
int nf_isosurface_table(uint32_t* out);

size_t nf_sparse_grid_workspace_bytes(int nx, int ny, int nz, int brick);
int nf_sparse_grid_lattice(int nx, int ny, int nz, int brick, const float* lo, const float* hi, int* index, float* coords,
                           int64_t capacity, nf_stream_t stream);
int nf_sparse_grid_classify(const float* grid, int nx, int ny, int nz, int brick, float level, float margin, int dilate,
                            void* workspace, size_t workspace_bytes, nf_stream_t stream);
int nf_sparse_grid_mark(int nx, int ny, int nz, int brick, void* workspace, size_t workspace_bytes, int64_t* counts_dev,
                        nf_stream_t stream);
int nf_sparse_grid_emit(float* grid, int nx, int ny, int nz, int brick, const float* lo, const float* hi, void* workspace,
                        size_t workspace_bytes, int* index, float* coords, int64_t capacity, nf_stream_t stream);
int nf_sparse_grid_scatter(const float* values, const int* index, int64_t count, float* grid, int nx, int ny, int nz,
                           nf_stream_t stream);

size_t nf_mesh_components_workspace_bytes(int64_t n_vertices, int64_t n_faces);
int nf_mesh_components_label(const int* faces, int64_t n_vertices, int64_t n_faces, void* workspace, size_t workspace_bytes,
                             int* vertex_label, int* face_label, int* face_counts, int* vertex_counts, int64_t* counts_dev,
                             nf_stream_t stream);
int nf_mesh_components_select(const int* vertex_label, const int* face_label, const int* face_counts, int64_t n_vertices,
                              int64_t n_faces, int largest, int64_t min_faces, void* workspace, size_t workspace_bytes,
                              int64_t* counts_dev, nf_stream_t stream);
int nf_mesh_components_emit(const float* vertices, const int* faces, const float* normals, const int* vertex_label,
                            const int* face_label, const int* face_counts, int64_t n_vertices, int64_t n_faces, void* workspace,
                            size_t workspace_bytes, float* out_vertices, int64_t cap_vertices, int* out_faces, int64_t cap_faces,
                            float* out_normals, nf_stream_t stream);

size_t nf_mesh_smooth_workspace_bytes(int64_t n_vertices, int64_t n_faces);
int nf_mesh_smooth_adjacency(const int* faces, int64_t n_vertices, int64_t n_faces, void* workspace, size_t workspace_bytes,
                             int* row_start, int* neighbours, int* multiplicity, uint8_t* boundary, int64_t* counts_dev,
                             nf_stream_t stream);
int nf_mesh_smooth_run(const float* vertices, int64_t n_vertices, const int* row_start, const int* neighbours, const uint8_t* pinned,
                       int iterations, float lam, float mu, float* tmp, float* out, nf_stream_t stream);
int nf_mesh_smooth_normals(const float* vertices, const int* faces, int64_t n_vertices, int64_t n_faces, void* workspace,
                           size_t workspace_bytes, float* normals, nf_stream_t stream);

int nf_selftest_dw_tables_f32(void);
int nf_selftest_dw_tables_lcode_f32(void);
int nf_selftest_dw_tables_smaller_f32(void);
int nf_selftest_dw_tables_bf16(void);
int nf_selftest_dw_tables_tiny(void);
int nf_selftest_dw_tables_flex(int num_layers);
long nf_paper_stream_table_bf16(uint32_t* out, size_t n_entries);
long nf_paper_stream_table_bwd_bf16(uint32_t* out, size_t n_entries);
long nf_lcode_stream_table_bf16(uint32_t* out, size_t n_entries);
long nf_lcode_stream_table_bwd_bf16(uint32_t* out, size_t n_entries);

#ifdef __cplusplus
}
#endif
#endif
```

Baseline: 622,300 rays/s.

## Prefetch next unit's z and first-layer weights ahead of the trunk head

Restructures the start of each work unit in the live/gated MLP kernel. The next unit's z samples are loaded early, during the first layer of the current unit. The first-layer bias and weights are loaded alongside the ray inputs, and the first PE layer double-buffers its weight chunks. Ray index math switches to 32-bit division when the point count fits. New head-phase clock instrumentation entry points are added; this raises register pressure in exchange for hiding load latency at unit entry.

After: 625,600 rays/s (median of 6 runs). Within noise of the previous version (+0.5%).

```diff
diff --git a/4d-facial-avatars_amd/csrc/nf_live_index.h b/4d-facial-avatars_amd/csrc/nf_live_index.h
--- /dev/null
+++ b/4d-facial-avatars_amd/csrc/nf_live_index.h
@@ -0,0 +1,16 @@
+#pragma once
+#include <stdint.h>
+
+#if defined(__HIPCC__) || defined(__CUDACC__)
+#define NF_IDX_HD __host__ __device__ __forceinline__
+#else
+#define NF_IDX_HD inline
+#endif
+
+NF_IDX_HD bool nf_idx_narrow(int64_t n_points) { return n_points < ((int64_t)1 << 31); }
+
+NF_IDX_HD uint32_t nf_idx_ray32(uint32_t p, uint32_t S) { return p / S; }
+NF_IDX_HD bool nf_idx_last32(uint32_t p, uint32_t S) { return (p + 1u) % S == 0u; }
+
+NF_IDX_HD int64_t nf_idx_ray64(int64_t p, int S) { return p / S; }
+NF_IDX_HD bool nf_idx_last64(int64_t p, int S) { return (p + 1) % S == 0; }
diff --git a/4d-facial-avatars_amd/csrc/nf_mlp_gated_stats.hip b/4d-facial-avatars_amd/csrc/nf_mlp_gated_stats.hip
--- a/4d-facial-avatars_amd/csrc/nf_mlp_gated_stats.hip
+++ b/4d-facial-avatars_amd/csrc/nf_mlp_gated_stats.hip
@@ -1,11 +1,11 @@
 #include "nf_mlp_live_kernel.h"
 
-static int nf_gated_stats_launch(bool clocks, const float* packed, const float* bound, const float* cond, const float* ro, const float* rd,
+static int nf_gated_stats_launch(int clocks, const float* packed, const float* bound, const float* cond, const float* ro, const float* rd,
                                  const float* rd_view, const float* z, int64_t n_rays, int n_samples, float* raw, float* scratch,
                                  size_t scratch_floats, int max_workgroups, int64_t* stats, size_t stats_rows, nf_stream_t stream) {
     static_assert(sizeof(long long) == sizeof(int64_t), "a statistics row is int64s");
     if (max_workgroups < 0 || !stats || ((uintptr_t)stats & 7) || stats_rows < (size_t)nf_live_grid_cap(max_workgroups) * NF_MLP_WAVES) return NF_EINVAL;
-    const size_t cols = NF_GATE_STAT_COLS + (clocks ? NF_LIVE_PHASES : 0);
+    const size_t cols = NF_GATE_STAT_COLS + (clocks ? NF_LIVE_PHASES : 0) + (clocks == 2 ? NF_LIVE_HEAD_PHASES : 0);
     const hipError_t e = hipMemsetAsync(stats, 0, stats_rows * cols * sizeof(int64_t), nf_s(stream));
     if (e != hipSuccess) return (int)e;
     return nf_live_launch<true, true>(packed, cond, ro, rd, rd_view, z, n_rays, n_samples, raw, scratch, scratch_floats, max_workgroups,
@@ -15,13 +15,20 @@
 extern "C" int nf_paper_mlp_fwd_gated_stats(const float* packed, const float* bound, const float* cond, const float* ro, const float* rd,
                                             const float* rd_view, const float* z, int64_t n_rays, int n_samples, float* raw, float* scratch,
                                             size_t scratch_floats, int max_workgroups, int64_t* stats, size_t stats_rows, nf_stream_t stream) {
-    return nf_gated_stats_launch(false, packed, bound, cond, ro, rd, rd_view, z, n_rays, n_samples, raw, scratch, scratch_floats, max_workgroups,
+    return nf_gated_stats_launch(0, packed, bound, cond, ro, rd, rd_view, z, n_rays, n_samples, raw, scratch, scratch_floats, max_workgroups,
                                  stats, stats_rows, stream);
 }
 
 extern "C" int nf_paper_mlp_fwd_gated_phases(const float* packed, const float* bound, const float* cond, const float* ro, const float* rd,
                                              const float* rd_view, const float* z, int64_t n_rays, int n_samples, float* raw, float* scratch,
                                              size_t scratch_floats, int max_workgroups, int64_t* stats, size_t stats_rows, nf_stream_t stream) {
-    return nf_gated_stats_launch(true, packed, bound, cond, ro, rd, rd_view, z, n_rays, n_samples, raw, scratch, scratch_floats, max_workgroups,
+    return nf_gated_stats_launch(1, packed, bound, cond, ro, rd, rd_view, z, n_rays, n_samples, raw, scratch, scratch_floats, max_workgroups,
                                  stats, stats_rows, stream);
 }
+
+extern "C" int nf_paper_mlp_fwd_gated_head(const float* packed, const float* bound, const float* cond, const float* ro, const float* rd,
+                                           const float* rd_view, const float* z, int64_t n_rays, int n_samples, float* raw, float* scratch,
+                                           size_t scratch_floats, int max_workgroups, int64_t* stats, size_t stats_rows, nf_stream_t stream) {
+    return nf_gated_stats_launch(2, packed, bound, cond, ro, rd, rd_view, z, n_rays, n_samples, raw, scratch, scratch_floats, max_workgroups,
+                                 stats, stats_rows, stream);
+}
diff --git a/4d-facial-avatars_amd/csrc/nf_mlp_live_kernel.h b/4d-facial-avatars_amd/csrc/nf_mlp_live_kernel.h
--- a/4d-facial-avatars_amd/csrc/nf_mlp_live_kernel.h
+++ b/4d-facial-avatars_amd/csrc/nf_mlp_live_kernel.h
@@ -1,6 +1,7 @@
 #pragma once
 #include <mutex>
 #include "nf_mlp_paper_net.h"
+#include "nf_live_index.h"
 
 #define NF_LIVE_ROWS 64
 #ifndef NF_LIVE_PF
@@ -101,13 +102,19 @@
 #define NF_LIVE_PH_RUN 4
 #define NF_LIVE_PH_DEAD 5
 #define NF_LIVE_PHASES 6
+#define NF_LIVE_PH_H_LOAD 6
+#define NF_LIVE_PH_H_PE 7
+#define NF_LIVE_PH_H_WAIT 8
+#define NF_LIVE_PH_H_L0 9
+#define NF_LIVE_PH_H_REST 10
+#define NF_LIVE_HEAD_PHASES 5
 #define NF_LIVE_STAT_COLS 4
 #define NF_GATE_STAT_COLS 5
 
 template <bool STATS, int COLS = NF_LIVE_STAT_COLS>
 __device__ __forceinline__ void nf_live_stat(long long* stats, int col, long long add, bool set = false) {
     if constexpr (STATS) {
-        const int cols = COLS + (((uintptr_t)stats & 1) ? NF_LIVE_PHASES : 0);
+        const int cols = COLS + (((uintptr_t)stats & 1) ? NF_LIVE_PHASES : 0) + (((uintptr_t)stats & 2) ? NF_LIVE_HEAD_PHASES : 0);
         stats = reinterpret_cast<long long*>((uintptr_t)stats & ~(uintptr_t)7);
         if ((threadIdx.x & 63) == 0) {
             long long* at = stats + ((size_t)blockIdx.x * NF_MLP_WAVES + (threadIdx.x >> 6)) * cols + col;
@@ -117,15 +124,19 @@
     }
 }
 
-template <bool STATS, int COLS>
-__device__ __forceinline__ void nf_live_mark(long long* stats, int end, int start) {
+template <bool STATS, int COLS, bool HEAD = false>
+__device__ __forceinline__ void nf_live_mark(long long* stats, int end, int start, int arrived = -1) {
     if constexpr (STATS) {
-        if ((uintptr_t)stats & 1) {
+        if constexpr (HEAD) asm volatile("" : "+s"(stats));
+        if ((uintptr_t)stats & (HEAD ? 2 : 1)) {
             __builtin_amdgcn_sched_barrier(0);
+            if (HEAD && arrived == 0) __builtin_amdgcn_s_waitcnt(0x0F70);
+            if (HEAD && arrived == 32) __builtin_amdgcn_s_waitcnt(0x8F70);
             const long long t = (long long)__builtin_amdgcn_s_memtime();
             if ((threadIdx.x & 63) == 0) {
+                const int cols = COLS + NF_LIVE_PHASES + (((uintptr_t)stats & 2) ? NF_LIVE_HEAD_PHASES : 0);
                 long long* row = reinterpret_cast<long long*>((uintptr_t)stats & ~(uintptr_t)7) +
-                                 ((size_t)blockIdx.x * NF_MLP_WAVES + (threadIdx.x >> 6)) * (COLS + NF_LIVE_PHASES) + COLS;
+                                 ((size_t)blockIdx.x * NF_MLP_WAVES + (threadIdx.x >> 6)) * cols + COLS;
                 if (end >= 0) (void)__hip_atomic_fetch_add(row + end, t, __ATOMIC_RELAXED, __HIP_MEMORY_SCOPE_AGENT);
                 if (start >= 0) (void)__hip_atomic_fetch_add(row + start, -t, __ATOMIC_RELAXED, __HIP_MEMORY_SCOPE_AGENT);
             }
@@ -137,10 +148,133 @@
 struct NfMarkedPre : Pre {
     long long* stats;
     __device__ __forceinline__ void wait() const {
+        nf_live_mark<true, COLS, true>(stats, NF_LIVE_PH_H_REST, -1);
         nf_live_mark<true, COLS>(stats, NF_LIVE_PH_TRUNK, NF_LIVE_PH_TILE);
         Pre::wait();
     }
+    __device__ __forceinline__ void first(f32x4 (&bias)[16], f32x4 (&w)[16]) const {
+        Pre::first(bias, w);
+        nf_live_mark<true, COLS, true>(stats, NF_LIVE_PH_H_WAIT, NF_LIVE_PH_H_L0, 0);
+    }
+    __device__ __forceinline__ void early(int lane) const {
+        nf_live_mark<true, COLS, true>(stats, NF_LIVE_PH_H_L0, NF_LIVE_PH_H_REST);
+        Pre::early(lane);
+    }
 };
+
+typedef const __attribute__((address_space(1))) float nf_gcf32;
+template <int NT>
+__device__ __forceinline__ void nf_live_z(float (&zn)[NT], const float* z_f, unsigned unit, int64_t n_points, int lane) {
+    nf_gcf32* z_v = (nf_gcf32*)z_f;
+    const int c = lane & 15;
+#pragma unroll
+    for (int t = 0; t < NT; ++t) {
+        int64_t p = (int64_t)unit * (16 * NT) + 16 * t + c;
+        if (p >= n_points) p = n_points - 1;
+        zn[t] = z_v[p];
+    }
+}
+
+struct NfLiveHead {
+    f32x4 (&hb)[16];
+    f32x4 (&hw)[16];
+    float (&zn)[NF_MLP_NT];
+    const unsigned& next_v;
+    const float* z_v;
+    int64_t n_points;
+    __device__ __forceinline__ void first(f32x4 (&bias)[16], f32x4 (&w)[16]) const {
+#pragma unroll
+        for (int no = 0; no < 16; ++no) {
+            bias[no] = hb[no];
+            w[no] = hw[no];
+        }
+    }
+    __device__ __forceinline__ void early(int lane) const {
+        nf_live_z<NF_MLP_NT>(zn, z_v, (unsigned)__builtin_amdgcn_readfirstlane((int)next_v), n_points, lane);
+        __builtin_amdgcn_sched_barrier(0);
+    }
+};
+template <class Pre>
+struct NfHeadPre : Pre {
+    static constexpr bool HEAD = true;
+    NfLiveHead h;
+    __device__ __forceinline__ void first(f32x4 (&bias)[16], f32x4 (&w)[16]) const { h.first(bias, w); }
+    __device__ __forceinline__ void early(int lane) const { h.early(lane); }
+};
+
+__device__ __forceinline__ void nf_live_pin(f32x4& v) {
+    float a = v.x, b = v.y, c = v.z, d = v.w;
+    asm volatile("" : "+v"(a), "+v"(b), "+v"(c), "+v"(d));
+    v = (f32x4){a, b, c, d};
+}
+
+__device__ __forceinline__ bool nf_live_narrow(int64_t n_points) {
+    asm volatile("" : "+s"(n_points));
+    return nf_idx_narrow(n_points);
+}
+
+template <int NT, bool STATS, int COLS>
+__device__ __forceinline__ void nf_live_inputs(f32x4 (&pe)[NT][4], f32x4 (&dirf)[NT][1], f32x4 (&hb)[16], f32x4 (&hw)[16], const float (&zn)[NT],
+                                               int64_t p0, int64_t n_points, int S, int lane, const NfW& Wi, const NfW& Ci,
+                                               const float* __restrict__ ro, const float* __restrict__ rd, const float* __restrict__ rd_view,
+                                               long long* stats) {
+    using Net = NfPaperNet;
+    const int g = lane >> 4, c = lane & 15;
+    int64_t ray[NT];
+    if (nf_live_narrow(n_points)) {
+        uint32_t S_h = (uint32_t)S, n_h = (uint32_t)n_points;
+        asm volatile("" : "+s"(S_h), "+s"(n_h));
+#pragma unroll
+        for (int t = 0; t < NT; ++t) {
+            uint32_t p = (uint32_t)p0 + 16 * t + c;
+            if (p >= n_h) p = n_h - 1u;
+            ray[t] = (int64_t)nf_idx_ray32(p, S_h);
+        }
+    } else {
+#pragma unroll
+        for (int t = 0; t < NT; ++t) {
+            int64_t p = p0 + 16 * t + c;
+            if (p >= n_points) p = n_points - 1;
+            ray[t] = nf_idx_ray64(p, S);
+        }
+    }
+    float o[NT][3], d[NT][3], dv[NT];
+    nf_gcf32* rdv = (nf_gcf32*)rd_view;
+#pragma unroll
+    for (int t = 0; t < NT; ++t) {
+#pragma unroll
+        for (int k = 0; k < 3; ++k) {
+            d[t][k] = rd[ray[t] * 3 + k];
+            o[t][k] = ro[ray[t] * 3 + k];
+        }
+        dv[t] = rdv[ray[t] * 3 + 2];
+    }
+    __builtin_amdgcn_sched_barrier(0);
+    nf_load_bias<16>(hb, Ci, Net::B_L0, lane);
+    nf_load_w16<16>(hw, Wi, Net::OFF_L0 / 4, lane);
+    __builtin_amdgcn_sched_barrier(0);
+    nf_live_mark<STATS, COLS, true>(stats, NF_LIVE_PH_H_LOAD, NF_LIVE_PH_H_PE, 32);
+#pragma unroll
+    for (int t = 0; t < NT; ++t) {
+        const float zz = zn[t];
+        const float px = nf_add(o[t][0], nf_mul(d[t][0], zz));
+        const float py = nf_add(o[t][1], nf_mul(d[t][1], zz));
+        const float pz = nf_add(o[t][2], nf_mul(d[t][2], zz));
+        nf_encode_point(px, py, pz, g, pe[t]);
+        float s, cs;
+        nf_sincos(nf_mul(dv[t], (float)(1 << g)), &s, &cs);
+        dirf[t][0] = (f32x4){s, cs, 0.0f, 0.0f};
+    }
+    if constexpr (STATS) {
+#pragma unroll
+        for (int t = 0; t < NT; ++t) {
+#pragma unroll
+            for (int j = 0; j < 4; ++j) nf_live_pin(pe[t][j]);
+            nf_live_pin(dirf[t][0]);
+        }
+    }
+    nf_live_mark<STATS, COLS, true>(stats, NF_LIVE_PH_H_PE, NF_LIVE_PH_H_WAIT);
+}
 
 template <int NT, bool STATS, bool GATE = false>
 __global__ void __launch_bounds__(64 * NF_MLP_WAVES, 1)
@@ -171,6 +305,9 @@
     unsigned unit_v = 0;
     if (lane == 0) unit_v = __hip_atomic_fetch_add(ctr_v, 1u, __ATOMIC_RELAXED, __HIP_MEMORY_SCOPE_AGENT);
     asm volatile("" : "+v"(unit_v));
+    float zn[NT] = {};
+    if (const unsigned u0 = (unsigned)__builtin_amdgcn_readfirstlane((int)unit_v); (int64_t)u0 * (16 * NT) < n_points)
+        nf_live_z<NT>(zn, z_v, u0, n_points, lane);
 #pragma unroll 1
     for (;;) {
         const int64_t p0 = (int64_t)(uint32_t)__builtin_amdgcn_readfirstlane((int)unit_v) * (16 * NT);
@@ -194,16 +331,19 @@
         int live_v = 0, run_v = 0;
         if (more) {
             nf_live_mark<STATS, COLS>(stats, -1, NF_LIVE_PH_TRUNK);
-            f32x4 pe[NT][4];
-            nf_net_inputs<NT>(pe, dirf, p0, n_points, S, lane, ro, rd, rdv_v, z_v);
+            nf_live_mark<STATS, COLS, true>(stats, -1, NF_LIVE_PH_H_LOAD);
+            f32x4 pe[NT][4], hb[16], hw[16];
+            nf_live_inputs<NT, STATS, COLS>(pe, dirf, hb, hw, zn, p0, n_points, S, lane, Wi, Ci, ro, rd, rdv_v, stats);
+            const NfLiveHead hd{hb, hw, zn, next_v, z_v, n_points};
             f32x4 acc[NT][16];
             if constexpr (GATE) {
                 if constexpr (STATS)
-                    nf_paper_net_body<Net, NT, 1, true, NfMarkedPre<NfGatePre, COLS>, true>(
-                        acc, sigma_own, pe, dirf, Wi, Ci, act4, lane, NfMarkedPre<NfGatePre, COLS>{{st, pf, ring_v, head_v, tail_v, bound_v}, stats});
+                    nf_paper_net_body<Net, NT, 1, true, NfMarkedPre<NfHeadPre<NfGatePre>, COLS>, true>(
+                        acc, sigma_own, pe, dirf, Wi, Ci, act4, lane,
+                        NfMarkedPre<NfHeadPre<NfGatePre>, COLS>{{{st, pf, ring_v, head_v, tail_v, bound_v}, hd}, stats});
                 else
-                    nf_paper_net_body<Net, NT, 1, true, NfGatePre, true>(acc, sigma_own, pe, dirf, Wi, Ci, act4, lane,
-                                                                         NfGatePre{st, pf, ring_v, head_v, tail_v, bound_v});
+                    nf_paper_net_body<Net, NT, 1, true, NfHeadPre<NfGatePre>, true>(
+                        acc, sigma_own, pe, dirf, Wi, Ci, act4, lane, NfHeadPre<NfGatePre>{{st, pf, ring_v, head_v, tail_v, bound_v}, hd});
 #pragma unroll
                 for (int t = 0; t < NT; ++t) {
                     const float s = acc[t][8].x, u = acc[t][8].y;
@@ -212,9 +352,10 @@
                 }
             } else if constexpr (STATS) {
                 nf_paper_net_body<Net, NT, 1, true>(acc, sigma_own, pe, dirf, Wi, Ci, act4, lane,
-                                                    NfMarkedPre<NfLivePre, COLS>{{st, wd, pf, ring_v, head_v, tail_v}, stats});
+                                                    NfMarkedPre<NfHeadPre<NfLivePre>, COLS>{{{st, wd, pf, ring_v, head_v, tail_v}, hd}, stats});
             } else {
-                nf_paper_net_body<Net, NT, 1, true>(acc, sigma_own, pe, dirf, Wi, Ci, act4, lane, NfLivePre{st, wd, pf, ring_v, head_v, tail_v});
+                nf_paper_net_body<Net, NT, 1, true>(acc, sigma_own, pe, dirf, Wi, Ci, act4, lane,
+                                                    NfHeadPre<NfLivePre>{{st, wd, pf, ring_v, head_v, tail_v}, hd});
             }
             nf_live_mark<STATS, COLS>(stats, NF_LIVE_PH_TILE, NF_LIVE_PH_APPEND);
             int lane_o = lane;
@@ -225,16 +366,24 @@
             asm volatile("" : "+v"(S_o));
             const int64_t p0_o = (int64_t)(uint32_t)__builtin_amdgcn_readfirstlane((int)(uint32_t)p0_v) |
                                  ((int64_t)__builtin_amdgcn_readfirstlane((int)(p0_v >> 32)) << 32);
+            bool last_o[NT];
+            if (nf_live_narrow(n_points)) {
+#pragma unroll
+                for (int t = 0; t < NT; ++t) last_o[t] = nf_idx_last32((uint32_t)p0_o + 16 * t + c, (uint32_t)S_o);
+            } else {
+#pragma unroll
+                for (int t = 0; t < NT; ++t) last_o[t] = nf_idx_last64(p0_o + 16 * t + c, S_o);
+            }
 #pragma unroll
             for (int t = 0; t < NT; ++t) {
                 const int64_t p = p0_o + 16 * t + c;
                 bool is_live;
                 if constexpr (GATE) {
-                    const bool last = (p + 1) % S_o == 0;
+                    const bool last = last_o[t];
                     is_live = g == 0 && p < n_points && (!proven[t] || last);
                     tag_own[t] = __int_as_float(last ? 1 : 0);
                 } else {
-                    is_live = g == 0 && p < n_points && (!(sigma_own[t] <= 0.0f) || (p + 1) % S_o == 0);
+                    is_live = g == 0 && p < n_points && (!(sigma_own[t] <= 0.0f) || last_o[t]);
                 }
                 live |= ((unsigned)__builtin_amdgcn_ballot_w64(is_live) & 0xffffu) << (16 * t);
             }
@@ -451,14 +600,14 @@
 template <bool STATS, bool GATE = false>
 static inline int nf_live_launch(const float* packed, const float* cond, const float* ro, const float* rd, const float* rd_view, const float* z,
                                  int64_t n_rays, int n_samples, float* raw, float* scratch, size_t scratch_floats, int max_workgroups,
-                                 long long* stats, nf_stream_t stream, const float* bound = nullptr, bool clocks = false) {
+                                 long long* stats, nf_stream_t stream, const float* bound = nullptr, int clocks = 0) {
     static_assert(NF_MLP_WAVES * 16 * NF_MLP_NT == 128, "nf_mlp_fwd_launch sizes the grid for 128 points per workgroup");
     if (max_workgroups < 0 || !scratch || ((uintptr_t)scratch & 15) ||
         scratch_floats < (size_t)nf_live_grid_cap(max_workgroups) * NF_MLP_WAVES * (NF_LIVE_WAVE_B / 4) ||
         (GATE && (!bound || ((uintptr_t)bound & 15))))
         return NF_EINVAL;
     const float* rdv = rd_view ? rd_view : rd;
-    if (STATS && clocks) stats = reinterpret_cast<long long*>((uintptr_t)stats | 1);
+    if (STATS && clocks) stats = reinterpret_cast<long long*>((uintptr_t)stats | (clocks == 2 ? 3 : 1));
     int rc = 0;
     const int launched = nf_mlp_fwd_launch(NF_FWD_INFER, packed, cond, ro, rd, z, raw, nullptr, n_rays, n_samples, [&](int64_t n_points, unsigned grid) {
         if ((n_points + 31) / 32 > ((int64_t)1 << 31)) {
diff --git a/4d-facial-avatars_amd/csrc/nf_mlp_live_stats.hip b/4d-facial-avatars_amd/csrc/nf_mlp_live_stats.hip
--- a/4d-facial-avatars_amd/csrc/nf_mlp_live_stats.hip
+++ b/4d-facial-avatars_amd/csrc/nf_mlp_live_stats.hip
@@ -1,11 +1,11 @@
 #include "nf_mlp_live_kernel.h"
 
-static int nf_live_stats_launch(bool clocks, const float* packed, const float* cond, const float* ro, const float* rd, const float* rd_view,
+static int nf_live_stats_launch(int clocks, const float* packed, const float* cond, const float* ro, const float* rd, const float* rd_view,
                                 const float* z, int64_t n_rays, int n_samples, float* raw, float* scratch, size_t scratch_floats,
                                 int max_workgroups, int64_t* stats, size_t stats_rows, nf_stream_t stream) {
     static_assert(sizeof(long long) == sizeof(int64_t), "a statistics row is int64s");
     if (max_workgroups < 0 || !stats || ((uintptr_t)stats & 7) || stats_rows < (size_t)nf_live_grid_cap(max_workgroups) * NF_MLP_WAVES) return NF_EINVAL;
-    const size_t cols = NF_LIVE_STAT_COLS + (clocks ? NF_LIVE_PHASES : 0);
+    const size_t cols = NF_LIVE_STAT_COLS + (clocks ? NF_LIVE_PHASES : 0) + (clocks == 2 ? NF_LIVE_HEAD_PHASES : 0);
     const hipError_t e = hipMemsetAsync(stats, 0, stats_rows * cols * sizeof(int64_t), nf_s(stream));
     if (e != hipSuccess) return (int)e;
     return nf_live_launch<true>(packed, cond, ro, rd, rd_view, z, n_rays, n_samples, raw, scratch, scratch_floats, max_workgroups,
@@ -15,13 +15,20 @@
 extern "C" int nf_paper_mlp_fwd_live_stats(const float* packed, const float* cond, const float* ro, const float* rd, const float* rd_view,
                                            const float* z, int64_t n_rays, int n_samples, float* raw, float* scratch, size_t scratch_floats,
                                            int max_workgroups, int64_t* stats, size_t stats_rows, nf_stream_t stream) {
-    return nf_live_stats_launch(false, packed, cond, ro, rd, rd_view, z, n_rays, n_samples, raw, scratch, scratch_floats, max_workgroups, stats,
+    return nf_live_stats_launch(0, packed, cond, ro, rd, rd_view, z, n_rays, n_samples, raw, scratch, scratch_floats, max_workgroups, stats,
                                 stats_rows, stream);
 }
 
 extern "C" int nf_paper_mlp_fwd_live_phases(const float* packed, const float* cond, const float* ro, const float* rd, const float* rd_view,
                                             const float* z, int64_t n_rays, int n_samples, float* raw, float* scratch, size_t scratch_floats,
                                             int max_workgroups, int64_t* stats, size_t stats_rows, nf_stream_t stream) {
-    return nf_live_stats_launch(true, packed, cond, ro, rd, rd_view, z, n_rays, n_samples, raw, scratch, scratch_floats, max_workgroups, stats,
+    return nf_live_stats_launch(1, packed, cond, ro, rd, rd_view, z, n_rays, n_samples, raw, scratch, scratch_floats, max_workgroups, stats,
                                 stats_rows, stream);
 }
+
+extern "C" int nf_paper_mlp_fwd_live_head(const float* packed, const float* cond, const float* ro, const float* rd, const float* rd_view,
+                                          const float* z, int64_t n_rays, int n_samples, float* raw, float* scratch, size_t scratch_floats,
+                                          int max_workgroups, int64_t* stats, size_t stats_rows, nf_stream_t stream) {
+    return nf_live_stats_launch(2, packed, cond, ro, rd, rd_view, z, n_rays, n_samples, raw, scratch, scratch_floats, max_workgroups, stats,
+                                stats_rows, stream);
+}
diff --git a/4d-facial-avatars_amd/csrc/nf_mlp_net_common.h b/4d-facial-avatars_amd/csrc/nf_mlp_net_common.h
--- a/4d-facial-avatars_amd/csrc/nf_mlp_net_common.h
+++ b/4d-facial-avatars_amd/csrc/nf_mlp_net_common.h
@@ -83,6 +83,26 @@
         nf_load_w16<16>(w, Wi, (OFF_) / 4 + 3 * 16 * 64, lane);                                               \
         NF_NET_PE_B(3); nf_tail<NT, 16, 16, 16, 1>(acc, w, bj, st, Wi, (OFF_NEXT_) / 4, Ci, B_NEXT_, act4, lane); \
     } while (0)
+template <int NT, bool FIRST>
+__device__ __forceinline__ void nf_pe_chunk_ahead(f32x4 (&acc)[NT][16], const f32x4 (&w)[16], f32x4 (&wn)[16], const NfW& W, unsigned wsrc,
+                                                  const f32x4 (&b)[NT], const f32x4 (&bias)[16], int lane) {
+    __builtin_amdgcn_sched_barrier(0);
+    nf_load_w16<16>(wn, W, wsrc, lane);
+    nf_chunk<NT, 16, FIRST>(acc, w, b, bias);
+#pragma unroll
+    for (int no = 0; no < 16; ++no) {
+        __builtin_amdgcn_sched_group_barrier(0x008, 4 * NT, 0);
+        __builtin_amdgcn_sched_group_barrier(0x020, 1, 0);
+    }
+    __builtin_amdgcn_sched_barrier(0);
+}
+#define NF_NET_PE_LAYER_FROM(OFF_, OFF_NEXT_, B_NEXT_)                                                        \
+    do {                                                                                                      \
+        NF_NET_PE_B(0); nf_pe_chunk_ahead<NT, true>(acc, w, st.wb, Wi, (OFF_) / 4 + 1 * 16 * 64, bj, st.bias, lane);  \
+        NF_NET_PE_B(1); nf_pe_chunk_ahead<NT, false>(acc, st.wb, w, Wi, (OFF_) / 4 + 2 * 16 * 64, bj, st.bias, lane); \
+        NF_NET_PE_B(2); nf_pe_chunk_ahead<NT, false>(acc, w, st.wb, Wi, (OFF_) / 4 + 3 * 16 * 64, bj, st.bias, lane); \
+        NF_NET_PE_B(3); nf_tail<NT, 16, 16, 16, 1>(acc, st.wb, bj, st, Wi, (OFF_NEXT_) / 4, Ci, B_NEXT_, act4, lane); \
+    } while (0)
 
 #define NF_NET_SAVE_PENDING(RELU_, MASKL_, NCH_)                                                    \
     do {                                                                                            \
diff --git a/4d-facial-avatars_amd/csrc/nf_mlp_paper_net.h b/4d-facial-avatars_amd/csrc/nf_mlp_paper_net.h
--- a/4d-facial-avatars_amd/csrc/nf_mlp_paper_net.h
+++ b/4d-facial-avatars_amd/csrc/nf_mlp_paper_net.h
@@ -206,6 +206,7 @@
     nf_chunk<NT, 1, false>(acc, st.wb, bj, st.bias)
 
 struct NfNoPre {
+    static constexpr bool HEAD = false;
     __device__ __forceinline__ void wait() const {}
     __device__ __forceinline__ void loads(const NfW&, const NfW&, int) const {}
 };
@@ -287,7 +288,14 @@
     nf_seg_lds<NT, 16, FIRST_, true>(acc, st, Wi, OFF_, 16, act4, lane);                                                    \
     nf_pending_b<NT, true>(bj, st);                                                                                         \
     nf_tail<NT, 16, 16, NO_NEXT_, NEXT_B_>(acc, st.wb, bj, st, Wi, OFF_NEXT_, Ci, B_NEXT_, act4, lane)
-    NF_NET_PE_LAYER(Net::B_L0, Net::OFF_L0, Net::OFF_L1, Net::B_L1);
+    if constexpr (Pre::HEAD) {
+        f32x4 w[16];
+        pre.first(st.bias, w);
+        NF_NET_PE_LAYER_FROM(Net::OFF_L0, Net::OFF_L1, Net::B_L1);
+        pre.early(lane);
+    } else {
+        NF_NET_PE_LAYER(Net::B_L0, Net::OFF_L0, Net::OFF_L1, Net::B_L1);
+    }
     NF_NET_LAYER256(Net::OFF_L1 / 4, true, Net::OFF_L2 / 4, Net::B_L2, 16, 1);
     NF_NET_LAYER256(Net::OFF_L2 / 4, true, Net::OFF_L3 / 4, Net::B_L3, 16, 0);
     NF_NET_L3_PE();
diff --git a/4d-facial-avatars_amd/nerf/_hip.py b/4d-facial-avatars_amd/nerf/_hip.py
--- a/4d-facial-avatars_amd/nerf/_hip.py
+++ b/4d-facial-avatars_amd/nerf/_hip.py
@@ -192,6 +192,8 @@
 _PROTOTYPES["nf_paper_mlp_fwd_live_phases"] = _PROTOTYPES["nf_paper_mlp_fwd_live_stats"]
 _PROTOTYPES["nf_paper_mlp_fwd_gated_stats"] = (C.c_int, [_P, _P, _P, _P, _P, _P, _P, _L, _I, _P, _P, _Z, _I, _P, _Z, _P])
 _PROTOTYPES["nf_paper_mlp_fwd_gated_phases"] = _PROTOTYPES["nf_paper_mlp_fwd_gated_stats"]
+_PROTOTYPES["nf_paper_mlp_fwd_live_head"] = _PROTOTYPES["nf_paper_mlp_fwd_live_stats"]
+_PROTOTYPES["nf_paper_mlp_fwd_gated_head"] = _PROTOTYPES["nf_paper_mlp_fwd_gated_stats"]
 _PROTOTYPES["nf_isosurface_workspace_bytes"] = (_Z, [_I, _I, _I])
 _PROTOTYPES["nf_isosurface_count"] = (C.c_int, [_P, _I, _I, _I, _F, _P, _Z, _P, _P])
 _PROTOTYPES["nf_isosurface_emit"] = (C.c_int, [_P, _I, _I, _I, _F, _P, _P, _P, _Z, _P, _L, _P, _L, _P, _P])
diff --git a/4d-facial-avatars_amd/nerf/ops.py b/4d-facial-avatars_amd/nerf/ops.py
--- a/4d-facial-avatars_amd/nerf/ops.py
+++ b/4d-facial-avatars_amd/nerf/ops.py
@@ -390,7 +390,10 @@
 LIVE_STAT_COLUMNS = ("units", "colour_runs", "flush_rows", "exit_clock") + LIVE_PHASE_COLUMNS
 
 
-def mlp_fwd_live_stats(fam: MLPFamily, packed, cond, ro, rd, z, rd_view=None, max_workgroups: int = 0):
+LIVE_HEAD_COLUMNS = ("clk_inputs_arrive", "clk_input_arithmetic", "clk_first_weights", "clk_layers_xyz_0", "clk_trunk_rest")
+
+
+def mlp_fwd_live_stats(fam: MLPFamily, packed, cond, ro, rd, z, rd_view=None, max_workgroups: int = 0, head: bool = False):
     if fam.prefix not in LIVE_FAMILIES:
         raise NotImplementedError(f"the {fam.prefix} model family has no live-colour kernel")
     dev = H.require_device(packed, cond, ro, rd, z, rd_view)
@@ -399,8 +402,8 @@
     with torch.cuda.device(dev):
         scratch = torch.empty(fam.fn("mlp_fwd_live_scratch_floats")(int(max_workgroups)), dtype=torch.float32, device=dev)
         waves = scratch.numel() * 4 // (LIVE_RING_ROWS * LIVE_ROW_BYTES)
-        stats = torch.empty((waves, len(LIVE_STAT_COLUMNS)), dtype=torch.int64, device=dev)
-        fam.call("mlp_fwd_live_phases", H.ptr(packed), H.ptr(cond), H.ptr(ro), H.ptr(rd), H.ptr(rd_view), H.ptr(z), n_rays, n_samples,
+        stats = torch.empty((waves, len(LIVE_STAT_COLUMNS) + (len(LIVE_HEAD_COLUMNS) if head else 0)), dtype=torch.int64, device=dev)
+        fam.call("mlp_fwd_live_head" if head else "mlp_fwd_live_phases", H.ptr(packed), H.ptr(cond), H.ptr(ro), H.ptr(rd), H.ptr(rd_view), H.ptr(z), n_rays, n_samples,
                  H.ptr(raw), H.ptr(scratch), scratch.numel(), int(max_workgroups), stats.data_ptr(), waves, H.stream_ptr(dev))
     return raw, stats
 
@@ -463,7 +466,7 @@
     return raw
 
 
-def mlp_fwd_gated_stats(fam: MLPFamily, packed, bound, cond, ro, rd, z, rd_view=None, max_workgroups: int = 0):
+def mlp_fwd_gated_stats(fam: MLPFamily, packed, bound, cond, ro, rd, z, rd_view=None, max_workgroups: int = 0, head: bool = False):
     if fam.prefix not in LIVE_FAMILIES:
         raise NotImplementedError(f"the {fam.prefix} model family has no gated kernel")
     dev = H.require_device(packed, bound, cond, ro, rd, z, rd_view)
@@ -472,8 +475,8 @@
     with torch.cuda.device(dev):
         scratch = torch.empty(fam.fn("mlp_fwd_live_scratch_floats")(int(max_workgroups)), dtype=torch.float32, device=dev)
         waves = scratch.numel() * 4 // (LIVE_RING_ROWS * LIVE_ROW_BYTES)
-        stats = torch.empty((waves, len(GATED_STAT_COLUMNS)), dtype=torch.int64, device=dev)
-        _gated_call("mlp_fwd_gated_phases", fam, packed, bound, cond, ro, rd, z, rd_view, max_workgroups, scratch, raw, stats.data_ptr(), waves,
+        stats = torch.empty((waves, len(GATED_STAT_COLUMNS) + (len(LIVE_HEAD_COLUMNS) if head else 0)), dtype=torch.int64, device=dev)
+        _gated_call("mlp_fwd_gated_head" if head else "mlp_fwd_gated_phases", fam, packed, bound, cond, ro, rd, z, rd_view, max_workgroups, scratch, raw, stats.data_ptr(), waves,
                     H.stream_ptr(dev))
     return raw, stats
 
diff --git a/include/nerface_hip.h b/include/nerface_hip.h
--- a/include/nerface_hip.h
+++ b/include/nerface_hip.h
@@ -412,6 +412,12 @@
 int nf_paper_mlp_fwd_gated_stats(const float* packed, const float* bound, const float* cond, const float* ro, const float* rd,
                                  const float* rd_view, const float* z, int64_t n_rays, int n_samples, float* raw, float* scratch,
                                  size_t scratch_floats, int max_workgroups, int64_t* stats, size_t stats_rows, nf_stream_t stream);
+int nf_paper_mlp_fwd_live_head(const float* packed, const float* cond, const float* ro, const float* rd, const float* rd_view,
+                               const float* z, int64_t n_rays, int n_samples, float* raw, float* scratch, size_t scratch_floats,
+                               int max_workgroups, int64_t* stats, size_t stats_rows, nf_stream_t stream);
+int nf_paper_mlp_fwd_gated_head(const float* packed, const float* bound, const float* cond, const float* ro, const float* rd,
+                                const float* rd_view, const float* z, int64_t n_rays, int n_samples, float* raw, float* scratch,
+                                size_t scratch_floats, int max_workgroups, int64_t* stats, size_t stats_rows, nf_stream_t stream);
 
 size_t nf_isosurface_workspace_bytes(int nx, int ny, int nz);
 int nf_isosurface_count(const float* grid, int nx, int ny, int nz, float level, void* workspace, size_t workspace_bytes,
```
